# facebookresearch/DetectAndTrack

Hardware: AMD Instinct MI355X
Metric: clips/sec (8-frame 800px) (higher is better)
Workload: dtype bf16; 1 GPU; 3D R-18 FPN3D keypoint R-CNN inference, 4 clip(s) of 1x3x8x768x1344 per step (= per forward) per GPU (kT=3 body+FPN, slice-center 2D heads, per clip: 1000 proposals, 100 detections -> kps_score -> decoded keypoints); mode=infer, weights=random-init (synthetic_params, seed 3), images_per_forward=4, forwards_in_flight=3, clips_in_flight=12, keyframe_dce=False, hip_graph=True, resident_input=True, parallelism=clip-sharded x1 (no data-path collective)

## Files before the change

### detectandtrack_amd/csrc/c_api.hip

```cpp
#include <stdlib.h>

#include "dat_common.h"

int dat_ensure_ws(dat_ctx* ctx, size_t bytes) {
    if (ctx->ws_bytes >= bytes) return DAT_OK;
    const size_t want = bytes + (bytes >> 2);
    void* grown = nullptr;
    if (hipMalloc(&grown, want) != hipSuccess) {
        (void)hipGetLastError();
        DAT_FAIL(ctx, DAT_ERR_ALLOC, "workspace hipMalloc(%zu) failed", want);
    }
    if (ctx->dbg_ws_poison && (hipMemset(grown, 0xFF, want) != hipSuccess || hipDeviceSynchronize() != hipSuccess)) {
        (void)hipGetLastError();
        hipFree(grown);
        DAT_FAIL(ctx, DAT_ERR_ALLOC, "workspace poison fill failed");
    }
    if (ctx->ws) ctx->ws_retired.push_back(ctx->ws);
    ctx->ws = grown;
    ctx->ws_bytes = want;
    ctx->ws_generation++;
    return DAT_OK;
}

extern "C" {

int dat_version(void) { return 1; }
int dat_h16_format(void) { return DAT_H16_FORMAT; }

int dat_ctx_create(dat_ctx** out, int device) {
    if (!out) return DAT_ERR_ARG;
    int ndev = 0;
    if (hipGetDeviceCount(&ndev) != hipSuccess || device < 0 || device >= ndev) return DAT_ERR_ARG;
    if (hipSetDevice(device) != hipSuccess) return DAT_ERR_ARG;
    dat_ctx* c = new dat_ctx();
    c->device = device;
    c->prof_enabled = 0;
    c->prof_ev = nullptr;
    c->prof_cap = c->prof_n = 0;
    c->prof_flops = nullptr;
    c->prof_tag = nullptr;
    c->ws = nullptr;
    c->ws_bytes = 0;
    c->ws_generation = 0;
    c->zeros = nullptr;
    {
        auto env_int = [](const char* name, int dflt) { const char* e = getenv(name); return e ? atoi(e) : dflt; };
        c->force_bp = env_int("DAT_CONV_BP", 0);
        c->force_ks = env_int("DAT_CONV_KSPLIT", 0);
        c->dbg_ablate = env_int("DAT_CONV_ABLATE", 0);
        c->dbg_ntap = env_int("DAT_CONV_NTAP", 1);
        c->dbg_ws64 = env_int("DAT_CONV_WS64", 1);
        c->dbg_pwlw = env_int("DAT_CONV_PWLW", 1);
        c->dbg_pwks = env_int("DAT_CONV_PWKS", 8);
        c->dbg_temporal = env_int("DAT_CONV_TEMPORAL", 1);
        c->dbg_wgrad_direct = env_int("DAT_WGRAD_DIRECT", 1);
        c->dbg_wgrad_ks = env_int("DAT_WGRAD_KS", 0);
        c->dbg_ablate_wgrad = env_int("DAT_WGRAD_ABLATE", 0);
        c->dbg_wgrad_sub = env_int("DAT_WGRAD_SUB", 2);
        c->dbg_pw_xcd = env_int("DAT_CONV_PW_XCD", 1);
        c->dbg_wgrad_pw = env_int("DAT_WGRAD_PW", 1);
        c->dbg_kps_sep = env_int("DAT_KPS_DECODE_SEP", 1);
        c->dbg_linear = env_int("DAT_CONV_LINEAR", 1);
        c->dbg_order = env_int("DAT_CONV_ORDER", 0);
        c->dbg_persist_pct = env_int("DAT_PERSIST_PCT", 100);
        c->dbg_bt_min = env_int("DAT_CONV_BT_MIN", 390);
        c->dbg_bt = env_int("DAT_CONV_BT", 1);
        c->dbg_roi_fold = env_int("DAT_ROI_BWD_FOLD", 1);
        c->dbg_ws_poison = env_int("DAT_WS_POISON", 0);
        c->num_cu = 0;
    }
    c->util_stream = nullptr;
    c->pinned = nullptr;
    if (hipStreamCreateWithFlags((hipStream_t*)&c->util_stream, hipStreamNonBlocking) != hipSuccess ||
        hipHostMalloc(&c->pinned, 256, hipHostMallocDefault) != hipSuccess) {
        if (c->util_stream) hipStreamDestroy((hipStream_t)c->util_stream);
        delete c;
        return DAT_ERR_ALLOC;
    }
    if (hipMalloc(&c->zeros, 512) != hipSuccess || hipMemsetAsync(c->zeros, 0, 512, (hipStream_t)c->util_stream) != hipSuccess ||
        hipStreamSynchronize((hipStream_t)c->util_stream) != hipSuccess) {
        if (c->zeros) hipFree(c->zeros);
        hipHostFree(c->pinned);
        hipStreamDestroy((hipStream_t)c->util_stream);
        delete c;
        return DAT_ERR_ALLOC;
    }
    *out = c;
    return DAT_OK;
}

void dat_ctx_destroy(dat_ctx* ctx) {
    if (!ctx) return;
    if (ctx->prof_ev) {
        for (int i = 0; i < 2 * ctx->prof_cap; ++i) hipEventDestroy(ctx->prof_ev[i]);
        delete[] ctx->prof_ev;
        delete[] ctx->prof_flops;
        delete[] ctx->prof_tag;
    }
    if (ctx->ws) hipFree(ctx->ws);
    for (void* p : ctx->ws_retired) hipFree(p);
    if (ctx->zeros) hipFree(ctx->zeros);
    if (ctx->pinned) hipHostFree(ctx->pinned);
    if (ctx->util_stream) hipStreamDestroy((hipStream_t)ctx->util_stream);
    delete ctx;
}

const char* dat_last_error(dat_ctx* ctx) { return ctx ? ctx->last_error.c_str() : "null dat_ctx"; }

int dat_ws_info(dat_ctx* ctx, void** ptr, size_t* bytes, int* generation) {
    if (!ctx) return DAT_ERR_ARG;
    if (ptr) *ptr = ctx->ws;
    if (bytes) *bytes = ctx->ws_bytes;
    if (generation) *generation = ctx->ws_generation;
    return DAT_OK;
}

int dat_ws_reserve(dat_ctx* ctx, size_t bytes) {
    if (!ctx) return DAT_ERR_ARG;
    return dat_ensure_ws(ctx, bytes);
}

int dat_prof_enable(dat_ctx* ctx, int capacity) {
    if (!ctx) return DAT_ERR_ARG;
    if (capacity <= 0) {
        ctx->prof_enabled = 0;
        return DAT_OK;
    }
    if (capacity > ctx->prof_cap) {
        if (ctx->prof_ev) {
            for (int i = 0; i < 2 * ctx->prof_cap; ++i) hipEventDestroy(ctx->prof_ev[i]);
            delete[] ctx->prof_ev;
            delete[] ctx->prof_flops;
            delete[] ctx->prof_tag;
        }
        ctx->prof_ev = new hipEvent_t[2 * capacity];
        for (int i = 0; i < 2 * capacity; ++i) hipEventCreate(&ctx->prof_ev[i]);
        ctx->prof_flops = new double[capacity];
        ctx->prof_tag = new int[capacity];
        ctx->prof_cap = capacity;
    }
    ctx->prof_n = 0;
    ctx->prof_enabled = 1;
    if (hipDeviceSynchronize() != hipSuccess ||
        hipMemsetAsync((char*)ctx->zeros + 256, 0, 16, (hipStream_t)ctx->util_stream) != hipSuccess ||
        hipStreamSynchronize((hipStream_t)ctx->util_stream) != hipSuccess) return DAT_ERR_LAUNCH;
    return DAT_OK;
}

int dat_prof_clock(dat_ctx* ctx, double* shader_mhz) {
    if (!ctx || !shader_mhz) return DAT_ERR_ARG;
    unsigned long long* h = (unsigned long long*)ctx->pinned;
    if (hipDeviceSynchronize() != hipSuccess ||
        hipMemcpyAsync(h, (char*)ctx->zeros + 256, 16, hipMemcpyDeviceToHost, (hipStream_t)ctx->util_stream) != hipSuccess ||
        hipStreamSynchronize((hipStream_t)ctx->util_stream) != hipSuccess) return DAT_ERR_LAUNCH;
    *shader_mhz = h[1] ? 100.0 * (double)h[0] / (double)h[1] : 0.0;
    return DAT_OK;
}

int dat_prof_read(dat_ctx* ctx, int max_records, int* tags, double* flops, float* ms) {
    if (!ctx) return DAT_ERR_ARG;
    const int n = ctx->prof_n < max_records ? ctx->prof_n : max_records;
    for (int i = 0; i < n; ++i) {
        float t = 0.f;
        if (hipEventSynchronize(ctx->prof_ev[2 * i + 1]) != hipSuccess ||
            hipEventElapsedTime(&t, ctx->prof_ev[2 * i], ctx->prof_ev[2 * i + 1]) != hipSuccess) {
            (void)hipGetLastError();
            t = 0.f;
        }
        if (tags) tags[i] = ctx->prof_tag[i];
        if (flops) flops[i] = ctx->prof_flops[i];
        if (ms) ms[i] = t;
    }
    ctx->prof_n = 0;
    return n;
}

int dat_fill_zero(dat_ctx* ctx, dat_stream s, void* ptr, size_t bytes) {
    DAT_ENFORCE(ctx, ptr || bytes == 0, "fill_zero: null pointer");
    if (bytes == 0) return DAT_OK;
    if (hipMemsetAsync(ptr, 0, bytes, (hipStream_t)s) != hipSuccess) DAT_FAIL(ctx, DAT_ERR_LAUNCH, "fill_zero: hipMemsetAsync failed");
    return DAT_OK;
}

}
```

### detectandtrack_amd/csrc/conv3d_igemm.hip

```cpp
#include "conv_internal.h"

using namespace dat_conv;

namespace {

template <int BP, int NTAP> struct MinWaves { static constexpr int value = (NTAP > 0 && NTAP != 10 && BP == 128) ? 3 : 2; };
template <int DT, int BN, int BP, int WAVES_N, int ONE, int NTAP, int ODT>
__global__ __launch_bounds__(NTHREADS, (MinWaves<BP, NTAP>::value)) void conv3d_igemm_kernel(const ConvParams p) {
    static_assert(ONE == 1, "see the comment above");
    constexpr int ES = ElemOf<DT>::size;
    constexpr int OES = ElemOf<ODT>::size;
    constexpr int CK = Mma<DT>::CK;
    constexpr int WAVES_P = 4 / WAVES_N;
    constexpr int WN = BN / WAVES_N;
    constexpr int WP = BP / WAVES_P;
    constexpr int MT = WN / 32;
    constexpr int PT = WP / 32;
    static_assert(MT >= 1 && PT >= 1, "tile too small");

#ifdef DAT_CONV_TRACE
    const unsigned long long tr_k0 = __builtin_amdgcn_s_memtime();
    unsigned long long tr_k1 = tr_k0;
#endif
    unsigned long long clk_c0 = 0, clk_r0 = 0;
    if (p.clk) { clk_c0 = __builtin_amdgcn_s_memtime(); clk_r0 = __builtin_amdgcn_s_memrealtime(); }
    extern __shared__ __attribute__((aligned(16))) char smem[];
    char* patch = smem;

    const int tid = threadIdx.x;
    const int lane = tid & 63;
    const int wave = __builtin_amdgcn_readfirstlane(tid >> 6);
    const int wave_n = wave % WAVES_N;
    const int wave_p = wave / WAVES_N;

    unsigned bid = blockIdx.x;
    if (!(p.ablate & 16)) bid = xcd_block_map(bid, p.nblocks);
    int split, nb;
    unsigned tile;
    if (p.order) {
        tile = bid % p.ntiles;
        bid /= p.ntiles;
        split = bid % p.ksplit;
        nb = bid / p.ksplit;
    } else {
        split = bid % p.ksplit;
        bid /= p.ksplit;
        nb = bid % p.nblk_n;
        tile = bid / p.nblk_n;
    }
    const int fc = tile % p.otn;
    tile /= p.otn;
    const int tw_i = tile % p.tiles_w;
    tile /= p.tiles_w;
    const int th_i = tile % p.tiles_h;
    const int clip = tile / p.tiles_h;
    const int f = clip * p.otn + fc;
    const int t = p.ot0 + fc;
    const int f_in = clip * p.T + t;
    const int n0 = nb * BN;
    const int TW = 1 << p.tw_log2;
    const int oh0 = th_i << p.th_log2;
    const int ow0 = tw_i * p.tile_w;
    const int ih0 = oh0 * p.sh - p.ph;
    const int iw0 = ow0 * p.sw - p.pw;

    int rowbase[PT];
#pragma unroll
    for (int j = 0; j < PT; ++j) {
        const int pos = wave_p * WP + j * 32 + (lane & 31);
        const int ohl = pos >> p.tw_log2, owl = pos & (TW - 1);
        rowbase[j] = ohl * p.rsh * p.PW + owl * p.rsw;
    }
    const int khalf = lane >> 5;

    f32x16_t acc[MT][PT];
#pragma unroll
    for (int i = 0; i < MT; ++i)
#pragma unroll
        for (int j = 0; j < PT; ++j)
#pragma unroll
            for (int r = 0; r < 16; ++r) acc[i][j][r] = 0.f;

    int kt_lo = 0, kt_hi = p.KT - 1;
    while (kt_lo < p.KT && (t + kt_lo - p.pt) < p.in_lo) ++kt_lo;
    while (kt_hi >= 0 && (t + kt_hi - p.pt) >= p.in_hi) --kt_hi;
    const int n_kt = kt_hi - kt_lo + 1;
    const int ntap = p.KH * p.KW;
    const int ntab = p.tab_n;
    const int npatch = n_kt * p.n_cchunks;
    const int pi_lo = (npatch * split) / p.ksplit, pi_hi = (npatch * (split + 1)) / p.ksplit;
    const int total = (pi_hi - pi_lo) * ntab;

    const int npatch_items = p.PH * p.PW * 8;

    typedef const __attribute__((address_space(1))) void* gptr_t;
    typedef __attribute__((address_space(3))) void* lptr_t;
#ifndef DAT_PATCH_AUX
#define DAT_PATCH_AUX 0
#endif
#define P_DMA(SRC_, DST_) __builtin_amdgcn_global_load_lds((gptr_t)(SRC_), (lptr_t)(DST_), 16, 0, DAT_PATCH_AUX)
#define P_COMMIT() asm volatile("s_waitcnt vmcnt(0)" ::: "memory")

    const size_t wd_cc_stride = (size_t)(p.Cout_pad >> 5) * 4096;
    const char* const wd_lane = p.w + (size_t)((n0 + wave_n * WN) >> 5) * 4096 + lane * 16;
#define WD_PTR(KT_, CC_, TI_) (wd_lane + ((size_t)((KT_) * ntap + p.tab_tap[(TI_)]) * p.n_cchunks + (CC_)) * wd_cc_stride)
    if constexpr (NTAP > 0) {
      constexpr int NT = NTAP == 10 ? 9 : NTAP;
      if (total > 0) {
        constexpr int MAXCH = patch_pieces_per_wave(NTAP, BP);
        const int kt_hi_x = kt_lo + n_kt;
        int kshift = 0;
        if (n_kt == p.KT && (DAT_KT_ROTATE)) kshift = (p.KT - (t + kt_lo - p.pt) % p.KT) % p.KT;
        int kt = kt_lo + pi_lo / p.n_cchunks + kshift, cc = pi_lo % p.n_cchunks;
        if (kt >= kt_hi_x) kt -= n_kt;
        constexpr bool PACK16 = NTAP != 10;
        constexpr int NQ = PACK16 ? (PT + 1) / 2 : PT;
        unsigned qp[NT][NQ];
#pragma unroll
        for (int tp = 0; tp < NT; ++tp)
#pragma unroll
            for (int j = 0; j < PT; ++j) {
                int row = rowbase[j] + p.tab_rowoff[tp];
                if (p.lin_w > 0) {
                    const int gpos = ow0 + wave_p * WP + j * 32 + (lane & 31);
                    const int rem = gpos % (p.lin_h * p.lin_w);
                    const int y = rem / p.lin_w, x = rem - y * p.lin_w;
                    const int yy = y + tp / p.KW - p.KH / 2, xx = x + tp % p.KW - p.KW / 2;
                    if ((unsigned)yy >= (unsigned)p.lin_h || (unsigned)xx >= (unsigned)p.lin_w) row = p.lin_zero_row;
                }
                const int g = (row >> 1) & 7;
                const unsigned a16 = (unsigned)(row * PPITCH) + (unsigned)(((khalf ^ (g & 1)) << 4) | ((g >> 1) << 5));
                if (!PACK16) qp[tp][j] = a16;
                else if (j & 1) qp[tp][j >> 1] |= a16 << 16;
                else qp[tp][j >> 1] = a16;
            }
        const int nchunks = (npatch_items + 63) >> 6;
        int poff[MAXCH];
#pragma unroll
        for (int u = 0; u < MAXCH; ++u) {
            const int c = wave + 4 * u;
            const int it = c * 64 + lane;
            int off = -2;
            if (c < nchunks && it < npatch_items) {
                const int row = it >> 3;
                const int slot = (it ^ (row >> 1)) & 7;
                const int prow = p.pw_magic ? (int)__umulhi((unsigned)row, p.pw_magic) : row, pcol = row - prow * p.PW;
                const int ih = ih0 + p.tab_dy[0] + prow * p.psh, iw = iw0 + p.tab_dx[0] + pcol * p.psw;
                off = (ih >= 0 && ih < p.H && iw >= 0 && iw < p.W && row != p.lin_zero_row) ? (int)((unsigned)(ih * p.W + iw) * (unsigned)(p.Cin * ES) + (unsigned)(slot * 16)) : -1;
            }
            poff[u] = off;
        }
        const size_t tap_stride = (size_t)p.n_cchunks * wd_cc_stride;
        const char* const wd_base = p.w + (size_t)((n0 + wave_n * WN) >> 5) * 4096;
        const unsigned lane16 = (unsigned)lane * 16u;
        const char* wcur = wd_base + ((size_t)(kt * ntap) * p.n_cchunks + cc) * wd_cc_stride;
        uint4 wa[MT][4];
#pragma unroll
        for (int i = 0; i < MT; ++i)
#pragma unroll
            for (int ks = 0; ks < 4; ++ks) wa[i][ks] = *(const uint4*)(wcur + i * 4096 + ks * 1024 + lane16);
        const int npat = pi_hi - pi_lo;
        for (int pi = 0; pi < npat; ++pi) {
            if (!((p.ablate & 1) && pi > 0) && !(p.x3 && pi > 0 && cc % 3 == 1)) {
                __syncthreads();
                const int fin = f_in + kt - p.pt;
                const char* xbase = p.x + ((size_t)fin * p.H * p.W) * p.Cin * ES + (size_t)(p.x3 ? (cc / 3) * 2 + (cc % 3 == 2) : cc) * CK * ES;
#pragma unroll
                for (int u = 0; u < MAXCH; ++u) {
                    if (poff[u] != -2) {
                        const char* src = poff[u] >= 0 ? xbase + (unsigned)poff[u] : p.zeros;
                        P_DMA(src, patch + (wave + 4 * u) * 1024);
                    }
                }
                P_COMMIT();
                __syncthreads();
            }
            int ncc = cc + 1, nkt = kt;
            if (ncc == p.n_cchunks) { ncc = 0; if (++nkt == kt_hi_x) nkt = kt_lo; }
            const char* wnextpatch = (pi + 1 < npat) ? wd_base + ((size_t)(nkt * ntap) * p.n_cchunks + ncc) * wd_cc_stride : wcur;
            __builtin_amdgcn_s_setprio(1);
            uint4 b[2][PT];
            unsigned qa[PT];
#pragma unroll
            for (int jj = 0; jj < NQ; ++jj) asm volatile("" : "+v"(qp[0][jj]));
#pragma unroll
            for (int j = 0; j < PT; ++j) qa[j] = !PACK16 ? qp[0][j % NQ] : (j & 1) ? (qp[0][(j >> 1) % NQ] >> 16) : (qp[0][(j >> 1) % NQ] & 0xffffu);
#pragma unroll
            for (int j = 0; j < PT; ++j) b[0][j] = *(const uint4*)(patch + qa[j]);
#pragma unroll
            for (int tp = 0; tp < NT; ++tp) {
                const char* wnext = (tp + 1 < NT) ? wcur + (size_t)(tp + 1) * tap_stride : wnextpatch;
#pragma unroll
                for (int ks = 0; ks < 4; ++ks) {
                    const int cur = ks & 1, nxt = cur ^ 1;
                    if (ks < 3) {
#pragma unroll
                        for (int j = 0; j < PT; ++j) b[nxt][j] = *(const uint4*)(patch + (qa[j] ^ (unsigned)((ks + 1) << 5)));
                    } else if (tp + 1 < NT) {
#pragma unroll
                        for (int jj = 0; jj < NQ; ++jj) asm volatile("" : "+v"(qp[tp + 1 < NT ? tp + 1 : tp][jj]));
#pragma unroll
                        for (int j = 0; j < PT; ++j) {
                            const unsigned w2 = qp[tp + 1 < NT ? tp + 1 : tp][(PACK16 ? j >> 1 : j) % NQ];
                            qa[j] = !PACK16 ? w2 : (j & 1) ? (w2 >> 16) : (w2 & 0xffffu);
                        }
#pragma unroll
                        for (int j = 0; j < PT; ++j) b[nxt][j] = *(const uint4*)(patch + qa[j]);
                    }
#pragma unroll
                    for (int i = 0; i < MT; ++i)
#pragma unroll
                        for (int j = 0; j < PT; ++j) Mma<DT>::step(wa[i][ks], b[cur][j], acc[i][j]);
#pragma unroll
                    for (int i = 0; i < MT; ++i) wa[i][ks] = *(const uint4*)(wnext + i * 4096 + ks * 1024 + lane16);
                    __builtin_amdgcn_sched_barrier(0);
                }
            }
            __builtin_amdgcn_s_setprio(0);
            wcur = wnextpatch;
            cc = ncc; kt = nkt;
        }
      }
    } else
    if (total > 0) {
        const int kt_hi_x = kt_lo + n_kt;
        int kshift = 0;
        if (n_kt == p.KT && (DAT_KT_ROTATE)) kshift = (p.KT - (t + kt_lo - p.pt) % p.KT) % p.KT;
        int kt = kt_lo + pi_lo / p.n_cchunks + kshift, cc = pi_lo % p.n_cchunks, ti = 0;
        if (kt >= kt_hi_x) kt -= n_kt;
        uint4 wa[MT][4];
        {
            const char* w0 = WD_PTR(kt, cc, 0);
#pragma unroll
            for (int i = 0; i < MT; ++i)
#pragma unroll
                for (int ks = 0; ks < 4; ++ks) wa[i][ks] = *(const uint4*)(w0 + i * 4096 + ks * 1024);
        }
        const int nchunks = (npatch_items + 63) >> 6;
#ifdef DAT_CONV_TRACE
        unsigned long long tr_reload = 0, tr_wait = 0, tr_bar = 0, tr_issue = 0, tr_mma = 0, tr_t;
#define TR_NOW() __builtin_readcyclecounter()
#define TR_ADD(ACC_) { const unsigned long long n_ = TR_NOW(); ACC_ += n_ - tr_t; tr_t = n_; }
        tr_t = TR_NOW();
        const unsigned long long tr_c0 = __builtin_amdgcn_s_memtime(), tr_r0 = __builtin_amdgcn_s_memrealtime();
#else
#define TR_ADD(ACC_)
#endif
        for (int step = 0; step < total; ++step) {
            const bool x3_same = p.x3 && p.tab_new == 1u && step > 0 && cc % 3 == 1;
            if (((p.tab_new >> ti) & 1u) && !((p.ablate & 1) && step > 0) && !(p.ablate & 8) && !x3_same) {
                __syncthreads();
                const int fin = f_in + kt - p.pt;
                const char* xbase = p.x + ((size_t)fin * p.H * p.W) * p.Cin * ES + (size_t)(p.x3 ? (cc / 3) * 2 + (cc % 3 == 2) : cc) * CK * ES;
                const int py0 = ih0 + p.tab_dy[ti], px0 = iw0 + p.tab_dx[ti];
#pragma unroll 2
                for (int c = wave; c < nchunks; c += 4) {
                    const int it = c * 64 + lane;
                    if (it < npatch_items) {
                        const int row = it >> 3;
                        const int slot = (it ^ (row >> 1)) & 7;
                        const int prow = p.pw_magic ? (int)__umulhi((unsigned)row, p.pw_magic) : row, pcol = row - prow * p.PW;
                        const int ih = py0 + prow * p.psh, iw = px0 + pcol * p.psw;
                        const char* src = p.zeros;
                        if (ih >= 0 && ih < p.H && iw >= 0 && iw < p.W)
                            src = xbase + ((unsigned)(ih * p.W + iw) * (unsigned)(p.Cin * ES) + (unsigned)(slot * 16));
                        P_DMA(src, patch + c * 1024);
                    }
                }
            }
            TR_ADD(tr_reload);
            if ((p.tab_new >> ti) & 1u) {
                P_COMMIT();
                TR_ADD(tr_wait);
                __syncthreads();
            }
            TR_ADD(tr_bar);
            int nti = ti + 1, ncc = cc, nkt = kt;
            if (nti == ntab) {
                nti = 0;
                if (++ncc == p.n_cchunks) { ncc = 0; if (++nkt == kt_hi_x) nkt = kt_lo; }
            }
            const char* const wnext = (step + 1 < total) ? WD_PTR(nkt, ncc, nti) : WD_PTR(kt, cc, ti);

            TR_ADD(tr_issue);
            __builtin_amdgcn_s_setprio(1);
            {
                const int tapoff = p.tab_rowoff[ti];
                const char* bp[PT];
                int bx[PT];
#pragma unroll
                for (int j = 0; j < PT; ++j) {
                    const int row = rowbase[j] + tapoff;
                    const int g = (row >> 1) & 7;
                    bp[j] = patch + (row * PPITCH + ((khalf ^ (g & 1)) << 4));
                    bx[j] = g >> 1;
                }
                uint4 b[2][PT];
#pragma unroll
                for (int j = 0; j < PT; ++j) b[0][j] = *(const uint4*)(bp[j] + (bx[j] << 5));
#pragma unroll
                for (int ks = 0; ks < 4; ++ks) {
                    const int cur = ks & 1, nxt = cur ^ 1;
                    if (ks < 3) {
#pragma unroll
                        for (int j = 0; j < PT; ++j) b[nxt][j] = *(const uint4*)(bp[j] + (((ks + 1) ^ bx[j]) << 5));
                    }
#pragma unroll
                    for (int i = 0; i < MT; ++i)
#pragma unroll
                        for (int j = 0; j < PT; ++j) Mma<DT>::step(wa[i][ks], b[cur][j], acc[i][j]);
#pragma unroll
                    for (int i = 0; i < MT; ++i) wa[i][ks] = *(const uint4*)(wnext + i * 4096 + ks * 1024);
                    __builtin_amdgcn_sched_barrier(0);
                }
            }
            __builtin_amdgcn_s_setprio(0);
            ti = nti; cc = ncc; kt = nkt;
            TR_ADD(tr_mma);
        }
#ifdef DAT_CONV_TRACE
        if (tid == 0 && p.dbg) {
            atomicAdd(&p.dbg[0], tr_reload); atomicAdd(&p.dbg[1], tr_wait); atomicAdd(&p.dbg[2], tr_bar);
            atomicAdd(&p.dbg[3], tr_issue); atomicAdd(&p.dbg[4], tr_mma); atomicAdd(&p.dbg[5], (unsigned long long)total);
            atomicAdd(&p.dbg[6], __builtin_amdgcn_s_memtime() - tr_c0);
            atomicAdd(&p.dbg[7], __builtin_amdgcn_s_memrealtime() - tr_r0);
        }
        tr_k1 = __builtin_amdgcn_s_memtime();
#endif
    }
#undef WD_PTR
#undef P_COMMIT
#undef P_DMA

    static_assert(WN == 64, "epilogue staging assumes 64 channels per wave");
    constexpr int CPL = 16 / OES;
    constexpr int LPP = WN / CPL;
    constexpr int PPI = 64 / LPP;
    __syncthreads();
    char* est = smem + wave * (32 * EPI_PITCH);
    const int sl_c = (lane % LPP) * CPL;
    const int sl_p = lane / LPP;
    const int cbase = n0 + wave_n * WN;
    const int c_st = cbase + sl_c;
    const bool part_mode = p.ksplit > 1;
    float sc[CPL], bi[CPL];
#pragma unroll
    for (int e = 0; e < CPL; ++e) {
        const bool ok = (c_st + e) < p.Cout;
        sc[e] = (!part_mode && p.scale && ok) ? p.scale[c_st + e] : 1.f;
        bi[e] = (!part_mode && p.bias && ok) ? p.bias[c_st + e] : 0.f;
    }
    const size_t npos_all = (size_t)p.frames * p.Ho * p.Wo;
    const size_t tile_pos = ((size_t)f * p.Ho + oh0) * p.Wo + ow0;
    char* const ybase = p.y + tile_pos * p.out_cs * OES;
    const char* const rbase = p.res_mode == 2 ? p.res + (size_t)f * (p.Ho >> 1) * (p.Wo >> 1) * p.out_cs * OES
                                              : p.res + tile_pos * p.out_cs * OES;
    const char* const abase = p.res2 + tile_pos * p.out_cs * OES;
    float* const pbase = part_mode ? p.part + ((size_t)split * npos_all + tile_pos) * p.Cout : nullptr;
    constexpr int NQ = 32 / PPI;
    const bool m4 = p.res_mode == 4;
    const bool res_pre = p.res_mode && !m4 && !part_mode && (p.out_cs & 7) == 0 && c_st + CPL <= p.Cout;
    uint4 rq[2][NQ];
    auto res_fetch = [&](int j, uint4* dst) __attribute__((always_inline)) {
#pragma unroll
        for (int q = 0; q < NQ; ++q) {
            const int pos = wave_p * WP + j * 32 + q * PPI + sl_p;
            const int ohl = pos >> p.tw_log2, owl = pos & (TW - 1);
            const int oh = oh0 + ohl, ow = ow0 + owl;
            const bool live = oh < p.Ho && ow < p.Wo && !(p.ablate & 4);
            unsigned rpos = (unsigned)(ohl * p.Wo + owl);
            if (p.res_mode == 2) rpos = (unsigned)((oh >> 1) * (p.Wo >> 1) + (ow >> 1));
            dst[q] = *(const uint4*)(rbase + (live ? (rpos * (unsigned)p.out_cs + (unsigned)c_st) * (unsigned)OES : 0u));
        }
    };
    if (res_pre) res_fetch(0, rq[0]);
#pragma unroll
    for (int j = 0; j < PT; ++j) {
        if (res_pre && j + 1 < PT) res_fetch(j + 1, rq[(j + 1) & 1]);
#pragma unroll
        for (int i = 0; i < MT; ++i)
#pragma unroll
            for (int g = 0; g < 4; ++g)
                *(float4*)(est + (lane & 31) * EPI_PITCH + (i * 32 + g * 8 + khalf * 4) * 4) =
                    make_float4(acc[i][j][g * 4 + 0], acc[i][j][g * 4 + 1], acc[i][j][g * 4 + 2], acc[i][j][g * 4 + 3]);
        __builtin_amdgcn_wave_barrier();
#pragma unroll
        for (int q = 0; q < NQ; ++q) {
            const int pl = q * PPI + sl_p;
            float v[CPL];
#pragma unroll
            for (int e4 = 0; e4 < CPL / 4; ++e4) {
                const float4 t = *(const float4*)(est + pl * EPI_PITCH + (sl_c + e4 * 4) * 4);
                v[e4 * 4 + 0] = t.x; v[e4 * 4 + 1] = t.y; v[e4 * 4 + 2] = t.z; v[e4 * 4 + 3] = t.w;
            }
            const int pos = wave_p * WP + j * 32 + pl;
            const int ohl = pos >> p.tw_log2, owl = pos & (TW - 1);
            const int oh = oh0 + ohl, ow = ow0 + owl;
            if (oh >= p.Ho || ow >= p.Wo || c_st >= p.Cout || (p.ablate & 4)) continue;
            const unsigned lpos = (unsigned)(ohl * p.Wo + owl);
            const int nch = min(CPL, p.Cout - c_st);
            if (part_mode) {
                float* dst = pbase + (lpos * (unsigned)p.Cout + (unsigned)c_st);
#pragma unroll
                for (int e4 = 0; e4 < CPL / 4; ++e4)
                    if (e4 * 4 < nch) *(float4*)(dst + e4 * 4) = make_float4(v[e4 * 4], v[e4 * 4 + 1], v[e4 * 4 + 2], v[e4 * 4 + 3]);
                continue;
            }
#pragma unroll
            for (int e = 0; e < CPL; ++e) v[e] = v[e] * sc[e] + bi[e];
            if (res_pre) {
                const uint4 r = rq[j & 1][q];
                if (ODT == DAT_BF16) {
                    const uint32_t ru[4] = {r.x, r.y, r.z, r.w};
#pragma unroll
                    for (int e2 = 0; e2 < CPL / 2; ++e2) {
                        v[2 * e2] = res_combine(v[2 * e2], bf2f((uint16_t)(ru[e2 % 4] & 0xffff)), p.res_mode);
                        v[2 * e2 + 1] = res_combine(v[2 * e2 + 1], bf2f((uint16_t)(ru[e2 % 4] >> 16)), p.res_mode);
                    }
                } else {
                    v[0] = res_combine(v[0], __uint_as_float(r.x), p.res_mode); v[1] = res_combine(v[1], __uint_as_float(r.y), p.res_mode);
                    v[2] = res_combine(v[2], __uint_as_float(r.z), p.res_mode); v[3] = res_combine(v[3], __uint_as_float(r.w), p.res_mode);
                }
            } else if (m4) {
                const unsigned off = (lpos * (unsigned)p.out_cs + (unsigned)c_st) * (unsigned)OES;
                const char* rp = rbase + off;
                const char* ap = abase + off;
                if (ODT == DAT_BF16) {
#pragma unroll
                    for (int e4 = 0; e4 < CPL / 4; ++e4)
                        if (e4 * 4 < nch) {
                            const uint2 r = *(const uint2*)(rp + e4 * 8), o = *(const uint2*)(ap + e4 * 8);
                            v[e4 * 4 + 0] = res_combine4(v[e4 * 4 + 0], bf2f((uint16_t)(o.x & 0xffff)), bf2f((uint16_t)(r.x & 0xffff)));
                            v[e4 * 4 + 1] = res_combine4(v[e4 * 4 + 1], bf2f((uint16_t)(o.x >> 16)), bf2f((uint16_t)(r.x >> 16)));
                            v[e4 * 4 + 2] = res_combine4(v[e4 * 4 + 2], bf2f((uint16_t)(o.y & 0xffff)), bf2f((uint16_t)(r.y & 0xffff)));
                            v[e4 * 4 + 3] = res_combine4(v[e4 * 4 + 3], bf2f((uint16_t)(o.y >> 16)), bf2f((uint16_t)(r.y >> 16)));
                        }
                } else {
                    const float4 r = *(const float4*)rp, o = *(const float4*)ap;
                    v[0] = res_combine4(v[0], o.x, r.x); v[1] = res_combine4(v[1], o.y, r.y);
                    v[2] = res_combine4(v[2], o.z, r.z); v[3] = res_combine4(v[3], o.w, r.w);
                }
            } else if (p.res_mode) {
                unsigned rpos = lpos;
                if (p.res_mode == 2) rpos = (unsigned)((oh >> 1) * (p.Wo >> 1) + (ow >> 1));
                const char* rp = rbase + (rpos * (unsigned)p.out_cs + (unsigned)c_st) * (unsigned)OES;
                if (ODT == DAT_BF16) {
#pragma unroll
                    for (int e4 = 0; e4 < CPL / 4; ++e4)
                        if (e4 * 4 < nch) {
                            const uint2 r = *(const uint2*)(rp + e4 * 8);
                            v[e4 * 4 + 0] = res_combine(v[e4 * 4 + 0], bf2f((uint16_t)(r.x & 0xffff)), p.res_mode);
                            v[e4 * 4 + 1] = res_combine(v[e4 * 4 + 1], bf2f((uint16_t)(r.x >> 16)), p.res_mode);
                            v[e4 * 4 + 2] = res_combine(v[e4 * 4 + 2], bf2f((uint16_t)(r.y & 0xffff)), p.res_mode);
                            v[e4 * 4 + 3] = res_combine(v[e4 * 4 + 3], bf2f((uint16_t)(r.y >> 16)), p.res_mode);
                        }
                } else {
                    const float4 r = *(const float4*)rp;
                    v[0] = res_combine(v[0], r.x, p.res_mode); v[1] = res_combine(v[1], r.y, p.res_mode);
                    v[2] = res_combine(v[2], r.z, p.res_mode); v[3] = res_combine(v[3], r.w, p.res_mode);
                }
            }
            if (p.relu) {
#pragma unroll
                for (int e = 0; e < CPL; ++e) v[e] = fmaxf(v[e], 0.f);
            }
            char* yp = ybase + (lpos * (unsigned)p.out_cs + (unsigned)c_st) * (unsigned)OES;
            if (ODT == DAT_BF16) {
                uint32_t o[CPL / 2];
#pragma unroll
                for (int e2 = 0; e2 < CPL / 2; ++e2) o[e2] = f2bf2(v[2 * e2], v[2 * e2 + 1]);
                if (nch == CPL && (p.out_cs & 7) == 0) {
                    *(uint4*)yp = make_uint4(o[0], o[1], o[2], o[3]);
                } else {
                    *(uint2*)yp = make_uint2(o[0], o[1]);
                    if (nch > 4) *(uint2*)(yp + 8) = make_uint2(o[2], o[3]);
                }
            } else {
                *(float4*)yp = make_float4(v[0], v[1], v[2], v[3]);
                if (ODT == DAT_F32 && DT == DAT_BF16 && p.y_split)
                    split_hi_lo_store(p.y_split + ((tile_pos + lpos) * (size_t)(2 * p.out_cs) + (size_t)((c_st >> 6) * 128 + (c_st & 63))) * 2, v);
            }
        }
        __builtin_amdgcn_wave_barrier();
    }
    if (p.clk && threadIdx.x == 0) {
        atomicAdd(&p.clk[0], __builtin_amdgcn_s_memtime() - clk_c0);
        atomicAdd(&p.clk[1], __builtin_amdgcn_s_memrealtime() - clk_r0);
    }
#ifdef DAT_CONV_TRACE
    asm volatile("s_waitcnt vmcnt(0)" ::: "memory");
    if (tid == 0 && p.dbg) {
        const unsigned long long e = __builtin_amdgcn_s_memtime();
        atomicAdd(&p.dbg[8], e - tr_k0);
        atomicAdd(&p.dbg[9], e - tr_k1);
    }
#endif
}

template <int DT>
__global__ void splitk_finish_kernel(const float* __restrict__ part, int ksplit, size_t npos, int Cout, int out_cs,
                                     const float* __restrict__ scale, const float* __restrict__ bias,
                                     const char* __restrict__ res, int res_mode, int frames, int Ho, int Wo, int relu,
                                     char* y, char* __restrict__ y_split = nullptr, const char* res2 = nullptr) {
    const int c4 = Cout >> 2;
    const size_t total = npos * c4;
    for (size_t i = blockIdx.x * (size_t)blockDim.x + threadIdx.x; i < total; i += (size_t)gridDim.x * blockDim.x) {
        const int c = (int)(i % c4) * 4;
        const size_t opos = i / c4;
        float4 a = *(const float4*)(part + opos * Cout + c);
        for (int s = 1; s < ksplit; ++s) {
            const float4 b = *(const float4*)(part + ((size_t)s * npos + opos) * Cout + c);
            a.x += b.x; a.y += b.y; a.z += b.z; a.w += b.w;
        }
        float v[4] = {a.x, a.y, a.z, a.w};
        if (scale) { const float4 s4 = *(const float4*)(scale + c); v[0] *= s4.x; v[1] *= s4.y; v[2] *= s4.z; v[3] *= s4.w; }
        if (bias) { const float4 b4 = *(const float4*)(bias + c); v[0] += b4.x; v[1] += b4.y; v[2] += b4.z; v[3] += b4.w; }
        if (res_mode) {
            size_t rpos = opos;
            if (res_mode == 2) {
                const int ow = opos % Wo;
                const size_t q = opos / Wo;
                const int oh = q % Ho;
                const size_t f = q / Ho;
                rpos = (f * (Ho >> 1) + (oh >> 1)) * (Wo >> 1) + (ow >> 1);
            }
            if (res_mode == 4) {
                if (DT == DAT_BF16) {
                    const uint2 r = *(const uint2*)(res + (rpos * out_cs + c) * 2), o = *(const uint2*)(res2 + (opos * out_cs + c) * 2);
                    v[0] = res_combine4(v[0], bf2f((uint16_t)(o.x & 0xffff)), bf2f((uint16_t)(r.x & 0xffff)));
                    v[1] = res_combine4(v[1], bf2f((uint16_t)(o.x >> 16)), bf2f((uint16_t)(r.x >> 16)));
                    v[2] = res_combine4(v[2], bf2f((uint16_t)(o.y & 0xffff)), bf2f((uint16_t)(r.y & 0xffff)));
                    v[3] = res_combine4(v[3], bf2f((uint16_t)(o.y >> 16)), bf2f((uint16_t)(r.y >> 16)));
                } else {
                    const float4 r = *(const float4*)(res + (rpos * out_cs + c) * 4), o = *(const float4*)(res2 + (opos * out_cs + c) * 4);
                    v[0] = res_combine4(v[0], o.x, r.x); v[1] = res_combine4(v[1], o.y, r.y);
                    v[2] = res_combine4(v[2], o.z, r.z); v[3] = res_combine4(v[3], o.w, r.w);
                }
            } else if (DT == DAT_BF16) {
                const uint2 r = *(const uint2*)(res + (rpos * out_cs + c) * 2);
                v[0] = res_combine(v[0], bf2f((uint16_t)(r.x & 0xffff)), res_mode); v[1] = res_combine(v[1], bf2f((uint16_t)(r.x >> 16)), res_mode);
                v[2] = res_combine(v[2], bf2f((uint16_t)(r.y & 0xffff)), res_mode); v[3] = res_combine(v[3], bf2f((uint16_t)(r.y >> 16)), res_mode);
            } else {
                const float4 r = *(const float4*)(res + (rpos * out_cs + c) * 4);
                v[0] = res_combine(v[0], r.x, res_mode); v[1] = res_combine(v[1], r.y, res_mode);
                v[2] = res_combine(v[2], r.z, res_mode); v[3] = res_combine(v[3], r.w, res_mode);
            }
        }
        if (relu) { v[0] = fmaxf(v[0], 0.f); v[1] = fmaxf(v[1], 0.f); v[2] = fmaxf(v[2], 0.f); v[3] = fmaxf(v[3], 0.f); }
        if (DT == DAT_BF16) {
            uint2 o;
            o.x = f2bf2(v[0], v[1]);
            o.y = f2bf2(v[2], v[3]);
            *(uint2*)(y + (opos * out_cs + c) * 2) = o;
        } else {
            *(float4*)(y + (opos * out_cs + c) * 4) = make_float4(v[0], v[1], v[2], v[3]);
            if (y_split) split_hi_lo_store(y_split + (opos * (size_t)(2 * out_cs) + (size_t)((c >> 6) * 128 + (c & 63))) * 2, v);
        }
    }
}

static long long linear_tiles(const dat_ctx* ctx, const dat_conv_desc* d, const ConvParams& p, int bpv) {
    if (!ctx->dbg_linear || !ctx->dbg_ntap || d->KH != 3 || d->KW != 3 || d->stride_h != 1 || d->stride_w != 1 || d->res_mode == 2 ||
        p.H != p.Ho || p.W != p.Wo)
        return 0;
    if (d->KT == 1 && (d->pad_t != 0 || d->out_tn > 0)) return 0;
    const long long per = d->KT > 1 ? (long long)p.Ho * p.Wo : (long long)p.frames * p.Ho * p.Wo;
    const long long nr = bpv + 2 * (p.Wo + 1) + 1;
    if (((nr * 8 + 63) >> 6) > 4 * patch_pieces_per_wave(9, bpv) || nr * PPITCH >= 65536 ||
        per * std::max(p.Cin, std::max(p.out_cs, p.Cout)) * 4 >= (1ll << 31))
        return 0;
    return (d->KT > 1 ? (long long)p.frames : 1) * ((per + bpv - 1) / bpv);
}

}

namespace dat_conv {

TileChoice choose_tile(int Ho, int Wo, int bp_log2, int sh, int sw, int KH, int KW) {
    TileChoice best{0, bp_log2};
    double best_cost = 1e30;
    for (int a = 0; a <= bp_log2; ++a) {
        const int b = bp_log2 - a;
        const long long th = 1 << a, tw = 1 << b;
        const long long tiles = cdiv_ll(Ho, th) * cdiv_ll(Wo, tw);
        const double waste = (double)(tiles * th * tw) / ((double)Ho * Wo);
        const long long PH = th + (KH - 1) / sh;
        const long long PW = tw + (KW - 1) / sw;
        const double halo = (double)(PH * PW) / (double)(th * tw);
        const double conflict = (tw < 32 && KW > 1) ? 1.06 : 1.0;
        const double cost = waste * (1.0 + 0.15 * (halo - 1.0)) * conflict;
        if (cost < best_cost - 1e-9) {
            best_cost = cost;
            best = TileChoice{a, b};
        }
    }
    return best;
}

void conv_build_tap_table(ConvParams& p) {
    int n = 0;
    p.tab_new = 0;
    for (int py = 0; py < p.sh && py < p.KH; ++py)
        for (int px = 0; px < p.sw && px < p.KW; ++px) {
            bool first = true;
            for (int kh = py; kh < p.KH; kh += p.sh)
                for (int kw = px; kw < p.KW; kw += p.sw) {
                    p.tab_tap[n] = kh * p.KW + kw;
                    p.tab_rowoff[n] = (kh / p.sh) * p.PW + (kw / p.sw);
                    p.tab_dy[n] = (short)py;
                    p.tab_dx[n] = (short)px;
                    if (first) p.tab_new |= 1u << n;
                    first = false;
                    ++n;
                }
        }
    p.tab_n = n;
}

int conv_set_frame_window(dat_ctx* ctx, const dat_conv_desc* d, ConvParams& p, const char* who) {
    p.in_lo = d->in_tn > 0 ? d->in_t0 : 0;
    p.in_hi = d->in_tn > 0 ? d->in_t0 + d->in_tn : d->T;
    DAT_ENFORCE(ctx, p.in_lo >= 0 && p.in_hi <= d->T, "%s: non-zero input frames [%d, %d) outside T %d", who, p.in_lo, p.in_hi, d->T);
    p.ot0 = d->out_tn > 0 ? d->out_t0 : 0;
    p.otn = d->out_tn > 0 ? d->out_tn : d->T;
    DAT_ENFORCE(ctx, p.ot0 >= 0 && p.ot0 + p.otn <= d->T, "%s: output frames [%d, %d) outside T %d", who, p.ot0, p.ot0 + p.otn, d->T);
    p.frames = d->frames / d->T * p.otn;
    return DAT_OK;
}

}

namespace {

template <int DT, int BN, int BP, int WAVES_N, int NTAP, int ODT>
int launch_conv(dat_ctx* ctx, hipStream_t st, ConvParams& p, int bp_log2, int ksplit, bool linear = false) {
    TileChoice tc = choose_tile(p.Ho, p.Wo, bp_log2, p.sh, p.sw, p.KH, p.KW);
    p.lin_h = p.lin_w = 0;
    p.lin_zero_row = -1;
    if (linear) {
        const bool per_frame = p.KT > 1;
        const long long total = per_frame ? (long long)p.Ho * p.Wo : (long long)p.frames * p.Ho * p.Wo;
        DAT_ENFORCE(ctx, NTAP == 9 && (per_frame || p.pt == 0) && p.sh == 1 && p.sw == 1 && p.H == p.Ho && p.W == p.Wo && p.res_mode != 2 &&
                             total * std::max(p.Cin, std::max(p.out_cs, p.Cout)) * 4 < (1ll << 31),
                    "conv3d: linear tiling on an unsupported layer");
        p.lin_h = p.H; p.lin_w = p.W;
        const int wr = p.W, nr = BP + 2 * (wr + 1) + 1;
        tc = TileChoice{0, bp_log2};
        p.H = p.Ho = 1; p.W = p.Wo = (int)total;
        if (!per_frame) { p.frames = 1; p.T = 1; p.ot0 = 0; p.otn = 1; p.in_lo = 0; p.in_hi = 1; }
        p.ph = 0; p.pw = wr + 1;
        p.lin_zero_row = nr - 1;
        p.th_log2 = 0; p.tw_log2 = bp_log2;
        p.tile_w = BP;
        p.tiles_h = 1; p.tiles_w = (int)cdiv_ll(total, BP);
        p.psh = p.psw = 1; p.rsh = p.rsw = 1;
        p.PH = 1; p.PW = nr;
        p.tab_new = 1u; p.tab_n = 9;
        for (int i = 0; i < 9; ++i) { p.tab_tap[i] = i; p.tab_rowoff[i] = (i / 3) * wr + i % 3; p.tab_dy[i] = p.tab_dx[i] = 0; }
    }
    const int th = 1 << tc.th_log2, tw = 1 << tc.tw_log2;
    if (!linear) {
    p.th_log2 = tc.th_log2;
    p.tw_log2 = tc.tw_log2;
    p.tile_w = tw;
    p.tiles_h = (p.Ho + th - 1) / th;
    p.tiles_w = (p.Wo + tw - 1) / tw;
    p.psh = p.sh;
    p.psw = p.sw;
    p.rsh = p.rsw = 1;
    p.PH = th + (p.KH - 1) / p.sh;
    p.PW = tw + (p.KW - 1) / p.sw;
    }
    if (linear) {
    } else if (NTAP == 10) {
        p.psh = p.psw = 1;
        p.rsh = p.sh; p.rsw = p.sw;
        p.PH = (th - 1) * p.sh + p.KH;
        p.PW = (tw - 1) * p.sw + p.KW;
        p.tab_new = 1u;
        p.tab_n = p.KH * p.KW;
        for (int i = 0; i < p.tab_n; ++i) {
            p.tab_tap[i] = i;
            p.tab_rowoff[i] = (i / p.KW) * p.PW + i % p.KW;
            p.tab_dy[i] = p.tab_dx[i] = 0;
        }
    } else {
        DAT_ENFORCE(ctx, p.KH * p.KW <= 32, "conv3d: %dx%d spatial kernel exceeds the 32-entry tap table", p.KH, p.KW);
        conv_build_tap_table(p);
    }
    p.pw_magic = conv_pw_magic(p.PW);
    p.n_cchunks = p.x3 ? p.Cin / Mma<DT>::CK / 2 * 3 : p.Cin / Mma<DT>::CK;
    p.ablate = ctx->dbg_ablate;
    p.nblk_n = p.Cout_pad / BN;
    long long nblocks = (long long)p.frames * p.tiles_h * p.tiles_w * p.nblk_n;
    {
        const int npatch_min = (p.KT > 1 ? p.KT - 1 : 1) * p.n_cchunks;
        int ks = ksplit < 1 ? 1 : (ksplit > npatch_min ? npatch_min : ksplit);
        p.ksplit = ks;
        p.part = nullptr;
        if (ks > 1) {
            const size_t bytes = (size_t)ks * p.frames * p.Ho * p.Wo * p.Cout * sizeof(float);
            int rc = dat_ensure_ws(ctx, bytes);
            if (rc != DAT_OK) return rc;
            p.part = (float*)ctx->ws;
        }
        nblocks *= ks;
    }
    DAT_ENFORCE(ctx, nblocks > 0 && nblocks < (1ll << 31), "conv3d: grid of %lld blocks unsupported", nblocks);
    DAT_ENFORCE(ctx, (long long)p.Ho * p.Wo * std::max(p.out_cs, p.Cout) * 4 < (1ll << 31),
                "conv3d: one output frame of %dx%dx%d exceeds the 2-GB range of the epilogue's 32-bit offsets", p.Ho, p.Wo, p.out_cs);
    p.nblocks = (unsigned)nblocks;
    p.ntiles = (unsigned)(nblocks / ((long long)p.ksplit * p.nblk_n));
    p.order = ctx->dbg_order > 0;
    size_t lds = ((size_t)p.PH * p.PW * PPITCH + 1023) & ~(size_t)1023;
    if (lds < EPI_SLICES_BYTES) lds = EPI_SLICES_BYTES;
    DAT_ENFORCE(ctx, lds <= 160 * 1024, "conv3d: LDS patch of %zu bytes exceeds 160 KiB (tile %dx%d, stride %dx%d)", lds,
                th, tw, p.sh, p.sw);
    auto kern = conv3d_igemm_kernel<DT, BN, BP, WAVES_N, 1, NTAP, ODT>;
    if (NTAP > 0) {
        DAT_ENFORCE(ctx, p.tab_n == (NTAP == 10 ? 9 : NTAP) && p.tab_new == 1u &&
                             (((size_t)p.PH * p.PW * 8 + 63) >> 6) <= (size_t)4 * patch_pieces_per_wave(NTAP, BP) && (NTAP == 10 || (size_t)p.PH * p.PW * PPITCH < 65536),
                    "conv3d: unrolled-tap variant on an unsupported shape (%d taps, patch %dx%d)", p.tab_n, p.PH, p.PW);
        for (int i = 0; i < p.tab_n; ++i) DAT_ENFORCE(ctx, p.tab_tap[i] == i, "conv3d: unrolled-tap variant needs taps in natural order");
    }
    {
        const int rc = dat_ensure_lds(ctx, (const void*)kern, 160 * 1024);
        if (rc != DAT_OK) return rc;
    }
#ifdef DAT_CONV_TRACE
    static unsigned long long* dbg = nullptr;
    if (!dbg) hipMalloc(&dbg, 128);
    hipMemsetAsync(dbg, 0, 128, st);
    p.dbg = dbg;
#endif
    hipLaunchKernelGGL(kern, dim3(p.nblocks), dim3(NTHREADS), lds, st, p);
#ifdef DAT_CONV_TRACE
    {
        unsigned long long h[16];
        hipStreamSynchronize(st);
        hipMemcpy(h, dbg, 128, hipMemcpyDeviceToHost);
        if (h[5]) fprintf(stderr, "TRACE BN=%d BP=%d blocks=%u steps/blk=%.1f | per step: reload %.0f wait %.0f barrier %.0f issue %.0f mma %.0f | shader clock %.0f MHz | per block: total %.0f epilogue %.0f cycles\n",
                          BN, BP, p.nblocks, (double)h[5] / p.nblocks, (double)h[0] / h[5], (double)h[1] / h[5], (double)h[2] / h[5],
                          (double)h[3] / h[5], (double)h[4] / h[5], 100.0 * (double)h[6] / (double)h[7], (double)h[8] / p.nblocks, (double)h[9] / p.nblocks);
    }
#endif
    if (p.ksplit > 1) {
        const size_t npos = (size_t)p.frames * p.Ho * p.Wo;
        const size_t tot = npos * (p.Cout >> 2);
        const int blocks = (int)std::min<size_t>((tot + 255) / 256, 256 * 16);
        hipLaunchKernelGGL(splitk_finish_kernel<ODT>, dim3(blocks), dim3(256), 0, st, (const float*)p.part, p.ksplit, npos, p.Cout,
                           p.out_cs, p.scale, p.bias, p.res, p.res_mode, p.frames, p.Ho, p.Wo, p.relu, p.y, ODT == DAT_F32 && DT == DAT_BF16 ? p.y_split : nullptr, p.res2);
    }
    DAT_CHECK_LAUNCH(ctx, "conv3d_igemm");
    return DAT_OK;
}

}

extern "C" {

int dat_conv3d_out_shape(const dat_conv_desc* d, int* Ho, int* Wo) {
    if (!d || d->stride_h < 1 || d->stride_w < 1) return DAT_ERR_ARG;
    *Ho = (d->H + 2 * d->pad_h - d->KH) / d->stride_h + 1;
    *Wo = (d->W + 2 * d->pad_w - d->KW) / d->stride_w + 1;
    return DAT_OK;
}

size_t dat_conv3d_packed_weight_bytes(const dat_conv_desc* d) {
    if (d->dtype == DAT_BF16X3) return (size_t)d->KT * d->KH * d->KW * cout_pad_of(d) * d->Cin * 3 * 2;
    return (size_t)d->KT * d->KH * d->KW * cout_pad_of(d) * d->Cin * dat_esize(d->dtype);
}

double dat_conv3d_flops(const dat_conv_desc* d, int Cin_real, int Cout_real) {
    int Ho, Wo;
    dat_conv3d_out_shape(d, &Ho, &Wo);
    const double oframes = d->out_tn > 0 && d->T > 0 ? (double)(d->frames / d->T) * d->out_tn : (double)d->frames;
    return 2.0 * Cout_real * Cin_real * d->KT * d->KH * d->KW * oframes * Ho * Wo;
}

static int conv3d_fwd_impl(dat_ctx* ctx, dat_stream s, const dat_conv_desc* d, const void* x, const void* w_packed,
                           const float* scale, const float* bias, const void* residual, void* y, void* y_split, const void* addend = nullptr);

int dat_conv3d_fwd(dat_ctx* ctx, dat_stream s, const dat_conv_desc* d, const void* x, const void* w_packed,
                   const float* scale, const float* bias, const void* residual, void* y) {
    return conv3d_fwd_impl(ctx, s, d, x, w_packed, scale, bias, residual, y, nullptr);
}

int dat_conv3d_fwd_x3(dat_ctx* ctx, dat_stream s, const dat_conv_desc* d, const void* x_split, const void* w_packed,
                      const float* scale, const float* bias, const void* residual, void* y, void* y_split) {
    DAT_ENFORCE(ctx, d && d->dtype == DAT_BF16X3, "conv3d_fwd_x3: the descriptor's dtype must be DAT_BF16X3");
    DAT_ENFORCE(ctx, !y_split || (d->out_cstride % 64 == 0 && d->Cout == d->out_cstride),
                "conv3d_fwd_x3: a split output needs Cout == out_cstride, a multiple of 64 (got %d / %d)", d->Cout, d->out_cstride);
    return conv3d_fwd_impl(ctx, s, d, x_split, w_packed, scale, bias, residual, y, y_split);
}

int dat_conv3d_fwd_sum_mask(dat_ctx* ctx, dat_stream s, const dat_conv_desc* d, const void* x, const void* w_packed,
                            const float* scale, const float* bias, const void* addend, const void* mask, void* y) {
    DAT_ENFORCE(ctx, d && d->res_mode == 4, "conv3d_fwd_sum_mask: the descriptor's res_mode must be 4");
    DAT_ENFORCE(ctx, addend && mask, "conv3d_fwd_sum_mask: null addend / mask");
    return conv3d_fwd_impl(ctx, s, d, x, w_packed, scale, bias, mask, y, nullptr, addend);
}

static int conv3d_fwd_impl(dat_ctx* ctx, dat_stream s, const dat_conv_desc* d, const void* x, const void* w_packed,
                           const float* scale, const float* bias, const void* residual, void* y, void* y_split, const void* addend) {
    DAT_ENFORCE(ctx, d && x && w_packed && y, "conv3d_fwd: null argument");
    DAT_ENFORCE(ctx, d->dtype == DAT_F32 || d->dtype == DAT_BF16 || d->dtype == DAT_BF16X3, "conv3d_fwd: bad dtype %d", d->dtype);
    const bool x3 = d->dtype == DAT_BF16X3;
    DAT_ENFORCE(ctx, !x3 || DAT_H16_FORMAT == 0, "conv3d_fwd: DAT_BF16X3 needs the bf16 build of the library (this one holds IEEE half in its 16-bit tensors)");
    DAT_ENFORCE(ctx, d->Cin % 64 == 0, "conv3d_fwd: Cin (channel stride) %d must be a multiple of 64", d->Cin);
    DAT_ENFORCE(ctx, d->Cout % 4 == 0 && d->out_cstride % 4 == 0 && d->out_cstride >= d->Cout,
                "conv3d_fwd: Cout %d / out_cstride %d must be multiples of 4", d->Cout, d->out_cstride);
    DAT_ENFORCE(ctx, d->frames % d->T == 0, "conv3d_fwd: frames %d not a multiple of T %d", d->frames, d->T);
    DAT_ENFORCE(ctx, d->res_mode >= 0 && d->res_mode <= 4, "conv3d_fwd: res_mode %d", d->res_mode);
    DAT_ENFORCE(ctx, d->res_mode != 4 || (!x3 && !y_split && addend), "conv3d_fwd: res_mode 4 (sum + mask) goes through dat_conv3d_fwd_sum_mask, bf16 / fp32 only");
    DAT_ENFORCE(ctx, d->res_mode == 0 || residual, "conv3d_fwd: res_mode %d needs a residual pointer", d->res_mode);
    DAT_ENFORCE(ctx, d->pad_t * 2 + 1 == d->KT || d->out_tn > 0,
                "conv3d_fwd: temporal pad %d must be (KT-1)/2 for KT %d unless out_t0/out_tn select the output frames",
                d->pad_t, d->KT);
    ConvParams p;
    memset(&p, 0, sizeof(p));
    p.x = (const char*)x; p.w = (const char*)w_packed; p.scale = scale; p.bias = bias;
    p.res = (const char*)residual; p.res2 = (const char*)addend; p.y = (char*)y; p.y_split = (char*)y_split;
    p.zeros = (const char*)ctx->zeros;
    p.clk = ctx->prof_enabled ? (unsigned long long*)((char*)ctx->zeros + 256) : nullptr;
    {
        const int rcw = conv_set_frame_window(ctx, d, p, "conv3d_fwd");
        if (rcw != DAT_OK) return rcw;
    }
    p.T = d->T; p.H = d->H; p.W = d->W; p.Cin = x3 ? 2 * d->Cin : d->Cin;
    p.x3 = x3;
    dat_conv3d_out_shape(d, &p.Ho, &p.Wo);
    DAT_ENFORCE(ctx, p.Ho > 0 && p.Wo > 0, "conv3d_fwd: empty output %dx%d", p.Ho, p.Wo);
    DAT_ENFORCE(ctx, d->res_mode != 2 || (p.Ho % 2 == 0 && p.Wo % 2 == 0), "conv3d_fwd: res_mode 2 needs even output dims");
    p.Cout = d->Cout; p.out_cs = d->out_cstride; p.Cout_pad = cout_pad_of(d);
    p.KT = d->KT; p.KH = d->KH; p.KW = d->KW; p.sh = d->stride_h; p.sw = d->stride_w;
    p.pt = d->pad_t; p.ph = d->pad_h; p.pw = d->pad_w; p.relu = d->relu; p.res_mode = d->res_mode;
    hipStream_t st = (hipStream_t)s;

    const bool small_n = d->Cout <= 64;
    const int force_bp = ctx->force_bp, force_ks = ctx->force_ks;
    const int ck = d->dtype == DAT_F32 ? 32 : 64;
    const int ncc = x3 ? d->Cin / 64 * 3 : d->Cin / ck;
    const int npatch = d->KT * ncc, npatch_min = (d->KT > 1 ? d->KT - 1 : 1) * ncc;
    const int ntaps = d->KH * d->KW;
    const long long nbn = p.Cout_pad / (small_n ? 64 : 128);
    int bp = 128, ksplit = 1;
    {
        double best = 1e30;
        const bool deep_1x1 = (ntaps == 1 && ncc >= 16);
        for (int cand_bp = 128; cand_bp <= 256; cand_bp += 128) {
            if (cand_bp == 256 && (small_n || ntaps == 1)) continue;
            if (cand_bp == 256 && !force_bp && ctx->dbg_ntap && !(ctx->dbg_ntap & 4) && d->KH == 3 && d->KW == 3 && d->stride_h == 2 && d->stride_w == 2) continue;
            if (force_bp && cand_bp != force_bp && !(force_bp == 256 && (small_n || ntaps == 1))) continue;
            const int lg = cand_bp == 256 ? 8 : 7;
            const TileChoice tc = choose_tile(p.Ho, p.Wo, lg, p.sh, p.sw, p.KH, p.KW);
            long long tiles = cdiv_ll(p.Ho, 1ll << tc.th_log2) * cdiv_ll(p.Wo, 1ll << tc.tw_log2) * p.frames;
            {
                const long long tl = linear_tiles(ctx, d, p, cand_bp);
                if (tl > 0 && tl * 10 <= tiles * 9) tiles = tl;
            }
            const int ks_max = (ntaps > 1 || deep_1x1) ? (deep_1x1 ? 8 : 4) : 1;
            for (int ks = 1; ks <= ks_max && ks <= npatch_min; ++ks) {
                if (force_ks && ks != std::min(force_ks, npatch_min)) continue;
                const double nblk = (double)tiles * nbn * ks;
                const double slots = 512.0;
                double rounds = nblk / slots;
                if (rounds <= 3.0) rounds = ceil(rounds); else rounds += 0.5;
                const double steps = ceil((double)npatch / ks) * ntaps;
                const bool strided_taps = ntaps > 1 && (d->stride_h > 1 || d->stride_w > 1);
                const double step_us = cand_bp == 256 ? (strided_taps ? 2.8 : 2.15) : 1.35;
                const double fixed_us = 2.0 + 0.6 * ceil((double)npatch / ks);
                double t = rounds * (steps * step_us + fixed_us);
                if (ks > 1) t += 4.0 + 2.0 * ks * (double)p.frames * p.Ho * p.Wo * d->Cout * 4.0 / 3.0e6;
                if (t < best) { best = t; bp = cand_bp; ksplit = ks; }
            }
        }
    }
    const bool big = bp == 256;
    int tag = (small_n ? 64 : 128) * 10000 + bp * 10 + d->dtype;
    ProfBracket prof(ctx, st);
    int rc;
    long long bt_blocks = 0;
    if (bt_eligible(ctx, d)) bt_tile_twl(p, &bt_blocks);
    const long long ncu = ctx_num_cu(ctx), bt_rounds = cdiv_ll(bt_blocks, ncu);
    const bool bt_fits = ctx->dbg_bt >= 2 ? bt_blocks * 2 >= 3 * ncu : (bt_blocks * 100 >= (long long)ctx->dbg_bt_min * ncu && bt_blocks * 100 >= bt_rounds * ncu * 95);
    const bool mask_mode = d->res_mode >= 3;
    if (bt_fits && ksplit == 1 && !force_bp && !force_ks && !mask_mode) {
        tag = 256 * 10000 + 2560 + d->dtype;
        rc = launch_bt(ctx, st, p);
    } else if (pw256_eligible(ctx, d) && !force_bp && !force_ks && !mask_mode) {
        tag = 256 * 10000 + 320 + d->dtype;
        rc = launch_pw256(ctx, st, p);
    } else if (pwks_eligible(ctx, d) && !force_bp && !force_ks) {
        tag = 256 * 10000 + 340 + d->dtype;
        rc = launch_pwks(ctx, st, p);
    } else if (tks_eligible(ctx, d) && !force_bp && !force_ks) {
        tag = 256 * 10000 + 350 + d->dtype;
        rc = launch_tks(ctx, st, p);
    } else if (pwlw_eligible(ctx, d) && !force_bp && !force_ks && d->res_mode != 3) {
        tag = 256 * 10000 + 330 + d->dtype;
        rc = launch_pwlw(ctx, st, p, d);
    } else if (ws64_eligible(ctx, d) && !force_bp && !force_ks && !mask_mode) {
        tag = 64 * 10000 + 9990 + d->dtype;
        rc = launch_ws64(ctx, st, p);
    } else {
        const TileChoice tc = choose_tile(p.Ho, p.Wo, big ? 8 : 7, p.sh, p.sw, p.KH, p.KW);
        const long long prow = ((1ll << tc.th_log2) + (p.KH - 1) / p.sh) * ((1ll << tc.tw_log2) + (p.KW - 1) / p.sw);
        const bool fits = ((prow * 8 + 63) >> 6) <= 4 * patch_pieces_per_wave(9, big ? 256 : 128);
        const bool pw_small = (long long)p.frames * p.Ho * p.Wo <= 65536;
        const long long drow = (((1ll << tc.th_log2) - 1) * p.sh + p.KH) * (((1ll << tc.tw_log2) - 1) * p.sw + p.KW);
        const bool dense2 = ctx->dbg_ntap && !big && d->KH == 3 && d->KW == 3 && d->stride_h == 2 && d->stride_w == 2 && !(ctx->dbg_ntap & 4) &&
                            ((drow * 8 + 63) >> 6) <= 4 * 19;
        const int ntapv = dense2 ? 10 : !ctx->dbg_ntap || !fits ? 0 : (d->KH == 3 && d->KW == 3 && d->stride_h == 1 && d->stride_w == 1) ? 9 :
                          (d->KH == 1 && d->KW == 1 && (pw_small || (ctx->dbg_ntap & 2))) ? 1 : 0;
        bool lin = false;
        const long long tlin = ntapv == 9 ? linear_tiles(ctx, d, p, big ? 256 : 128) : 0;
        if (tlin > 0) {
            const long long t2d = (long long)p.frames * cdiv_ll(p.Ho, 1ll << tc.th_log2) * cdiv_ll(p.Wo, 1ll << tc.tw_log2);
            lin = tlin * 10 <= t2d * 9;
        }
#define DAT_CONV_LAUNCH(DT_, BN_, WN_, ODT_) (ntapv == 10 ? launch_conv<DT_, BN_, 128, WN_, 10, ODT_>(ctx, st, p, 7, ksplit) : ntapv == 9 ? (big ? launch_conv<DT_, BN_, 256, WN_, 9, ODT_>(ctx, st, p, 8, ksplit, lin) : launch_conv<DT_, BN_, 128, WN_, 9, ODT_>(ctx, st, p, 7, ksplit, lin)) \
                            : ntapv == 1 ? (big ? launch_conv<DT_, BN_, 256, WN_, 1, ODT_>(ctx, st, p, 8, ksplit) : launch_conv<DT_, BN_, 128, WN_, 1, ODT_>(ctx, st, p, 7, ksplit)) \
                            : (big ? launch_conv<DT_, BN_, 256, WN_, 0, ODT_>(ctx, st, p, 8, ksplit) : launch_conv<DT_, BN_, 128, WN_, 0, ODT_>(ctx, st, p, 7, ksplit)))
        if (x3) rc = small_n ? DAT_CONV_LAUNCH(DAT_BF16, 64, 1, DAT_F32) : DAT_CONV_LAUNCH(DAT_BF16, 128, 2, DAT_F32);
        else if (small_n) rc = d->dtype == DAT_BF16 ? DAT_CONV_LAUNCH(DAT_BF16, 64, 1, DAT_BF16) : DAT_CONV_LAUNCH(DAT_F32, 64, 1, DAT_F32);
        else rc = d->dtype == DAT_BF16 ? DAT_CONV_LAUNCH(DAT_BF16, 128, 2, DAT_BF16) : DAT_CONV_LAUNCH(DAT_F32, 128, 2, DAT_F32);
#undef DAT_CONV_LAUNCH
    }
    prof.end(2.0 * d->Cout * d->Cin * d->KT * d->KH * d->KW * (double)p.frames * p.Ho * p.Wo, tag);
    return rc;
}

int dat_conv3d_persistent_share(dat_ctx* ctx, int percent) {
    if (!ctx) return DAT_ERR_ARG;
    DAT_ENFORCE(ctx, percent >= 1 && percent <= 100, "conv3d_persistent_share: %d percent out of range", percent);
    ctx->dbg_persist_pct = percent;
    return DAT_OK;
}

int dat_conv3d_tune_plan(dat_ctx* ctx, int positions_per_block, int ksplit) {
    if (!ctx) return DAT_ERR_ARG;
    DAT_ENFORCE(ctx, (positions_per_block == 0 || positions_per_block == 128 || positions_per_block == 256) && ksplit >= 0 && ksplit <= 8,
                "conv3d_tune_plan: positions per block %d / split-K %d out of range", positions_per_block, ksplit);
    ctx->force_bp = positions_per_block;
    ctx->force_ks = ksplit;
    return DAT_OK;
}

}
```

### detectandtrack_amd/csrc/conv_epilogue.h

```cpp
#ifndef DAT_CONV_EPILOGUE_H
#define DAT_CONV_EPILOGUE_H

namespace dat_conv __attribute__((visibility("hidden"))) {

constexpr int EPI_PITCH = 64 * 4 + 16;
constexpr int EPI_SLICES_BYTES = 4 * 32 * EPI_PITCH;

__device__ __forceinline__ unsigned xcd_block_map(unsigned bid, unsigned nblocks) {
    const unsigned nx = 8, q = nblocks / nx, r = nblocks % nx;
    const unsigned xcd = bid % nx, k = bid / nx;
    return (xcd < r ? xcd * (q + 1) : r * (q + 1) + (xcd - r) * q) + k;
}

template <int PITCH = EPI_PITCH>
__device__ __forceinline__ void epi_stage(char* est, int row, int khalf, int i, const f32x16_t& acc) {
#pragma unroll
    for (int g = 0; g < 4; ++g)
        *(float4*)(est + row * PITCH + (i * 32 + g * 8 + khalf * 4) * 4) = make_float4(acc[g * 4 + 0], acc[g * 4 + 1], acc[g * 4 + 2], acc[g * 4 + 3]);
}

template <int CPL, int PITCH = EPI_PITCH>
__device__ __forceinline__ void epi_load(const char* est, int pl, int sl_c, float (&v)[CPL]) {
#pragma unroll
    for (int e4 = 0; e4 < CPL / 4; ++e4) {
        const float4 t = *(const float4*)(est + pl * PITCH + sl_c * 4 + e4 * 16);
        v[e4 * 4 + 0] = t.x; v[e4 * 4 + 1] = t.y; v[e4 * 4 + 2] = t.z; v[e4 * 4 + 3] = t.w;
    }
}

template <int CPL>
__device__ __forceinline__ void epi_affine(float (&v)[CPL], const float (&sc)[CPL], const float (&bi)[CPL]) {
#pragma unroll
    for (int e = 0; e < CPL; ++e) v[e] = v[e] * sc[e] + bi[e];
}

template <int ODT, int CPL>
__device__ __forceinline__ void epi_residual(float (&v)[CPL], const uint4& r, int mode) {
    if (ODT == DAT_BF16) {
        const uint32_t ru[4] = {r.x, r.y, r.z, r.w};
#pragma unroll
        for (int e2 = 0; e2 < CPL / 2; ++e2) {
            v[2 * e2] = res_combine(v[2 * e2], bf2f((uint16_t)(ru[e2 % 4] & 0xffff)), mode);
            v[2 * e2 + 1] = res_combine(v[2 * e2 + 1], bf2f((uint16_t)(ru[e2 % 4] >> 16)), mode);
        }
    } else {
        v[0] = res_combine(v[0], __uint_as_float(r.x), mode); v[1] = res_combine(v[1], __uint_as_float(r.y), mode);
        v[2] = res_combine(v[2], __uint_as_float(r.z), mode); v[3] = res_combine(v[3], __uint_as_float(r.w), mode);
    }
}

template <int ODT, int CPL>
__device__ __forceinline__ void epi_residual4(float (&v)[CPL], const uint4& addend, const uint4& mask) {
    static_assert(ODT == DAT_BF16, "the kernels that prefetch both rows of mode 4 are 16-bit ones");
    const uint32_t au[4] = {addend.x, addend.y, addend.z, addend.w}, mu[4] = {mask.x, mask.y, mask.z, mask.w};
#pragma unroll
    for (int e2 = 0; e2 < CPL / 2; ++e2) {
        v[2 * e2] = res_combine4(v[2 * e2], bf2f((uint16_t)(au[e2 % 4] & 0xffff)), bf2f((uint16_t)(mu[e2 % 4] & 0xffff)));
        v[2 * e2 + 1] = res_combine4(v[2 * e2 + 1], bf2f((uint16_t)(au[e2 % 4] >> 16)), bf2f((uint16_t)(mu[e2 % 4] >> 16)));
    }
}

template <int CPL>
__device__ __forceinline__ void epi_relu(float (&v)[CPL], int relu) {
    if (relu) {
#pragma unroll
        for (int e = 0; e < CPL; ++e) v[e] = fmaxf(v[e], 0.f);
    }
}

template <int ODT, int CPL>
__device__ __forceinline__ void epi_store(char* yp, const float (&v)[CPL]) {
    static_assert(CPL == (ODT == DAT_BF16 ? 8 : 4), "a lane stores 16 bytes");
    if (ODT == DAT_BF16) *(uint4*)yp = make_uint4(f2bf2(v[0], v[1]), f2bf2(v[2], v[3]), f2bf2(v[4 % CPL], v[5 % CPL]), f2bf2(v[6 % CPL], v[7 % CPL]));
    else *(float4*)yp = make_float4(v[0], v[1], v[2], v[3]);
}

__device__ __forceinline__ void split_hi_lo_store(char* sp, const float* v) {
    const uint32_t h0 = f2bf2(v[0], v[1]), h1 = f2bf2(v[2], v[3]);
    const uint32_t l0 = f2bf2(v[0] - __uint_as_float(h0 << 16), v[1] - __uint_as_float(h0 & 0xffff0000u));
    const uint32_t l1 = f2bf2(v[2] - __uint_as_float(h1 << 16), v[3] - __uint_as_float(h1 & 0xffff0000u));
    *(uint2*)sp = make_uint2(h0, h1);
    *(uint2*)(sp + 128) = make_uint2(l0, l1);
}

}

#endif
```

### detectandtrack_amd/csrc/conv_internal.h

```cpp
#ifndef DAT_CONV_INTERNAL_H
#define DAT_CONV_INTERNAL_H

#include <math.h>
#include <stdlib.h>

#include <type_traits>
#include <utility>

#include "dat_common.h"

namespace dat_conv __attribute__((visibility("hidden"))) {

constexpr int PPITCH = 128;
constexpr int NTHREADS = 256;
#ifndef DAT_KT_ROTATE
#define DAT_KT_ROTATE 1
#endif

constexpr int patch_pieces_per_wave(int ntap, int bp) { return ntap == 10 ? 19 : bp >= 256 ? 14 : 10; }

struct ConvParams {
    const char* x;
    const char* w;
    const float* scale;
    const float* bias;
    const char* res;
    const char* res2;
    char* y;
    char* y_split;
    unsigned long long* dbg;
    unsigned long long* clk;
    const char* zeros;
    int frames, T, H, W, Cin;
    int ot0, otn;
    int in_lo, in_hi;
    int Ho, Wo, Cout, out_cs, Cout_pad;
    int KT, KH, KW, sh, sw, pt, ph, pw;
    int relu, res_mode;
    int th_log2, tw_log2;
    int tiles_h, tiles_w;
    int PH, PW;
    int psh, psw;
    int rsh, rsw;
    int lin_h, lin_w;
    int tile_w;
    int lin_zero_row;
    int tab_n;
    int tab_tap[32];
    int tab_rowoff[32];
    short tab_dy[32], tab_dx[32];
    unsigned tab_new;
    unsigned pw_magic;
    int n_cchunks;
    int ksplit;
    float* part;
    int ablate;
    int nblk_n;
    unsigned nblocks;
    unsigned ntiles;
    int x3;
    int order;
};

template <int DT> struct Mma;
template <> struct Mma<DAT_BF16> {
    static constexpr int CK = 64;
    __device__ static __forceinline__ void step(const uint4& a, const uint4& b, f32x16_t& c) {
        c = DAT_MFMA16(a, b, c);
    }
};
template <> struct Mma<DAT_F32> {
    static constexpr int CK = 32;
    __device__ static __forceinline__ void step(const uint4& a, const uint4& b, f32x16_t& c) {
        c = __builtin_amdgcn_mfma_f32_32x32x2f32(__uint_as_float(a.x), __uint_as_float(b.x), c, 0, 0, 0);
        c = __builtin_amdgcn_mfma_f32_32x32x2f32(__uint_as_float(a.y), __uint_as_float(b.y), c, 0, 0, 0);
        c = __builtin_amdgcn_mfma_f32_32x32x2f32(__uint_as_float(a.z), __uint_as_float(b.z), c, 0, 0, 0);
        c = __builtin_amdgcn_mfma_f32_32x32x2f32(__uint_as_float(a.w), __uint_as_float(b.w), c, 0, 0, 0);
    }
};

__device__ __forceinline__ float res_combine(float v, float r, int mode) { return mode == 3 ? (r > 0.f ? v : 0.f) : v + r; }
__device__ __forceinline__ float res_combine4(float v, float old, float m) { return m > 0.f ? v + old : 0.f; }

}

#include "conv_epilogue.h"

namespace dat_conv __attribute__((visibility("hidden"))) {

template <int... I, class F>
__device__ __forceinline__ void static_for(std::integer_sequence<int, I...>, F&& f) {
    (f(std::integral_constant<int, I>{}), ...);
}


inline int cout_pad_of(const dat_conv_desc* d) {
    const int bn = d->Cout <= 64 ? 64 : 128;
    return (d->Cout + bn - 1) / bn * bn;
}

struct TileChoice {
    int th_log2, tw_log2;
};
TileChoice choose_tile(int Ho, int Wo, int bp_log2, int sh, int sw, int KH, int KW);
void conv_build_tap_table(ConvParams& p);
inline unsigned conv_pw_magic(int PW) { return PW == 1 ? 0u : (unsigned)((0x100000000ull + (unsigned)PW - 1) / (unsigned)PW); }
int conv_set_frame_window(dat_ctx* ctx, const dat_conv_desc* d, ConvParams& p, const char* who);

struct ProfBracket {
    dat_ctx* ctx;
    hipStream_t st;
    hipEvent_t e1 = nullptr;
    ProfBracket(dat_ctx* ctx_, hipStream_t st_) : ctx(ctx_), st(st_) {
        hipStreamCaptureStatus cap_st = hipStreamCaptureStatusNone;
        if (ctx->prof_enabled && ctx->prof_n < ctx->prof_cap && hipStreamIsCapturing(st, &cap_st) == hipSuccess &&
            cap_st == hipStreamCaptureStatusNone) {
            e1 = ctx->prof_ev[2 * ctx->prof_n + 1];
            hipEventRecord(ctx->prof_ev[2 * ctx->prof_n], st);
        }
    }
    void end(double flops, int tag) {
        if (!e1) return;
        hipEventRecord(e1, st);
        ctx->prof_flops[ctx->prof_n] = flops;
        ctx->prof_tag[ctx->prof_n] = tag;
        ctx->prof_n++;
    }
};

int ctx_num_cu(dat_ctx* ctx);
bool ws64_eligible(const dat_ctx* ctx, const dat_conv_desc* d);
int launch_ws64(dat_ctx* ctx, hipStream_t st, const ConvParams& cp);
bool pw256_eligible(const dat_ctx* ctx, const dat_conv_desc* d);
int launch_pw256(dat_ctx* ctx, hipStream_t st, const ConvParams& cp);
bool pwlw_eligible(dat_ctx* ctx, const dat_conv_desc* d);
int launch_pwlw(dat_ctx* ctx, hipStream_t st, const ConvParams& cp, const dat_conv_desc* d);
bool pwks_eligible(dat_ctx* ctx, const dat_conv_desc* d);
int launch_pwks(dat_ctx* ctx, hipStream_t st, const ConvParams& cp);
bool tks_eligible(dat_ctx* ctx, const dat_conv_desc* d);
int launch_tks(dat_ctx* ctx, hipStream_t st, const ConvParams& cp);
bool bt_eligible(const dat_ctx* ctx, const dat_conv_desc* d);
int bt_tile_twl(const ConvParams& p, long long* nblocks);
int launch_bt(dat_ctx* ctx, hipStream_t st, ConvParams& p);

int launch_wgrad_finish(dat_ctx* ctx, hipStream_t st, const float* Gt, const float* scale, float* dW, int Cout, int Cin, int ntaps);

}

#endif
```

### detectandtrack_amd/csrc/conv_special.hip

```cpp
#include "conv_internal.h"

using namespace dat_conv;

namespace {

struct Ws64Params {
    const char* x;
    const char* w;
    const float* scale;
    const float* bias;
    const char* res;
    char* y;
    const char* zeros;
    int frames, H, W, out_cs, relu, res_mode;
    int tiles_h, tiles_w, ntiles;
    int ablate;
};

template <int TWL>
__global__ __launch_bounds__(NTHREADS) __attribute__((amdgpu_waves_per_eu(1, 1))) void conv3x3_c64_ws_kernel(const Ws64Params p) {
    constexpr int TW = 1 << TWL, TH = 256 >> TWL, PW = TW + 2, PH = TH + 2;
    constexpr int NPIX = PH * PW, NPIECE = (NPIX * 8 + 63) / 64, PBYTES = NPIECE * 1024, UMAX = (NPIECE + 3) / 4;
    extern __shared__ __attribute__((aligned(16))) char smem[];
    const int tid = threadIdx.x, lane = tid & 63;
    const int wave = __builtin_amdgcn_readfirstlane(tid >> 6);
    const int khalf = lane >> 5, n = lane & 31;
    char* const est = smem + 2 * PBYTES + wave * (32 * EPI_PITCH);
    typedef const __attribute__((address_space(1))) void* gptr_t;
    typedef __attribute__((address_space(3))) void* lptr_t;

    typedef unsigned u32x4_t __attribute__((ext_vector_type(4)));
    constexpr int VT = 3;
    u32x4_t wv[VT][2][4], wg[9 - VT][2][4];
    {
        const char* wl = p.w + lane * 16;
#pragma unroll
        for (int tp = 0; tp < 9; ++tp)
#pragma unroll
            for (int mb = 0; mb < 2; ++mb)
#pragma unroll
                for (int ks = 0; ks < 4; ++ks) {
                    const u32x4_t v = *(const u32x4_t*)(wl + ((tp * 2 + mb) * 4 + ks) * 1024);
                    if (tp < VT) wv[tp][mb][ks] = v; else wg[tp - VT][mb][ks] = v;
                }
    }
#define WS_MFMA0_V(ACC_, A_, B_) asm volatile(DAT_MFMA16_OP " %0, %1, %2, 0" : "=&a"(ACC_) : "v"(A_), "v"(B_) : "memory")
#define WS_MFMA_V(ACC_, A_, B_) asm volatile(DAT_MFMA16_OP " %0, %1, %2, %0" : "+a"(ACC_) : "v"(A_), "v"(B_) : "memory")
#define WS_MFMA_A(ACC_, A_, B_) asm volatile(DAT_MFMA16_OP " %0, %1, %2, %0" : "+a"(ACC_) : "a"(A_), "v"(B_) : "memory")
    unsigned qp[9];
#pragma unroll
    for (int tp = 0; tp < 9; ++tp) {
        unsigned q = 0;
#pragma unroll
        for (int j = 0; j < 2; ++j) {
            const int r = TWL == 5 ? 2 * wave + j : 4 * wave + 2 * j + (n >> 4), c = TWL == 5 ? n : (n & 15);
            const int row = (r + tp / 3) * PW + c + tp % 3;
            const int g = (row >> 1) & 7;
            const unsigned a16 = (unsigned)(row * PPITCH) + (unsigned)(((khalf ^ (g & 1)) << 4) | ((g >> 1) << 5));
            q |= a16 << (16 * j);
        }
        qp[tp] = q;
    }
    static_assert(PBYTES < 65536, "two 16-bit patch addresses per register");
    const int sl_c = (lane & 7) * 8, sl_p = lane >> 3;
    float sc[8], bi[8];
#pragma unroll
    for (int e = 0; e < 8; ++e) {
        sc[e] = p.scale ? p.scale[sl_c + e] : 1.f;
        bi[e] = p.bias ? p.bias[sl_c + e] : 0.f;
    }
    const int tiles_per_frame = p.tiles_h * p.tiles_w;

#define WS_DMA(TL_, B_)                                                                                                   \
    {                                                                                                                     \
        const int f_ = (TL_) / tiles_per_frame, r_ = (TL_) - f_ * tiles_per_frame;                                        \
        const int th_ = r_ / p.tiles_w, tw_ = r_ - th_ * p.tiles_w;                                                       \
        const int ih0_ = th_ * TH - 1, iw0_ = tw_ * TW - 1;                                                               \
        const char* xf_ = p.x + (size_t)f_ * p.H * p.W * 128;                                                             \
        _Pragma("unroll") for (int u_ = 0; u_ < UMAX; ++u_) {                                                             \
            const int piece_ = wave + 4 * u_;                                                                             \
            if (piece_ < NPIECE) {                                                                                        \
                const int it_ = piece_ * 64 + lane, row_ = it_ >> 3;                                                      \
                const int slot_ = (it_ ^ (row_ >> 1)) & 7;                                                                \
                const int prow_ = row_ / PW, pcol_ = row_ - prow_ * PW;                                                   \
                const int ih_ = ih0_ + prow_, iw_ = iw0_ + pcol_;                                                         \
                const bool ok_ = row_ < NPIX && (unsigned)ih_ < (unsigned)p.H && (unsigned)iw_ < (unsigned)p.W;           \
                const char* src_ = ok_ ? xf_ + ((unsigned)(ih_ * p.W + iw_) * 128u + (unsigned)(slot_ * 16)) : p.zeros;   \
                __builtin_amdgcn_global_load_lds((gptr_t)src_, (lptr_t)(smem + (B_) * PBYTES + piece_ * 1024), 16, 0, 0); \
            }                                                                                                             \
        }                                                                                                                 \
    }

    int tile = blockIdx.x;
    if (tile < p.ntiles) WS_DMA(tile, 0);
    asm volatile("s_waitcnt vmcnt(0)" ::: "memory");
    int buf = 0;
    for (; tile < p.ntiles; tile += gridDim.x, buf ^= 1) {
        __syncthreads();
        const int next = tile + gridDim.x;
        if (next < p.ntiles && !(p.ablate & 1)) WS_DMA(next, buf ^ 1);
        f32x16_t acc[2][2];
        const unsigned boff = (unsigned)buf * PBYTES;
        __builtin_amdgcn_s_setprio(1);
        u32x4_t bq[3][2];
        unsigned a0 = 0, a1 = 0;
#define WS_READ(S_)                                                                                  \
        {                                                                                            \
            if ((S_) % 4 == 0) {                                                                     \
                unsigned q_ = qp[(S_) / 4];                                                          \
                asm volatile("" : "+v"(q_));    \
                a0 = (q_ & 0xffffu) + boff; a1 = (q_ >> 16) + boff;                                  \
            }                                                                                        \
            asm volatile("ds_read_b128 %0, %1" : "=v"(bq[(S_) % 3][0]) : "v"(a0 ^ (unsigned)(((S_) % 4) << 5)) : "memory"); \
            asm volatile("ds_read_b128 %0, %1" : "=v"(bq[(S_) % 3][1]) : "v"(a1 ^ (unsigned)(((S_) % 4) << 5)) : "memory"); \
        }
        WS_READ(0);
        WS_READ(1);
#pragma unroll
        for (int st = 0; st < 36; ++st) {
            if (st + 2 < 36) WS_READ(st + 2);
            if (st + 2 < 36) asm volatile("s_waitcnt lgkmcnt(4)" ::: "memory");
            else if (st + 1 < 36) asm volatile("s_waitcnt lgkmcnt(2)" ::: "memory");
            else asm volatile("s_waitcnt lgkmcnt(0)" ::: "memory");
            const int tp = st / 4, ks = st % 4;
            const u32x4_t b0 = bq[st % 3][0], b1 = bq[st % 3][1];
            if (st == 0) {
                WS_MFMA0_V(acc[0][0], wv[0][0][0], b0); WS_MFMA0_V(acc[1][0], wv[0][1][0], b0);
                WS_MFMA0_V(acc[0][1], wv[0][0][0], b1); WS_MFMA0_V(acc[1][1], wv[0][1][0], b1);
            } else if (tp < VT) {
                WS_MFMA_V(acc[0][0], wv[tp < VT ? tp : 0][0][ks], b0); WS_MFMA_V(acc[1][0], wv[tp < VT ? tp : 0][1][ks], b0);
                WS_MFMA_V(acc[0][1], wv[tp < VT ? tp : 0][0][ks], b1); WS_MFMA_V(acc[1][1], wv[tp < VT ? tp : 0][1][ks], b1);
            } else {
                WS_MFMA_A(acc[0][0], wg[tp >= VT ? tp - VT : 0][0][ks], b0); WS_MFMA_A(acc[1][0], wg[tp >= VT ? tp - VT : 0][1][ks], b0);
                WS_MFMA_A(acc[0][1], wg[tp >= VT ? tp - VT : 0][0][ks], b1); WS_MFMA_A(acc[1][1], wg[tp >= VT ? tp - VT : 0][1][ks], b1);
            }
        }
#undef WS_READ
        asm volatile("s_nop 15\n\ts_nop 15" ::: "memory");
        __builtin_amdgcn_s_setprio(0);
        asm volatile("s_waitcnt vmcnt(0)" ::: "memory");

        const int f = tile / tiles_per_frame, rr = tile - f * tiles_per_frame;
        const int th_i = rr / p.tiles_w, tw_i = rr - th_i * p.tiles_w;
        const int oh0 = th_i * TH, ow0 = tw_i * TW;
        const size_t tile_pos = ((size_t)f * p.H + oh0) * p.W + ow0;
        char* const ybase = p.y + tile_pos * p.out_cs * 2;
        const char* const rbase = p.res + tile_pos * p.out_cs * 2;
        uint4 rq[2][4];
        auto res_fetch = [&](int j, uint4* dst) __attribute__((always_inline)) {
#pragma unroll
            for (int q = 0; q < 4; ++q) {
                const int pl = q * 8 + sl_p;
                const int ohl = TWL == 5 ? 2 * wave + j : 4 * wave + 2 * j + (pl >> 4), owl = TWL == 5 ? pl : (pl & 15);
                const bool live = oh0 + ohl < p.H && ow0 + owl < p.W && !(p.ablate & 4);
                dst[q] = *(const uint4*)(rbase + (live ? ((unsigned)(ohl * p.W + owl) * (unsigned)p.out_cs + (unsigned)sl_c) * 2u : 0u));
            }
        };
        if (p.res_mode) res_fetch(0, rq[0]);
#pragma unroll
        for (int j = 0; j < 2; ++j) {
            if (p.res_mode && j == 0) res_fetch(1, rq[1]);
#pragma unroll
            for (int i = 0; i < 2; ++i) epi_stage(est, n, khalf, i, acc[i][j]);
            __builtin_amdgcn_wave_barrier();
#pragma unroll
            for (int q = 0; q < 4; ++q) {
                const int pl = q * 8 + sl_p;
                float v[8];
                epi_load(est, pl, sl_c, v);
                const int ohl = TWL == 5 ? 2 * wave + j : 4 * wave + 2 * j + (pl >> 4), owl = TWL == 5 ? pl : (pl & 15);
                if (oh0 + ohl >= p.H || ow0 + owl >= p.W || (p.ablate & 4)) continue;
                const unsigned lpos = (unsigned)(ohl * p.W + owl);
                epi_affine(v, sc, bi);
                if (p.res_mode) epi_residual<DAT_BF16>(v, rq[j][q], 1);
                epi_relu(v, p.relu);
                epi_store<DAT_BF16>(ybase + (lpos * (unsigned)p.out_cs + (unsigned)sl_c) * 2u, v);
            }
            __builtin_amdgcn_wave_barrier();
        }
    }
#undef WS_DMA
#undef WS_MFMA0_V
#undef WS_MFMA_V
#undef WS_MFMA_A
}

struct Pw256Params {
    const char* x;
    const char* w;
    const float* scale;
    const float* bias;
    const char* res;
    char* y;
    long long npos;
    int H, W, out_cs, relu, res_mode;
    int ntiles;
    unsigned hw, w_magic;
};

__global__ __launch_bounds__(NTHREADS) __attribute__((amdgpu_waves_per_eu(1, 1))) void conv1x1_k64_c256_ws_kernel(const Pw256Params p) {
    constexpr int EPITCH = 256 * 4 + 16;
    extern __shared__ __attribute__((aligned(16))) char smem[];
    const int tid = threadIdx.x, lane = tid & 63;
    const int wave = __builtin_amdgcn_readfirstlane(tid >> 6);
    const int khalf = lane >> 5, n = lane & 31;
    char* const est = smem + wave * (32 * EPITCH);
    uint4 wa[8][4];
#pragma unroll
    for (int mb = 0; mb < 8; ++mb)
#pragma unroll
        for (int ks = 0; ks < 4; ++ks) wa[mb][ks] = *(const uint4*)(p.w + (mb * 4 + ks) * 1024 + lane * 16);
    const int sl_c = (lane & 31) * 8, sl_p = lane >> 5;
    float sc[8], bi[8];
#pragma unroll
    for (int e = 0; e < 8; ++e) {
        sc[e] = p.scale ? p.scale[sl_c + e] : 1.f;
        bi[e] = p.bias ? p.bias[sl_c + e] : 0.f;
    }
    const int nwaves = gridDim.x * 4;
    int tile = blockIdx.x * 4 + wave;
    uint4 bcur[4], bnext[4];
#define PW_LOAD(DST_, TILE_)                                                                                   \
    {                                                                                                          \
        const unsigned pos_ = min((unsigned)(TILE_) * 32u + (unsigned)n, (unsigned)p.npos - 1u);               \
        const char* src_ = p.x + (size_t)(pos_ * 128u + (unsigned)khalf * 16u);                                                   \
        _Pragma("unroll") for (int ks_ = 0; ks_ < 4; ++ks_) DST_[ks_] = *(const uint4*)(src_ + ks_ * 32);      \
    }
    if (tile < p.ntiles) PW_LOAD(bcur, tile);
    for (; tile < p.ntiles; tile += nwaves) {
        const int next = tile + nwaves;
        if (next < p.ntiles) PW_LOAD(bnext, next);
        const unsigned pos0 = (unsigned)tile * 32u;
        const unsigned f0 = pos0 / p.hw;
        uint4 rr[16];
        if (p.res_mode) {
#pragma unroll
            for (int q = 0; q < 16; ++q) {
                const unsigned pl = (unsigned)(q * 2 + sl_p);
                const unsigned pos = min(pos0 + pl, (unsigned)p.npos - 1u);
                unsigned rpos = pos;
                if (p.res_mode == 2) {
                    unsigned fr = f0, rem = pos - f0 * p.hw;
                    if (rem >= p.hw) { rem -= p.hw; ++fr; }
                    const unsigned oh = __umulhi(rem, p.w_magic), ow = rem - oh * (unsigned)p.W;
                    rpos = (fr * (unsigned)(p.H >> 1) + (oh >> 1)) * (unsigned)(p.W >> 1) + (ow >> 1);
                }
                rr[q] = *(const uint4*)(p.res + (size_t)((rpos * (unsigned)p.out_cs + (unsigned)sl_c) * 2u));
            }
        }
        f32x16_t acc[8];
#pragma unroll
        for (int mb = 0; mb < 8; ++mb)
#pragma unroll
            for (int r = 0; r < 16; ++r) acc[mb][r] = 0.f;
#pragma unroll
        for (int ks = 0; ks < 4; ++ks)
#pragma unroll
            for (int mb = 0; mb < 8; ++mb) Mma<DAT_BF16>::step(wa[mb][ks], bcur[ks], acc[mb]);
#pragma unroll
        for (int mb = 0; mb < 8; ++mb) epi_stage<EPITCH>(est, n, khalf, mb, acc[mb]);
        __builtin_amdgcn_wave_barrier();
#pragma unroll
        for (int q = 0; q < 16; ++q) {
            const int pl = q * 2 + sl_p;
            float v[8];
            epi_load<8, EPITCH>(est, pl, sl_c, v);
            const unsigned pos = pos0 + (unsigned)pl;
            epi_affine(v, sc, bi);
            if (p.res_mode) epi_residual<DAT_BF16>(v, rr[q], 1);
            epi_relu(v, p.relu);
            if (pos < (unsigned)p.npos)
                epi_store<DAT_BF16>(p.y + (size_t)((pos * (unsigned)p.out_cs + (unsigned)sl_c) * 2u), v);
        }
        __builtin_amdgcn_wave_barrier();
#pragma unroll
        for (int ks = 0; ks < 4; ++ks) bcur[ks] = bnext[ks];
    }
#undef PW_LOAD
}

struct PwLwParams {
    const char* x;
    const char* w;
    const float* scale;
    const float* bias;
    const char* res;
    const char* res2;
    char* y;
    unsigned npos;
    int Ho, Wo, H, W, stride;
    int in_cs, out_cs, cout;
    int relu, res_mode;
    int ntiles;
    unsigned how, wo_magic;
    int nsplit, mb_total;
    int xcd;
};

template <int KC, int MBW, int NPASS, int M4 = 0>
__global__ __launch_bounds__(NTHREADS) __attribute__((amdgpu_waves_per_eu(1, 1))) void conv1x1_lw_kernel(const PwLwParams p) {
    constexpr int EPITCH = 32 * 4 + 16;
    constexpr int MBP = MBW * NPASS;
    constexpr int WBYTES = KC * MBP * 4096;
    extern __shared__ __attribute__((aligned(16))) char smem[];
    const int tid = threadIdx.x, lane = tid & 63;
    const int wave = __builtin_amdgcn_readfirstlane(tid >> 6);
    const int khalf = lane >> 5, n = lane & 31;
    int part = blockIdx.x % p.nsplit, stream = blockIdx.x / p.nsplit;
    if (p.xcd) {
        const int xcd = blockIdx.x & 7, k = blockIdx.x >> 3;
        part = k % p.nsplit;
        stream = (k / p.nsplit) * 8 + xcd;
    }
    char* const wl = smem;
    float* const sbl = (float*)(smem + WBYTES);
    char* const est = smem + WBYTES + MBP * 32 * 8 + wave * (32 * EPITCH);
    const int c_part0 = part * MBP * 32;
    for (int i = tid; i < WBYTES / 16; i += NTHREADS) {
        const int frag = i >> 6, l16 = i & 63;
        const int ks = frag & 3, mbl = (frag >> 2) % MBP, kc = (frag >> 2) / MBP;
        const size_t src = ((((size_t)kc * p.mb_total + (size_t)part * MBP + mbl) * 4 + ks) * 64 + l16) * 16;
        *(uint4*)(wl + (size_t)i * 16) = *(const uint4*)(p.w + src);
    }
    for (int i = tid; i < MBP * 32; i += NTHREADS) {
        const int c = c_part0 + i;
        const bool ok = c < p.cout;
        sbl[i] = ok ? (p.scale ? p.scale[c] : 1.f) : 0.f;
        sbl[MBP * 32 + i] = (ok && p.bias) ? p.bias[c] : 0.f;
    }
    __syncthreads();
    const int sq = lane & 3, spl = lane >> 2;
    const int nwaves = (gridDim.x / p.nsplit) * 4;
    int tile = stream * 4 + wave;
    uint4 bcur[KC * 4], bnext[KC * 4];
#define LW_LOAD(DST_, TILE_)                                                                                          \
    {                                                                                                                 \
        const unsigned pos_ = min((unsigned)(TILE_) * 32u + (unsigned)n, p.npos - 1u);                                \
        unsigned ip_ = pos_;                                                                                          \
        if (p.stride == 2) {                                                                                          \
            const unsigned f_ = pos_ / p.how, rem_ = pos_ - f_ * p.how;                                               \
            const unsigned oh_ = __umulhi(rem_, p.wo_magic), ow_ = rem_ - oh_ * (unsigned)p.Wo;                       \
            ip_ = (f_ * (unsigned)p.H + 2u * oh_) * (unsigned)p.W + 2u * ow_;                                         \
        }                                                                                                             \
        const char* src_ = p.x + ((size_t)ip_ * (unsigned)p.in_cs + (unsigned)khalf * 8u) * 2u;                       \
        _Pragma("unroll") for (int i_ = 0; i_ < KC * 4; ++i_) DST_[i_] = *(const uint4*)(src_ + (i_ >> 2) * 128 + (i_ & 3) * 32); \
    }
    if (tile < p.ntiles) LW_LOAD(bcur, tile);
    for (; tile < p.ntiles; tile += nwaves) {
        const int next = tile + nwaves;
        if (next < p.ntiles) LW_LOAD(bnext, next);
        const unsigned pos0 = (unsigned)tile * 32u;
        bool live[2];
        uint4 rr[NPASS][MBW][2];
        uint4 rm[NPASS == 1 ? MBW : 1][2];
        constexpr bool m4 = M4 != 0;
        const char* rb[2];
        const char* ab[2];
#pragma unroll
        for (int r = 0; r < 2; ++r) {
            const unsigned pos = pos0 + (unsigned)(r * 16 + spl);
            live[r] = pos < p.npos;
            if (m4) {
                const unsigned pc = min(pos, p.npos - 1u);
                rb[r] = p.res + ((size_t)pc * (unsigned)p.out_cs) * 2u;
                ab[r] = p.res2 + ((size_t)pc * (unsigned)p.out_cs) * 2u;
            } else if (p.res_mode) {
                const unsigned pc = min(pos, p.npos - 1u);
                unsigned rpos = pc;
                if (p.res_mode == 2) {
                    const unsigned fr = pc / p.how, rem = pc - fr * p.how;
                    const unsigned oh = __umulhi(rem, p.wo_magic), ow = rem - oh * (unsigned)p.Wo;
                    rpos = (fr * (unsigned)(p.Ho >> 1) + (oh >> 1)) * (unsigned)(p.Wo >> 1) + (ow >> 1);
                }
                const char* rbl = p.res + ((size_t)rpos * (unsigned)p.out_cs) * 2u;
#pragma unroll
                for (int pass = 0; pass < NPASS; ++pass)
#pragma unroll
                    for (int mb = 0; mb < MBW; ++mb) {
                        const unsigned c = (unsigned)min(c_part0 + (pass * MBW + mb) * 32 + sq * 8, p.out_cs - 8);
                        rr[pass][mb][r] = *(const uint4*)(rbl + c * 2u);
                    }
            }
        }
#pragma unroll
        for (int pass = 0; pass < NPASS; ++pass) {
            if (m4) {
#pragma unroll
                for (int r = 0; r < 2; ++r)
#pragma unroll
                    for (int mb = 0; mb < MBW; ++mb) {
                        const unsigned c = (unsigned)min(c_part0 + (pass * MBW + mb) * 32 + sq * 8, p.out_cs - 8);
                        rr[0][mb][r] = *(const uint4*)(ab[r] + c * 2u);
                        if (NPASS == 1) rm[NPASS == 1 ? mb : 0][r] = *(const uint4*)(rb[r] + c * 2u);
                        else rr[NPASS - 1][mb][r] = *(const uint4*)(rb[r] + c * 2u);
                    }
            }
            f32x16_t acc[MBW];
#pragma unroll
            for (int mb = 0; mb < MBW; ++mb)
#pragma unroll
                for (int r = 0; r < 16; ++r) acc[mb][r] = 0.f;
            const char* wp = wl + (size_t)(pass * MBW) * 4096 + lane * 16;
#pragma unroll
            for (int kc = 0; kc < KC; ++kc)
#pragma unroll
                for (int ks = 0; ks < 4; ++ks)
#pragma unroll
                    for (int mb = 0; mb < MBW; ++mb) {
                        const uint4 a = *(const uint4*)(wp + ((size_t)(kc * MBP + mb) * 4 + ks) * 1024);
                        Mma<DAT_BF16>::step(a, bcur[kc * 4 + ks], acc[mb]);
                    }
#pragma unroll
            for (int mb = 0; mb < MBW; ++mb) {
                const int cl = (pass * MBW + mb) * 32 + sq * 8;
                const int c0 = c_part0 + cl;
                epi_stage<EPITCH>(est, n, khalf, 0, acc[mb]);
                __builtin_amdgcn_wave_barrier();
                const float4 s0 = *(const float4*)(sbl + cl), s1 = *(const float4*)(sbl + cl + 4);
                const float4 b0 = *(const float4*)(sbl + MBP * 32 + cl), b1 = *(const float4*)(sbl + MBP * 32 + cl + 4);
                const float sc[8] = {s0.x, s0.y, s0.z, s0.w, s1.x, s1.y, s1.z, s1.w};
                const float bi[8] = {b0.x, b0.y, b0.z, b0.w, b1.x, b1.y, b1.z, b1.w};
#pragma unroll
                for (int r = 0; r < 2; ++r) {
                    const int pl = r * 16 + spl;
                    float v[8];
                    epi_load<8, EPITCH>(est, pl, sq * 8, v);
                    epi_affine(v, sc, bi);
                    if (m4) epi_residual4<DAT_BF16>(v, rr[0][mb][r], NPASS == 1 ? rm[NPASS == 1 ? mb : 0][r] : rr[NPASS - 1][mb][r]);
                    else if (p.res_mode) epi_residual<DAT_BF16>(v, rr[pass][mb][r], 1);
                    epi_relu(v, p.relu);
                    if (live[r] && c0 < p.cout) {
                        const unsigned pos = pos0 + (unsigned)pl;
                        epi_store<DAT_BF16>(p.y + ((size_t)pos * (unsigned)p.out_cs + (unsigned)c0) * 2u, v);
                    }
                }
                __builtin_amdgcn_wave_barrier();
            }
        }
#pragma unroll
        for (int i = 0; i < KC * 4; ++i) bcur[i] = bnext[i];
    }
#undef LW_LOAD
}

struct PwKsParams {
    const char* x;
    const char* w;
    const float* scale;
    const float* bias;
    const char* res;
    const char* res2;
    char* y;
    unsigned npos;
    int Ho, Wo, H, W, stride;
    int in_cs, out_cs, cout;
    int relu, res_mode;
    int ncb;
    int kchunks, mb_total;
    unsigned how, wo_magic;
    int ablate;
    int xcd;
};

constexpr int KS_THREADS = 512;
constexpr int KS_XBYTES = 256 * 128, KS_WBYTES = 8 * 4 * 1024;

__global__ __launch_bounds__(KS_THREADS) void conv1x1_ks_kernel(const PwKsParams p) {
    extern __shared__ __attribute__((aligned(16))) char smem[];
    char* const xb = smem;
    char* const wb = smem + 3 * KS_XBYTES;
    const int tid = threadIdx.x, lane = tid & 63;
    const int wave = __builtin_amdgcn_readfirstlane(tid >> 6);
    const int khalf = lane >> 5, n = lane & 31;
    unsigned bid = blockIdx.x;
    if (p.xcd) bid = xcd_block_map(bid, gridDim.x);
    const int cb = bid % p.ncb;
    const unsigned pos0 = (bid / p.ncb) * 256u;
    const int wq = wave & 3, ph = wave >> 2;
    typedef const __attribute__((address_space(1))) void* gptr_t;
    typedef __attribute__((address_space(3))) void* lptr_t;
    const char* xsrc[4];
#pragma unroll
    for (int u = 0; u < 4; ++u) {
        const int row = wave * 32 + u * 8 + (lane >> 3);
        const int slot = (lane & 7) ^ ((row >> 1) & 7);
        const unsigned pos = min(pos0 + (unsigned)row, p.npos - 1u);
        unsigned ip = pos;
        if (p.stride == 2) {
            const unsigned f = pos / p.how, rem = pos - f * p.how;
            const unsigned oh = __umulhi(rem, p.wo_magic), ow = rem - oh * (unsigned)p.Wo;
            ip = (f * (unsigned)p.H + 2u * oh) * (unsigned)p.W + 2u * ow;
        }
        xsrc[u] = p.x + (size_t)ip * (unsigned)p.in_cs * 2u + slot * 16;
    }
    const char* wsrc = p.w + (size_t)cb * 8 * 4096 + (size_t)(wave * 4) * 1024 + lane * 16;
    const size_t wstep = (size_t)p.mb_total * 4096;
    char* const xdma = xb + wave * (32 * 128);
    char* const wdma = wb + wave * 4096;
#define KS_DMA_X(KC_, BUF_)                                                                                  \
    {                                                                                                        \
        const size_t ko_ = (size_t)min((KC_), p.kchunks - 1) * 128;       \
        _Pragma("unroll") for (int u_ = 0; u_ < 4; ++u_)                                                     \
            __builtin_amdgcn_global_load_lds((gptr_t)(xsrc[u_] + ko_), (lptr_t)(xdma + (BUF_) * KS_XBYTES + u_ * 1024), 16, 0, 0); \
    }
#define KS_DMA_W(KC_, BUF_)                                                                                  \
    {                                                                                                        \
        const char* ws_ = wsrc + (size_t)min((KC_), p.kchunks - 1) * wstep;                                  \
        _Pragma("unroll") for (int u_ = 0; u_ < 4; ++u_)                                                     \
            __builtin_amdgcn_global_load_lds((gptr_t)(ws_ + u_ * 1024), (lptr_t)(wdma + (BUF_) * KS_WBYTES + u_ * 1024), 16, 0, 0); \
    }
#define KS_COMPUTE(XBUF_, WBUF_)                                                                             \
    {                                                                                                        \
        const char* xc_ = xb + (XBUF_) * KS_XBYTES + b_base;                                                 \
        const char* wc_ = wb + (WBUF_) * KS_WBYTES + a_off;                                                  \
        _Pragma("unroll") for (int ks_ = 0; ks_ < 4; ++ks_) {                                                \
            uint4 a_[2], b_[4];                                                                              \
            _Pragma("unroll") for (int i_ = 0; i_ < 2; ++i_) a_[i_] = *(const uint4*)(wc_ + (i_ * 4 + ks_) * 1024); \
            _Pragma("unroll") for (int j_ = 0; j_ < 4; ++j_) b_[j_] = *(const uint4*)(xc_ + j_ * 4096 + b_slot[ks_]); \
            _Pragma("unroll") for (int i_ = 0; i_ < 2; ++i_)                                                 \
                _Pragma("unroll") for (int j_ = 0; j_ < 4; ++j_) Mma<DAT_BF16>::step(a_[i_], b_[j_], acc[i_][j_]); \
        }                                                                                                    \
    }
    KS_DMA_W(0, 0);
    KS_DMA_X(0, 0);
    KS_DMA_X(1, 1);
    f32x16_t acc[2][4];
#pragma unroll
    for (int i = 0; i < 2; ++i)
#pragma unroll
        for (int j = 0; j < 4; ++j)
#pragma unroll
            for (int r = 0; r < 16; ++r) acc[i][j][r] = 0.f;
    const int a_off = (2 * wq) * 4096 + lane * 16;
    const int b_base = (ph * 128 + n) * 128;
    int b_slot[4];
#pragma unroll
    for (int ks = 0; ks < 4; ++ks) b_slot[ks] = (((ks * 2 + khalf) ^ (n >> 1)) & 7) << 4;
    asm volatile("s_waitcnt vmcnt(4)" ::: "memory");
    __syncthreads();
    int xi = 0;
    for (int kc = 0; kc < p.kchunks; ++kc) {
        const int x2 = xi >= 1 ? xi - 1 : 2;
        if (!(p.ablate & 2)) KS_DMA_W(kc + 1, (kc + 1) & 1);
        if (!(p.ablate & 1)) KS_DMA_X(kc + 2, x2);
        if (!(p.ablate & 4)) KS_COMPUTE(xi, kc & 1);
        asm volatile("s_waitcnt vmcnt(4)" ::: "memory");
        __syncthreads();
        xi = xi == 2 ? 0 : xi + 1;
    }
    asm volatile("s_waitcnt vmcnt(0)" ::: "memory");
    __syncthreads();
#undef KS_DMA_X
#undef KS_DMA_W
#undef KS_COMPUTE
    char* const est = smem + wave * (32 * EPI_PITCH);
    const int sq = lane & 7, spl = lane >> 3;
    const int c0 = cb * 256 + wq * 64 + sq * 8;
    float sc[8], bi[8];
#pragma unroll
    for (int e = 0; e < 8; ++e) {
        const bool ok = c0 + e < p.cout;
        const int c = ok ? c0 + e : 0;
        sc[e] = ok ? (p.scale ? p.scale[c] : 1.f) : 0.f;
        bi[e] = (ok && p.bias) ? p.bias[c] : 0.f;
    }
    const unsigned cres = (unsigned)min(c0, p.out_cs - 8);
#pragma unroll
    for (int j = 0; j < 4; ++j) {
        const unsigned tile0 = pos0 + (unsigned)(ph * 128 + j * 32);
        uint4 rr[4], ra[4];
        if (p.res_mode) {
#pragma unroll
            for (int r = 0; r < 4; ++r) {
                const unsigned pc = min(tile0 + (unsigned)(r * 8 + spl), p.npos - 1u);
                unsigned rpos = pc;
                if (p.res_mode == 2) {
                    const unsigned fr = pc / p.how, rem = pc - fr * p.how;
                    const unsigned oh = __umulhi(rem, p.wo_magic), ow = rem - oh * (unsigned)p.Wo;
                    rpos = (fr * (unsigned)(p.Ho >> 1) + (oh >> 1)) * (unsigned)(p.Wo >> 1) + (ow >> 1);
                }
                rr[r] = *(const uint4*)(p.res + ((size_t)rpos * (unsigned)p.out_cs + cres) * 2u);
                if (p.res_mode == 4) ra[r] = *(const uint4*)(p.res2 + ((size_t)pc * (unsigned)p.out_cs + cres) * 2u);
            }
        }
#pragma unroll
        for (int i = 0; i < 2; ++i) epi_stage(est, n, khalf, i, acc[i][j]);
        __builtin_amdgcn_wave_barrier();
#pragma unroll
        for (int r = 0; r < 4; ++r) {
            const int pl = r * 8 + spl;
            float v[8];
            epi_load(est, pl, sq * 8, v);
            epi_affine(v, sc, bi);
            if (p.res_mode == 4) epi_residual4<DAT_BF16>(v, ra[r], rr[r]);
            else if (p.res_mode) epi_residual<DAT_BF16>(v, rr[r], p.res_mode);
            epi_relu(v, p.relu);
            const unsigned pos = tile0 + (unsigned)pl;
            if (pos < p.npos && c0 < p.cout)
                epi_store<DAT_BF16>(p.y + ((size_t)pos * (unsigned)p.out_cs + (unsigned)c0) * 2u, v);
        }
        __builtin_amdgcn_wave_barrier();
    }
}

struct TkParams {
    const char* x;
    const char* w;
    const float* scale;
    const float* bias;
    const char* res;
    const char* zeros;
    char* y;
    unsigned npos;
    unsigned how;
    int T, pt, kt_n;
    int in_cs, out_cs, cout;
    int relu, res_mode;
    int ncb;
    int ncc, kchunks, mb_total;
    int xcd;
};

__global__ __launch_bounds__(KS_THREADS) void conv_kt1x1_ks_kernel(const TkParams p) {
    constexpr int CB = 256;
    constexpr int NWQ = CB / 64;
    constexpr int NJ = NWQ;
    constexpr int WBYTES = CB / 32 * 4 * 1024;
    constexpr int WPIECES = CB / 64;
    extern __shared__ __attribute__((aligned(16))) char smem[];
    char* const xb = smem;
    char* const wb = smem + 3 * KS_XBYTES;
    const int tid = threadIdx.x, lane = tid & 63;
    const int wave = __builtin_amdgcn_readfirstlane(tid >> 6);
    const int khalf = lane >> 5, n = lane & 31;
    unsigned bid = blockIdx.x;
    if (p.xcd) bid = xcd_block_map(bid, gridDim.x);
    const int cb = bid % p.ncb;
    const unsigned pos0 = (bid / p.ncb) * 256u;
    const int wq = wave % NWQ, ph = wave / NWQ;
    typedef const __attribute__((address_space(1))) void* gptr_t;
    typedef __attribute__((address_space(3))) void* lptr_t;
    const char* xsrc[4];
    int tq[4];
#pragma unroll
    for (int u = 0; u < 4; ++u) {
        const int row = wave * 32 + u * 8 + (lane >> 3);
        const int slot = (lane & 7) ^ ((row >> 1) & 7);
        const unsigned pos = min(pos0 + (unsigned)row, p.npos - 1u);
        const unsigned f = pos / p.how;
        tq[u] = (int)(f % (unsigned)p.T);
        xsrc[u] = p.x + (size_t)pos * (unsigned)p.in_cs * 2u + slot * 16;
    }
    const char* wsrc = p.w + (size_t)cb * (CB / 32) * 4096 + (size_t)(wave * WPIECES) * 1024 + lane * 16;
    const size_t wstep = (size_t)p.mb_total * 4096;
    const ptrdiff_t fstep = (ptrdiff_t)p.how * p.in_cs * 2;
    char* const xdma = xb + wave * (32 * 128);
    char* const wdma = wb + wave * (WPIECES * 1024);
    int rq_t = 0, rq_c = 0;
#define TK_DMA_X(BUF_)                                                                                       \
    {                                                                                                        \
        const int kt_ = min(rq_t, p.kt_n - 1), cc_ = rq_t < p.kt_n ? rq_c : p.ncc - 1;                       \
        const int dt_ = kt_ - p.pt;                                                                          \
        const ptrdiff_t off_ = (ptrdiff_t)dt_ * fstep + cc_ * 128;                                           \
        _Pragma("unroll") for (int u_ = 0; u_ < 4; ++u_) {                                                   \
            const bool in_ = (unsigned)(tq[u_] + dt_) < (unsigned)p.T;                                       \
            const char* s_ = in_ ? xsrc[u_] + off_ : p.zeros;                                     \
            __builtin_amdgcn_global_load_lds((gptr_t)s_, (lptr_t)(xdma + (BUF_) * KS_XBYTES + u_ * 1024), 16, 0, 0); \
        }                                                                                                    \
        if (++rq_c == p.ncc) { rq_c = 0; ++rq_t; }                                                           \
    }
#define TK_DMA_W(KC_, BUF_)                                                                                  \
    {                                                                                                        \
        const char* ws_ = wsrc + (size_t)min((KC_), p.kchunks - 1) * wstep;                                  \
        _Pragma("unroll") for (int u_ = 0; u_ < WPIECES; ++u_)                                               \
            __builtin_amdgcn_global_load_lds((gptr_t)(ws_ + u_ * 1024), (lptr_t)(wdma + (BUF_) * WBYTES + u_ * 1024), 16, 0, 0); \
    }
#define TK_COMPUTE(XBUF_, WBUF_)                                                                             \
    {                                                                                                        \
        const char* xc_ = xb + (XBUF_) * KS_XBYTES + b_base;                                                 \
        const char* wc_ = wb + (WBUF_) * WBYTES + a_off;                                                     \
        _Pragma("unroll") for (int ks_ = 0; ks_ < 4; ++ks_) {                                                \
            uint4 a_[2], b_[NJ];                                                                             \
            _Pragma("unroll") for (int i_ = 0; i_ < 2; ++i_) a_[i_] = *(const uint4*)(wc_ + (i_ * 4 + ks_) * 1024); \
            _Pragma("unroll") for (int j_ = 0; j_ < NJ; ++j_) b_[j_] = *(const uint4*)(xc_ + j_ * 4096 + b_slot[ks_]); \
            _Pragma("unroll") for (int i_ = 0; i_ < 2; ++i_)                                                 \
                _Pragma("unroll") for (int j_ = 0; j_ < NJ; ++j_) Mma<DAT_BF16>::step(a_[i_], b_[j_], acc[i_][j_]); \
        }                                                                                                    \
    }
    TK_DMA_W(0, 0);
    TK_DMA_X(0);
    TK_DMA_X(1);
    f32x16_t acc[2][NJ];
#pragma unroll
    for (int i = 0; i < 2; ++i)
#pragma unroll
        for (int j = 0; j < NJ; ++j)
#pragma unroll
            for (int r = 0; r < 16; ++r) acc[i][j][r] = 0.f;
    const int a_off = (2 * wq) * 4096 + lane * 16;
    const int b_base = (ph * (32 * NJ) + n) * 128;
    int b_slot[4];
#pragma unroll
    for (int ks = 0; ks < 4; ++ks) b_slot[ks] = (((ks * 2 + khalf) ^ (n >> 1)) & 7) << 4;
    asm volatile("s_waitcnt vmcnt(4)" ::: "memory");
    __syncthreads();
    int xi = 0;
    for (int kc = 0; kc < p.kchunks; ++kc) {
        const int x2 = xi >= 1 ? xi - 1 : 2;
        TK_DMA_W(kc + 1, (kc + 1) & 1);
        TK_DMA_X(x2);
        TK_COMPUTE(xi, kc & 1);
        asm volatile("s_waitcnt vmcnt(4)" ::: "memory");
        __syncthreads();
        xi = xi == 2 ? 0 : xi + 1;
    }
    asm volatile("s_waitcnt vmcnt(0)" ::: "memory");
    __syncthreads();
#undef TK_DMA_X
#undef TK_DMA_W
#undef TK_COMPUTE
    char* const est = smem + wave * (32 * EPI_PITCH);
    const int sq = lane & 7, spl = lane >> 3;
    const int c0 = cb * CB + wq * 64 + sq * 8;
    float sc[8], bi[8];
#pragma unroll
    for (int e = 0; e < 8; ++e) {
        const bool ok = c0 + e < p.cout;
        const int c = ok ? c0 + e : 0;
        sc[e] = ok ? (p.scale ? p.scale[c] : 1.f) : 0.f;
        bi[e] = (ok && p.bias) ? p.bias[c] : 0.f;
    }
    const unsigned cres = (unsigned)min(c0, p.out_cs - 8);
#pragma unroll
    for (int j = 0; j < NJ; ++j) {
        const unsigned tile0 = pos0 + (unsigned)(ph * (32 * NJ) + j * 32);
        uint4 rr[4];
        if (p.res_mode) {
#pragma unroll
            for (int r = 0; r < 4; ++r) {
                const unsigned pc = min(tile0 + (unsigned)(r * 8 + spl), p.npos - 1u);
                rr[r] = *(const uint4*)(p.res + ((size_t)pc * (unsigned)p.out_cs + cres) * 2u);
            }
        }
#pragma unroll
        for (int i = 0; i < 2; ++i) epi_stage(est, n, khalf, i, acc[i][j]);
        __builtin_amdgcn_wave_barrier();
#pragma unroll
        for (int r = 0; r < 4; ++r) {
            const int pl = r * 8 + spl;
            float v[8];
            epi_load(est, pl, sq * 8, v);
            epi_affine(v, sc, bi);
            if (p.res_mode) epi_residual<DAT_BF16>(v, rr[r], 1);
            epi_relu(v, p.relu);
            const unsigned pos = tile0 + (unsigned)pl;
            if (pos < p.npos && c0 < p.cout)
                epi_store<DAT_BF16>(p.y + ((size_t)pos * (unsigned)p.out_cs + (unsigned)c0) * 2u, v);
        }
        __builtin_amdgcn_wave_barrier();
    }
}

template <int TWL, int R>
__global__ __launch_bounds__(NTHREADS) __attribute__((amdgpu_waves_per_eu(1, 1))) void conv3x3_bt_kernel(const ConvParams p) {
    constexpr int TW = 1 << TWL, TH = 256 >> TWL, PW = TW + 2, PH = TH + 2;
    constexpr int NPIX = PH * PW, NPIECE = (NPIX * 8 + 63) / 64, PBYTES = NPIECE * 1024, UMAX = (NPIECE + 3) / 4;
    static_assert(36 % R == 0 && PBYTES < 65536, "ring slots are static per unrolled step; 16-bit patch addresses");
    typedef unsigned u32x4_t __attribute__((ext_vector_type(4)));
    typedef const __attribute__((address_space(1))) void* gptr_t;
    typedef __attribute__((address_space(3))) void* lptr_t;
    extern __shared__ __attribute__((aligned(16))) char smem[];
    unsigned long long clk_c0 = 0, clk_r0 = 0;
    if (p.clk) { clk_c0 = __builtin_amdgcn_s_memtime(); clk_r0 = __builtin_amdgcn_s_memrealtime(); }
    const int tid = threadIdx.x, lane = tid & 63;
    const int wave = __builtin_amdgcn_readfirstlane(tid >> 6);
    const int wave_n = wave & 1, wave_p = wave >> 1;
    const int khalf = lane >> 5, n = lane & 31;

    const unsigned bid = xcd_block_map(blockIdx.x, p.nblocks);
    const int nb = bid % p.nblk_n;
    unsigned tile = bid / p.nblk_n;
    const int fc = tile % p.otn; tile /= p.otn;
    const int tw_i = tile % p.tiles_w; tile /= p.tiles_w;
    const int th_i = tile % p.tiles_h;
    const int clip = tile / p.tiles_h;
    const int f = clip * p.otn + fc;
    const int t = p.ot0 + fc;
    const int f_in = clip * p.T + t;
    const int oh0 = th_i * TH, ow0 = tw_i * TW;

    int kt_lo = 0, kt_hi = p.KT - 1;
    while (kt_lo < p.KT && (t + kt_lo - p.pt) < p.in_lo) ++kt_lo;
    while (kt_hi >= 0 && (t + kt_hi - p.pt) >= p.in_hi) --kt_hi;
    const int n_kt = kt_hi - kt_lo + 1;
    const int npat = n_kt * p.n_cchunks;
    const int kt_hi_x = kt_lo + n_kt;
    int kshift = 0;
    if (n_kt == p.KT && (DAT_KT_ROTATE)) kshift = (p.KT - (t + kt_lo - p.pt) % p.KT) % p.KT;
    int kt = kt_lo + kshift, cc = 0;
    if (kt >= kt_hi_x) kt -= n_kt;

    unsigned qp[9][2];
#pragma unroll
    for (int tp = 0; tp < 9; ++tp)
#pragma unroll
        for (int j = 0; j < 4; ++j) {
            const int r = TWL == 5 ? 4 * wave_p + j : 8 * wave_p + 2 * j + (n >> 4), c = TWL == 5 ? n : (n & 15);
            const int row = (r + tp / 3) * PW + c + tp % 3;
            const int g = (row >> 1) & 7;
            const unsigned a16 = (unsigned)(row * PPITCH) + (unsigned)(((khalf ^ (g & 1)) << 4) | ((g >> 1) << 5));
            if (j & 1) qp[tp][j >> 1] |= a16 << 16; else qp[tp][j >> 1] = a16;
        }
    const size_t wd_cc_stride = (size_t)(p.Cout_pad >> 5) * 4096;
    const size_t tap_stride = (size_t)p.n_cchunks * wd_cc_stride;
    const char* const wd_base = p.w + (size_t)(nb * 8 + wave_n * 4) * 4096;
    unsigned aoff[4];
#pragma unroll
    for (int i = 0; i < 4; ++i) aoff[i] = (unsigned)lane * 16u + (unsigned)i * 4096u;

#define BT_DMA(KT_, CC_, B_)                                                                                              \
    {                                                                                                                     \
        const int fin_ = f_in + (KT_) - p.pt;                                                                             \
        const char* xf_ = p.x + ((size_t)fin_ * p.H * p.W) * p.Cin * 2 + (size_t)(CC_) * 128;                             \
        _Pragma("unroll") for (int u_ = 0; u_ < UMAX; ++u_) {                                                             \
            const int piece_ = min(wave + 4 * u_, NPIECE - 1);                                                            \
            const int it_ = piece_ * 64 + lane, row_ = it_ >> 3;                                                          \
            const int slot_ = (it_ ^ (row_ >> 1)) & 7;                                                                    \
            const int prow_ = row_ / PW, pcol_ = row_ - prow_ * PW;                                                       \
            const int ih_ = oh0 - 1 + prow_, iw_ = ow0 - 1 + pcol_;                                                       \
            const bool ok_ = row_ < NPIX && (unsigned)ih_ < (unsigned)p.H && (unsigned)iw_ < (unsigned)p.W;               \
            const char* src_ = ok_ ? xf_ + ((size_t)(unsigned)(ih_ * p.W + iw_) * (unsigned)(p.Cin * 2) + (unsigned)(slot_ * 16)) : p.zeros; \
            __builtin_amdgcn_global_load_lds((gptr_t)src_, (lptr_t)(smem + (B_) * PBYTES + piece_ * 1024), 16, 0, 0);     \
        }                                                                                                                 \
    }
#define BT_WPATCH(KT_, CC_) (wd_base + ((size_t)((KT_) * 9) * p.n_cchunks + (CC_)) * wd_cc_stride)
#define BT_ALOAD(WP_, S_, SLOT_)                                                                                          \
    {                                                                                                                     \
        const char* wt_ = (WP_) + (size_t)((S_) / 4) * tap_stride;                                                        \
        _Pragma("unroll") for (int i_ = 0; i_ < 4; ++i_)                                                                  \
            asm volatile("global_load_dwordx4 %0, %1, %2 offset:%3" : "=v"(aq[SLOT_][i_]) : "v"(aoff[i_]), "s"(wt_), "n"(((S_) % 4) * 1024) : "memory"); \
    }
#define BT_BREAD(S_, BOFF_)                                                                                               \
    {                                                                                                                     \
        if ((S_) % 4 == 0) {                                                                                              \
            unsigned q0_ = qp[(S_) / 4][0], q1_ = qp[(S_) / 4][1];                                                        \
            asm volatile("" : "+v"(q0_), "+v"(q1_));    \
            ba[0] = (q0_ & 0xffffu) + (BOFF_); ba[1] = (q0_ >> 16) + (BOFF_);                                             \
            ba[2] = (q1_ & 0xffffu) + (BOFF_); ba[3] = (q1_ >> 16) + (BOFF_);                                             \
        }                                                                                                                 \
        _Pragma("unroll") for (int j_ = 0; j_ < 4; ++j_)                                                                  \
            asm volatile("ds_read_b128 %0, %1" : "=v"(bq[(S_) % 2][j_]) : "v"(ba[j_] ^ (unsigned)(((S_) % 4) << 5)) : "memory"); \
    }
#define BT_MFMA(ACC_, A_, B_) asm volatile(DAT_MFMA16_OP " %0, %1, %2, %0" : "+a"(ACC_) : "v"(A_), "v"(B_) : "memory")

    f32x16_t acc[4][4];
#pragma unroll
    for (int i = 0; i < 4; ++i)
#pragma unroll
        for (int j = 0; j < 4; ++j)
#pragma unroll
            for (int r = 0; r < 16; ++r) acc[i][j][r] = 0.f;
    u32x4_t aq[R][4], bq[2][4];
    unsigned ba[4] = {0, 0, 0, 0};

    if (npat > 0) {
        BT_DMA(kt, cc, 0);
        const char* wcur = BT_WPATCH(kt, cc);
        static_for(std::make_integer_sequence<int, R>{}, [&](auto ic_) __attribute__((always_inline)) {
            constexpr int s0 = decltype(ic_)::value;
            (void)&aq; (void)&aoff;
            BT_ALOAD(wcur, s0, s0);
        });
        asm volatile("s_waitcnt vmcnt(%0)" :: "n"(4 * R) : "memory");
        __syncthreads();
        int buf = 0;
        for (int pi = 0; pi < npat; ++pi, buf ^= 1) {
            int ncc = cc + 1, nkt = kt;
            if (ncc == p.n_cchunks) { ncc = 0; if (++nkt == kt_hi_x) nkt = kt_lo; }
            const bool has_next = pi + 1 < npat;
            if (has_next) BT_DMA(nkt, ncc, buf ^ 1);
            const char* wnxt = has_next ? BT_WPATCH(nkt, ncc) : wcur;
            const unsigned boff = (unsigned)buf * PBYTES;
            __builtin_amdgcn_s_setprio(1);
            BT_BREAD(0, boff);
            static_for(std::make_integer_sequence<int, 36>{}, [&](auto ic_) __attribute__((always_inline)) {
                constexpr int st = decltype(ic_)::value;
                (void)&aq; (void)&aoff; (void)&bq; (void)&ba; (void)&acc; (void)&qp;
                if (st + 1 < 36) BT_BREAD(st + 1, boff);
                if (st + 1 < 36) asm volatile("s_waitcnt lgkmcnt(4)" ::: "memory"); else asm volatile("s_waitcnt lgkmcnt(0)" ::: "memory");
                if constexpr (st < R) {
                    if (has_next) asm volatile("s_waitcnt vmcnt(%0)" :: "n"(4 * (R - 1) + UMAX) : "memory");
                    else asm volatile("s_waitcnt vmcnt(%0)" :: "n"(4 * (R - 1)) : "memory");
                } else {
                    asm volatile("s_waitcnt vmcnt(%0)" :: "n"(4 * (R - 1)) : "memory");
                }
#pragma unroll
                for (int i = 0; i < 4; ++i)
#pragma unroll
                    for (int j = 0; j < 4; ++j) BT_MFMA(acc[i][j], aq[st % R][i], bq[st % 2][j]);
                if constexpr (st + R < 36) { BT_ALOAD(wcur, st + R, st % R); } else { BT_ALOAD(wnxt, st + R - 36, st % R); }
            });
            __builtin_amdgcn_s_setprio(0);
            __syncthreads();
            kt = nkt; cc = ncc; wcur = wnxt;
        }
    }
    asm volatile("s_waitcnt vmcnt(0) lgkmcnt(0)\n\ts_nop 15\n\ts_nop 15" ::: "memory");
#undef BT_MFMA
#undef BT_BREAD
#undef BT_ALOAD
#undef BT_WPATCH
#undef BT_DMA

    constexpr int EPITCH = EPI_PITCH;
    char* const est = smem + wave * (32 * EPITCH);
    const int sl_c = (lane & 7) * 8, sl_p = lane >> 3;
    const size_t tile_pos = ((size_t)f * p.Ho + oh0) * p.Wo + ow0;
    char* const ybase = p.y + tile_pos * p.out_cs * 2;
    const char* const rbase = p.res_mode == 2 ? p.res + (size_t)f * (p.Ho >> 1) * (p.Wo >> 1) * p.out_cs * 2 : p.res + tile_pos * p.out_cs * 2;
#pragma unroll
    for (int h = 0; h < 2; ++h) {
        const int c_st = nb * 256 + wave_n * 128 + h * 64 + sl_c;
        float sc[8], bi[8];
#pragma unroll
        for (int e = 0; e < 8; ++e) {
            const bool ok = (c_st + e) < p.Cout;
            sc[e] = (p.scale && ok) ? p.scale[c_st + e] : 1.f;
            bi[e] = (p.bias && ok) ? p.bias[c_st + e] : 0.f;
        }
        uint4 rq[2][4];
        const bool res_on = p.res_mode && c_st < p.Cout;
        auto res_fetch = [&](int j, uint4* dst) __attribute__((always_inline)) {
#pragma unroll
            for (int q = 0; q < 4; ++q) {
                const int pl = q * 8 + sl_p;
                const int ohl = TWL == 5 ? 4 * wave_p + j : 8 * wave_p + 2 * j + (pl >> 4), owl = TWL == 5 ? pl : (pl & 15);
                const int oh = oh0 + ohl, ow = ow0 + owl;
                const bool live = oh < p.Ho && ow < p.Wo && !(p.ablate & 4);
                unsigned rpos = (unsigned)(ohl * p.Wo + owl);
                if (p.res_mode == 2) rpos = (unsigned)((oh >> 1) * (p.Wo >> 1) + (ow >> 1));
                dst[q] = *(const uint4*)(rbase + (live ? (rpos * (unsigned)p.out_cs + (unsigned)c_st) * 2u : 0u));
            }
        };
        if (res_on) res_fetch(0, rq[0]);
#pragma unroll
        for (int j = 0; j < 4; ++j) {
            if (res_on && j + 1 < 4) res_fetch(j + 1, rq[(j + 1) & 1]);
#pragma unroll
            for (int i = 0; i < 2; ++i)
#pragma unroll
                for (int g = 0; g < 4; ++g)
                    *(float4*)(est + n * EPITCH + (i * 32 + g * 8 + khalf * 4) * 4) =
                        make_float4(acc[2 * h + i][j][g * 4 + 0], acc[2 * h + i][j][g * 4 + 1], acc[2 * h + i][j][g * 4 + 2], acc[2 * h + i][j][g * 4 + 3]);
            __builtin_amdgcn_wave_barrier();
#pragma unroll
            for (int q = 0; q < 4; ++q) {
                const int pl = q * 8 + sl_p;
                const float4 t0 = *(const float4*)(est + pl * EPITCH + sl_c * 4);
                const float4 t1 = *(const float4*)(est + pl * EPITCH + sl_c * 4 + 16);
                float v[8] = {t0.x, t0.y, t0.z, t0.w, t1.x, t1.y, t1.z, t1.w};
                const int ohl = TWL == 5 ? 4 * wave_p + j : 8 * wave_p + 2 * j + (pl >> 4), owl = TWL == 5 ? pl : (pl & 15);
                const int oh = oh0 + ohl, ow = ow0 + owl;
                if (oh >= p.Ho || ow >= p.Wo || c_st >= p.Cout || (p.ablate & 4)) continue;
                const unsigned lpos = (unsigned)(ohl * p.Wo + owl);
#pragma unroll
                for (int e = 0; e < 8; ++e) v[e] = v[e] * sc[e] + bi[e];
                if (p.res_mode) {
                    const uint4 r = rq[j & 1][q];
                    const uint32_t ru[4] = {r.x, r.y, r.z, r.w};
#pragma unroll
                    for (int e2 = 0; e2 < 4; ++e2) {
                        v[2 * e2] += bf2f((uint16_t)(ru[e2] & 0xffff));
                        v[2 * e2 + 1] += bf2f((uint16_t)(ru[e2] >> 16));
                    }
                }
                if (p.relu) {
#pragma unroll
                    for (int e = 0; e < 8; ++e) v[e] = fmaxf(v[e], 0.f);
                }
                *(uint4*)(ybase + (lpos * (unsigned)p.out_cs + (unsigned)c_st) * 2u) =
                    make_uint4(f2bf2(v[0], v[1]), f2bf2(v[2], v[3]), f2bf2(v[4], v[5]), f2bf2(v[6], v[7]));
            }
            __builtin_amdgcn_wave_barrier();
        }
    }
    if (p.clk && threadIdx.x == 0) {
        atomicAdd(&p.clk[0], __builtin_amdgcn_s_memtime() - clk_c0);
        atomicAdd(&p.clk[1], __builtin_amdgcn_s_memrealtime() - clk_r0);
    }
}

}

namespace dat_conv {

bool ws64_eligible(const dat_ctx* ctx, const dat_conv_desc* d) {
    return ctx->dbg_ws64 && d->dtype == DAT_BF16 && d->Cin == 64 && d->Cout == 64 && d->KT == 1 && d->KH == 3 && d->KW == 3 &&
           d->stride_h == 1 && d->stride_w == 1 && d->pad_h == 1 && d->pad_w == 1 && d->pad_t == 0 && d->res_mode != 2 &&
           d->out_tn <= 0 && d->out_cstride % 8 == 0;
}

int ctx_num_cu(dat_ctx* ctx);
static long long persist_cus(dat_ctx* ctx, int mult) {
    long long n = ctx_num_cu(ctx);
    if (ctx->dbg_persist_pct > 0 && ctx->dbg_persist_pct < 100) n = std::max<long long>(mult, n * ctx->dbg_persist_pct / 100 / mult * mult);
    return n;
}

int ctx_num_cu(dat_ctx* ctx) {
    if (ctx->num_cu == 0) {
        int dev = 0, n = 0;
        if (hipGetDevice(&dev) != hipSuccess || hipDeviceGetAttribute(&n, hipDeviceAttributeMultiprocessorCount, dev) != hipSuccess) n = 0;
        ctx->num_cu = n > 0 ? n : 256;
    }
    return ctx->num_cu;
}

bool bt_eligible(const dat_ctx* ctx, const dat_conv_desc* d) {
    return ctx->dbg_bt && d->dtype == DAT_BF16 && d->Cin % 64 == 0 && cout_pad_of(d) % 256 == 0 && d->Cout % 8 == 0 && d->KH == 3 && d->KW == 3 &&
           d->stride_h == 1 && d->stride_w == 1 && d->pad_h == 1 && d->pad_w == 1 && d->out_cstride % 8 == 0;
}

int bt_tile_twl(const ConvParams& p, long long* nblocks) {
    int best = 4;
    long long best_tiles = -1;
    for (int twl = 4; twl <= 5; ++twl) {
        const long long tiles = cdiv_ll(p.Ho, 256 >> twl) * cdiv_ll(p.Wo, 1 << twl);
        if (best_tiles < 0 || tiles < best_tiles) { best_tiles = tiles; best = twl; }
    }
    *nblocks = best_tiles * p.frames * (p.Cout_pad / 256);
    return best;
}

int launch_bt(dat_ctx* ctx, hipStream_t st, ConvParams& p) {
    long long nblocks = 0;
    const int twl = bt_tile_twl(p, &nblocks);
    const int tw = 1 << twl, th = 256 >> twl;
    p.th_log2 = 8 - twl; p.tw_log2 = twl; p.tile_w = tw;
    p.tiles_h = (int)cdiv_ll(p.Ho, th); p.tiles_w = (int)cdiv_ll(p.Wo, tw);
    p.n_cchunks = p.Cin / 64;
    p.nblk_n = p.Cout_pad / 256;
    p.ksplit = 1; p.part = nullptr;
    p.ablate = ctx->dbg_ablate;
    DAT_ENFORCE(ctx, nblocks > 0 && nblocks < (1ll << 31), "conv3d: grid of %lld blocks unsupported", nblocks);
    DAT_ENFORCE(ctx, (long long)p.Ho * p.Wo * std::max(p.out_cs, p.Cout) * 4 < (1ll << 31) && (long long)p.H * p.W * p.Cin * 2 < (1ll << 32),
                "conv3d: one frame of %dx%d exceeds the 32-bit offsets of the big-tile kernel", p.H, p.W);
    p.nblocks = (unsigned)nblocks;
    const int npiece = ((th + 2) * (tw + 2) * 8 + 63) / 64;
    const size_t lds = (size_t)2 * npiece * 1024;
#define BT_LAUNCH(TWL_, R_)                                                                                            \
    {                                                                                                                  \
        if (dat_ensure_lds(ctx, (const void*)conv3x3_bt_kernel<TWL_, R_>, 160 * 1024) != DAT_OK) return DAT_ERR_LAUNCH; \
        hipLaunchKernelGGL((conv3x3_bt_kernel<TWL_, R_>), dim3(p.nblocks), dim3(NTHREADS), lds, st, p);                \
    }
    if (twl == 5) BT_LAUNCH(5, 6) else BT_LAUNCH(4, 6)
#undef BT_LAUNCH
    DAT_CHECK_LAUNCH(ctx, "conv3x3_bt");
    return DAT_OK;
}

bool pw256_eligible(const dat_ctx* ctx, const dat_conv_desc* d) {
    return ctx->dbg_ws64 && d->dtype == DAT_BF16 && d->Cin == 64 && d->Cout == 256 && d->KT == 1 && d->KH == 1 && d->KW == 1 &&
           d->stride_h == 1 && d->stride_w == 1 && d->pad_h == 0 && d->pad_w == 0 && d->pad_t == 0 && d->out_tn <= 0 &&
           d->out_cstride % 8 == 0 &&
           (long long)d->H * d->W >= 32 && (long long)d->H * d->W * d->W < (1ll << 32) &&
           (long long)d->frames * d->H * d->W * std::max(d->out_cstride, 64) * 2 < (1ll << 32);
}

int launch_pw256(dat_ctx* ctx, hipStream_t st, const ConvParams& cp) {
    Pw256Params p;
    p.x = cp.x; p.w = cp.w; p.scale = cp.scale; p.bias = cp.bias; p.res = cp.res; p.y = cp.y;
    p.npos = (long long)cp.frames * cp.H * cp.W;
    p.H = cp.H; p.W = cp.W; p.out_cs = cp.out_cs; p.relu = cp.relu; p.res_mode = cp.res_mode;
    const long long ntiles = cdiv_ll(p.npos, 32);
    DAT_ENFORCE(ctx, ntiles > 0 && ntiles < (1ll << 31), "conv3d: %lld wave tiles unsupported", ntiles);
    p.ntiles = (int)ntiles;
    p.hw = (unsigned)(cp.H * cp.W);
    p.w_magic = cp.W == 1 ? 0u : (unsigned)((0x100000000ull + (unsigned)cp.W - 1) / (unsigned)cp.W);
    const unsigned grid = (unsigned)std::min<long long>(cdiv_ll(ntiles, 4), persist_cus(ctx, 8));
    const size_t lds = (size_t)4 * 32 * (256 * 4 + 16);
    if (dat_ensure_lds(ctx, (const void*)conv1x1_k64_c256_ws_kernel, 160 * 1024) != DAT_OK) return DAT_ERR_LAUNCH;
    hipLaunchKernelGGL(conv1x1_k64_c256_ws_kernel, dim3(grid), dim3(NTHREADS), lds, st, p);
    DAT_CHECK_LAUNCH(ctx, "conv1x1_k64_c256_ws");
    return DAT_OK;
}

static int lw_nsplit(const dat_conv_desc* d) {
    const long long wbytes = (long long)d->Cin * cout_pad_of(d) * 2;
    int ns = 1;
    while (wbytes / ns > 128 * 1024) ns *= 2;
    return ns;
}

bool pwlw_eligible(dat_ctx* ctx, const dat_conv_desc* d) {
    if (!(ctx->dbg_pwlw && d->dtype == DAT_BF16 && d->KT == 1 && d->KH == 1 && d->KW == 1 && d->pad_h == 0 && d->pad_w == 0 && d->pad_t == 0 &&
          d->out_tn <= 0 && d->stride_h == d->stride_w && (d->stride_h == 1 || d->stride_h == 2)))
        return false;
    const int kc = d->Cin / 64;
    if (d->Cin % 64 || !(kc == 1 || kc == 2 || kc == 4 || kc == 8)) return false;
    const int ns = lw_nsplit(d), mbt = cout_pad_of(d) / 32;
    if (ns > 4 || mbt % ns) return false;
    const int mbp = mbt / ns;
    if (!(mbp == 2 || mbp == 4 || mbp == 8 || mbp == 16) || (kc == 8 && mbp > 4)) return false;
    if ((long long)kc * mbp * 4096 + mbp * 256 + 4 * 32 * 144 > 160 * 1024) return false;
    if (d->out_cstride % 8 || d->out_cstride < d->Cout) return false;
    int Ho, Wo;
    dat_conv3d_out_shape(d, &Ho, &Wo);
    const long long npos = (long long)d->frames * Ho * Wo;
    if ((long long)Ho * Wo < 32 || (long long)Ho * Wo * Wo >= (1ll << 32)) return false;
    if (npos >= (1ll << 31) || (long long)d->frames * d->H * d->W >= (1ll << 31)) return false;
    return npos / 32 >= 2ll * 4 * ctx_num_cu(ctx) / ns;
}

template <int KC, int MBW, int NPASS>
static int launch_pwlw_t(dat_ctx* ctx, hipStream_t st, const PwLwParams& p, unsigned grid, size_t lds) {
    if (p.res_mode == 4) {
        if (dat_ensure_lds(ctx, (const void*)conv1x1_lw_kernel<KC, MBW, NPASS, 1>, 160 * 1024) != DAT_OK) return DAT_ERR_LAUNCH;
        hipLaunchKernelGGL((conv1x1_lw_kernel<KC, MBW, NPASS, 1>), dim3(grid), dim3(NTHREADS), lds, st, p);
        return DAT_OK;
    }
    if (dat_ensure_lds(ctx, (const void*)conv1x1_lw_kernel<KC, MBW, NPASS>, 160 * 1024) != DAT_OK) return DAT_ERR_LAUNCH;
    hipLaunchKernelGGL((conv1x1_lw_kernel<KC, MBW, NPASS>), dim3(grid), dim3(NTHREADS), lds, st, p);
    return DAT_OK;
}

int launch_pwlw(dat_ctx* ctx, hipStream_t st, const ConvParams& cp, const dat_conv_desc* d) {
    PwLwParams p;
    p.x = cp.x; p.w = cp.w; p.scale = cp.scale; p.bias = cp.bias; p.res = cp.res; p.y = cp.y; p.res2 = cp.res2;
    p.npos = (unsigned)((long long)cp.frames * cp.Ho * cp.Wo);
    p.Ho = cp.Ho; p.Wo = cp.Wo; p.H = cp.H; p.W = cp.W; p.stride = cp.sh;
    p.in_cs = cp.Cin; p.out_cs = cp.out_cs; p.cout = cp.Cout; p.relu = cp.relu; p.res_mode = cp.res_mode;
    p.ntiles = (int)cdiv_ll(p.npos, 32);
    p.how = (unsigned)(cp.Ho * cp.Wo);
    p.wo_magic = cp.Wo == 1 ? 0u : (unsigned)((0x100000000ull + (unsigned)cp.Wo - 1) / (unsigned)cp.Wo);
    p.nsplit = lw_nsplit(d); p.mb_total = cp.Cout_pad / 32;
    const int kc = cp.Cin / 64, mbp = p.mb_total / p.nsplit;
    const int mbw = kc <= 4 ? std::min(mbp, 8) : std::min(mbp, 4), npass = mbp / mbw;
    const long long per_part = std::min<long long>(cdiv_ll(p.ntiles, 4), persist_cus(ctx, 8 * p.nsplit) / p.nsplit);
    const unsigned grid = (unsigned)(per_part * p.nsplit);
    p.xcd = ctx->dbg_pw_xcd && p.nsplit > 1 && grid % (8u * (unsigned)p.nsplit) == 0;
    const size_t lds = (size_t)kc * mbp * 4096 + (size_t)mbp * 32 * 8 + 4 * 32 * (32 * 4 + 16);
    DAT_ENFORCE(ctx, lds <= 160 * 1024, "conv1x1_lw: %zu bytes of LDS", lds);
    int rc = DAT_ERR_UNSUPPORTED;
#define LW_CASE(KC_, MBW_, NP_) if (kc == KC_ && mbw == MBW_ && npass == NP_) rc = launch_pwlw_t<KC_, MBW_, NP_>(ctx, st, p, grid, lds);
    LW_CASE(1, 2, 1) LW_CASE(1, 4, 1) LW_CASE(1, 8, 1) LW_CASE(1, 8, 2)
    LW_CASE(2, 2, 1) LW_CASE(2, 4, 1) LW_CASE(2, 8, 1) LW_CASE(2, 8, 2)
    LW_CASE(4, 2, 1) LW_CASE(4, 4, 1) LW_CASE(4, 8, 1)
    LW_CASE(8, 2, 1) LW_CASE(8, 4, 1)
#undef LW_CASE
    if (rc != DAT_OK) DAT_FAIL(ctx, rc, "conv1x1_lw: no instantiation for K chunks %d x %d row blocks x %d passes", kc, mbw, npass);
    DAT_CHECK_LAUNCH(ctx, "conv1x1_lw");
    return DAT_OK;
}

bool pwks_eligible(dat_ctx* ctx, const dat_conv_desc* d) {
    if (!(ctx->dbg_pwks > 0 && d->dtype == DAT_BF16 && d->KT == 1 && d->KH == 1 && d->KW == 1 && d->pad_h == 0 && d->pad_w == 0 && d->pad_t == 0 &&
          d->out_tn <= 0 && d->stride_h == d->stride_w && (d->stride_h == 1 || d->stride_h == 2)))
        return false;
    if (d->Cin % 64 || d->Cin / 64 < ctx->dbg_pwks || cout_pad_of(d) % 256) return false;
    if (d->out_cstride % 8 || d->out_cstride < d->Cout || d->out_cstride < 8) return false;
    int Ho, Wo;
    dat_conv3d_out_shape(d, &Ho, &Wo);
    const long long npos = (long long)d->frames * Ho * Wo;
    if ((long long)Ho * Wo < 1 || (long long)Ho * Wo * Wo >= (1ll << 32)) return false;
    if (npos >= (1ll << 31) || (long long)d->frames * d->H * d->W >= (1ll << 31)) return false;
    const long long blocks = cdiv_ll(npos, 256) * (cout_pad_of(d) / 256);
    return npos >= 256 && blocks * 4 >= 3ll * ctx_num_cu(ctx);
}

int launch_pwks(dat_ctx* ctx, hipStream_t st, const ConvParams& cp) {
    PwKsParams p;
    p.x = cp.x; p.w = cp.w; p.scale = cp.scale; p.bias = cp.bias; p.res = cp.res; p.y = cp.y; p.res2 = cp.res2;
    p.npos = (unsigned)((long long)cp.frames * cp.Ho * cp.Wo);
    p.Ho = cp.Ho; p.Wo = cp.Wo; p.H = cp.H; p.W = cp.W; p.stride = cp.sh;
    p.in_cs = cp.Cin; p.out_cs = cp.out_cs; p.cout = cp.Cout; p.relu = cp.relu; p.res_mode = cp.res_mode;
    p.ncb = cp.Cout_pad / 256; p.kchunks = cp.Cin / 64; p.mb_total = cp.Cout_pad / 32;
    p.how = (unsigned)(cp.Ho * cp.Wo);
    p.wo_magic = cp.Wo == 1 ? 0u : (unsigned)((0x100000000ull + (unsigned)cp.Wo - 1) / (unsigned)cp.Wo);
    p.ablate = ctx->dbg_ablate;
    p.xcd = ctx->dbg_pw_xcd && p.ncb > 1;
    const long long blocks = cdiv_ll(p.npos, 256) * p.ncb;
    DAT_ENFORCE(ctx, blocks > 0 && blocks < (1ll << 31), "conv1x1_ks: grid of %lld blocks unsupported", blocks);
    const size_t lds = (size_t)3 * KS_XBYTES + 2 * KS_WBYTES;
    if (dat_ensure_lds(ctx, (const void*)conv1x1_ks_kernel, 160 * 1024) != DAT_OK) return DAT_ERR_LAUNCH;
    hipLaunchKernelGGL(conv1x1_ks_kernel, dim3((unsigned)blocks), dim3(KS_THREADS), lds, st, p);
    DAT_CHECK_LAUNCH(ctx, "conv1x1_ks");
    return DAT_OK;
}

bool tks_eligible(dat_ctx* ctx, const dat_conv_desc* d) {
    if (!(ctx->dbg_temporal > 0 && DAT_H16_FORMAT == 0 && d->dtype == DAT_BF16 && d->KT > 1 && d->KH == 1 && d->KW == 1 && d->pad_h == 0 &&
          d->pad_w == 0 && d->pad_t * 2 + 1 == d->KT && d->out_tn <= 0 && d->in_tn <= 0 && d->stride_h == 1 && d->stride_w == 1 &&
          (d->res_mode == 0 || d->res_mode == 1)))
        return false;
    if (d->Cin % 64 || cout_pad_of(d) % 256) return false;
    if (d->out_cstride % 8 || d->out_cstride < d->Cout || d->out_cstride < 8) return false;
    const long long how = (long long)d->H * d->W, npos = (long long)d->frames * how;
    if (how < 1 || npos >= (1ll << 31) || npos * d->Cin >= (1ll << 40)) return false;
    const long long blocks = cdiv_ll(npos, 256) * (cout_pad_of(d) / 256);
    return npos >= 256 && (ctx->dbg_temporal >= 2 || blocks * 4 >= 3ll * ctx_num_cu(ctx));
}

int launch_tks(dat_ctx* ctx, hipStream_t st, const ConvParams& cp) {
    TkParams p;
    p.x = cp.x; p.w = cp.w; p.scale = cp.scale; p.bias = cp.bias; p.res = cp.res; p.zeros = cp.zeros; p.y = cp.y;
    p.npos = (unsigned)((long long)cp.frames * cp.Ho * cp.Wo);
    p.how = (unsigned)(cp.Ho * cp.Wo);
    p.T = cp.T; p.pt = cp.pt; p.kt_n = cp.KT;
    p.in_cs = cp.Cin; p.out_cs = cp.out_cs; p.cout = cp.Cout; p.relu = cp.relu; p.res_mode = cp.res_mode;
    p.ncb = cp.Cout_pad / 256; p.ncc = cp.Cin / 64; p.kchunks = cp.KT * p.ncc; p.mb_total = cp.Cout_pad / 32;
    p.xcd = ctx->dbg_pw_xcd && p.ncb > 1;
    const long long blocks = cdiv_ll(p.npos, 256) * p.ncb;
    DAT_ENFORCE(ctx, blocks > 0 && blocks < (1ll << 31), "conv_kt1x1_ks: grid of %lld blocks unsupported", blocks);
    DAT_ENFORCE(ctx, cp.Ho == cp.H && cp.Wo == cp.W && cp.res_mode <= 1 && cp.Cout_pad % 256 == 0 && cp.zeros,
                "conv_kt1x1_ks: unsupported call");
    const size_t lds = (size_t)3 * KS_XBYTES + 2 * KS_WBYTES;
    if (dat_ensure_lds(ctx, (const void*)conv_kt1x1_ks_kernel, 160 * 1024) != DAT_OK) return DAT_ERR_LAUNCH;
    hipLaunchKernelGGL(conv_kt1x1_ks_kernel, dim3((unsigned)blocks), dim3(KS_THREADS), lds, st, p);
    DAT_CHECK_LAUNCH(ctx, "conv_kt1x1_ks");
    return DAT_OK;
}

int launch_ws64(dat_ctx* ctx, hipStream_t st, const ConvParams& cp) {
    Ws64Params p;
    p.x = cp.x; p.w = cp.w; p.scale = cp.scale; p.bias = cp.bias; p.res = cp.res; p.y = cp.y; p.zeros = cp.zeros;
    p.frames = cp.frames; p.H = cp.H; p.W = cp.W; p.out_cs = cp.out_cs; p.relu = cp.relu; p.res_mode = cp.res_mode;
    p.ablate = ctx->dbg_ablate;
    DAT_ENFORCE(ctx, (long long)p.H * p.W * std::max(p.out_cs, 64) * 2 < (1ll << 31), "conv3d: frame of %dx%d exceeds 32-bit offsets", p.H, p.W);
    int best_twl = 4;
    long long best_rounds = -1, best_tiles = 0;
    for (int twl = 4; twl <= 5; ++twl) {
        if ((ctx->dbg_ws64 == 2 && twl != 5) || (ctx->dbg_ws64 == 3 && twl != 4)) continue;
        const int tw = 1 << twl, th = 256 >> twl;
        const long long tiles = (long long)p.frames * cdiv_ll(p.H, th) * cdiv_ll(p.W, tw);
        const long long rounds = cdiv_ll(tiles, ctx_num_cu(ctx));
        if (best_rounds < 0 || rounds < best_rounds) { best_rounds = rounds; best_twl = twl; best_tiles = tiles; }
    }
    const int tw = 1 << best_twl, th = 256 >> best_twl;
    p.tiles_h = (int)cdiv_ll(p.H, th); p.tiles_w = (int)cdiv_ll(p.W, tw);
    DAT_ENFORCE(ctx, best_tiles > 0 && best_tiles < (1ll << 31), "conv3d: %lld tiles unsupported", best_tiles);
    p.ntiles = (int)best_tiles;
    const int npiece = ((th + 2) * (tw + 2) * 8 + 63) / 64;
    const size_t lds = (size_t)2 * npiece * 1024 + EPI_SLICES_BYTES;
    const unsigned grid = (unsigned)std::min<long long>(best_tiles, persist_cus(ctx, 8));
    if (best_twl == 5) {
        if (dat_ensure_lds(ctx, (const void*)conv3x3_c64_ws_kernel<5>, 160 * 1024) != DAT_OK) return DAT_ERR_LAUNCH;
        hipLaunchKernelGGL(conv3x3_c64_ws_kernel<5>, dim3(grid), dim3(NTHREADS), lds, st, p);
    } else {
        if (dat_ensure_lds(ctx, (const void*)conv3x3_c64_ws_kernel<4>, 160 * 1024) != DAT_OK) return DAT_ERR_LAUNCH;
        hipLaunchKernelGGL(conv3x3_c64_ws_kernel<4>, dim3(grid), dim3(NTHREADS), lds, st, p);
    }
    DAT_CHECK_LAUNCH(ctx, "conv3x3_c64_ws");
    return DAT_OK;
}

}
```

### detectandtrack_amd/csrc/dat_common.h

```cpp
#pragma once
#include <hip/hip_runtime.h>
#include <stdint.h>
#include <stdio.h>
#include <string.h>

#include <string>
#include <unordered_set>
#include <vector>

#include "../../include/dat_hip.h"

struct dat_ctx {
    int device;
    std::string last_error;
    int prof_enabled;
    hipEvent_t* prof_ev;
    int prof_cap, prof_n;
    double* prof_flops;
    int* prof_tag;
    void* ws;
    size_t ws_bytes;
    std::vector<void*> ws_retired;
    int ws_generation;
    void* zeros;
    void* util_stream;
    void* pinned;
    int force_bp, force_ks;
    int dbg_ablate;
    int dbg_linear;
    int dbg_order;
    int dbg_persist_pct;
    int dbg_bt_min;
    int dbg_bt;
    int dbg_ws64;
    int dbg_pwks;
    int dbg_pwlw;
    int dbg_wgrad_direct;
    int dbg_ablate_wgrad;
    int dbg_wgrad_sub;
    int dbg_pw_xcd;
    int dbg_wgrad_ks;
    int dbg_wgrad_pw;
    int dbg_kps_sep;
    int dbg_ws_poison;
    int dbg_roi_fold;
    int num_cu;
    int dbg_ntap;
    int dbg_temporal;
    std::unordered_set<const void*> lds_attr_done;
};

static inline int dat_ensure_lds(dat_ctx* ctx, const void* kern, int bytes) {
    if (ctx->lds_attr_done.count(kern)) return DAT_OK;
    if (hipFuncSetAttribute(kern, hipFuncAttributeMaxDynamicSharedMemorySize, bytes) != hipSuccess) {
        (void)hipGetLastError();
        ctx->last_error = "hipFuncSetAttribute(MaxDynamicSharedMemorySize) failed";
        return DAT_ERR_LAUNCH;
    }
    ctx->lds_attr_done.insert(kern);
    return DAT_OK;
}

#define DAT_FAIL(ctx, code, ...)                                  \
    do {                                                          \
        char _b[512];                                             \
        snprintf(_b, sizeof(_b), __VA_ARGS__);                    \
        if (ctx) (ctx)->last_error = _b;                          \
        return (code);                                            \
    } while (0)

#define DAT_CHECK_LAUNCH(ctx, what)                                                         \
    do {                                                                                    \
        hipError_t _e = hipGetLastError();                                                  \
        if (_e != hipSuccess) DAT_FAIL(ctx, DAT_ERR_LAUNCH, "%s: %s", what, hipGetErrorString(_e)); \
    } while (0)

#define DAT_ENFORCE(ctx, cond, ...)                               \
    do {                                                          \
        if (!(cond)) DAT_FAIL(ctx, DAT_ERR_ARG, __VA_ARGS__);     \
    } while (0)

typedef __attribute__((ext_vector_type(8))) __bf16 bf16x8_t;
typedef __attribute__((ext_vector_type(16))) float f32x16_t;
typedef __attribute__((ext_vector_type(4))) float f32x4_t;

#ifdef DAT_H16_IS_FP16
typedef __attribute__((ext_vector_type(8))) _Float16 h16x8_t;
typedef _Float16 dat_h16x2_t __attribute__((ext_vector_type(2)));
typedef float dat_f32x2_t __attribute__((ext_vector_type(2)));
__device__ __forceinline__ uint16_t f2bf(float f) { return __builtin_bit_cast(uint16_t, (_Float16)f); }
__device__ __forceinline__ uint32_t f2bf2(float lo, float hi) {
    const dat_f32x2_t v = {lo, hi};
    return __builtin_bit_cast(uint32_t, __builtin_convertvector(v, dat_h16x2_t));
}
__device__ __forceinline__ float bf2f(uint16_t h) { return (float)__builtin_bit_cast(_Float16, h); }
#define DAT_MFMA16(A_, B_, C_) __builtin_amdgcn_mfma_f32_32x32x16_f16(__builtin_bit_cast(h16x8_t, A_), __builtin_bit_cast(h16x8_t, B_), C_, 0, 0, 0)
#define DAT_MFMA16_OP "v_mfma_f32_32x32x16_f16"
#define DAT_H16_FORMAT 1
#else
typedef __bf16 dat_bf16x2_t __attribute__((ext_vector_type(2)));
typedef float dat_f32x2_t __attribute__((ext_vector_type(2)));
__device__ __forceinline__ uint16_t f2bf(float f) { return __builtin_bit_cast(uint16_t, (__bf16)f); }
__device__ __forceinline__ uint32_t f2bf2(float lo, float hi) {
    const dat_f32x2_t v = {lo, hi};
    return __builtin_bit_cast(uint32_t, __builtin_convertvector(v, dat_bf16x2_t));
}
__device__ __forceinline__ float bf2f(uint16_t h) { return __uint_as_float(((uint32_t)h) << 16); }
#define DAT_MFMA16(A_, B_, C_) __builtin_amdgcn_mfma_f32_32x32x16_bf16(__builtin_bit_cast(bf16x8_t, A_), __builtin_bit_cast(bf16x8_t, B_), C_, 0, 0, 0)
#define DAT_MFMA16_OP "v_mfma_f32_32x32x16_bf16"
#define DAT_H16_FORMAT 0
#endif

template <int DT> struct ElemOf;
template <> struct ElemOf<DAT_F32> {
    typedef float type;
    static constexpr int size = 4;
    __device__ static __forceinline__ float ld(const void* p, size_t i) { return ((const float*)p)[i]; }
    __device__ static __forceinline__ void st(void* p, size_t i, float v) { ((float*)p)[i] = v; }
};
template <> struct ElemOf<DAT_BF16> {
    typedef uint16_t type;
    static constexpr int size = 2;
    __device__ static __forceinline__ float ld(const void* p, size_t i) { return bf2f(((const uint16_t*)p)[i]); }
    __device__ static __forceinline__ void st(void* p, size_t i, float v) { ((uint16_t*)p)[i] = f2bf(v); }
};

template <typename T, int N>
__device__ __forceinline__ T dat_pick(const T (&a)[N], int i) {
    T r = a[0];
#pragma unroll
    for (int k = 1; k < N; ++k)
        if (i == k) r = a[k];
    return r;
}

int dat_ensure_ws(dat_ctx* ctx, size_t bytes);

static inline int dat_esize(int dtype) { return dtype == DAT_BF16 ? 2 : 4; }
static inline long long cdiv_ll(long long a, long long b) { return (a + b - 1) / b; }
```

Before: 248.8 clips/s.

## Use 16x16x32 MFMA tiles for bf16 dense 3x3 conv kernels

Adds an MF template variant of the implicit-GEMM and bt 3x3 conv kernels that issues v_mfma_f32_16x16x32 instead of 32x32x16. To match the new fragment shape it changes the LDS patch swizzle, the weight fragment offsets, the accumulator types and the epilogue staging. The variant is on by default through DAT_CONV_MFMA and applies to bf16 128-channel dense 3x3 convs. The bt kernel's weight ring depth drops from 6 to 3. The aim is better MFMA issue efficiency and register pressure, at the cost of twice as many MFMA instructions and different LDS access patterns.

```diff
diff --git a/detectandtrack_amd/csrc/c_api.hip b/detectandtrack_amd/csrc/c_api.hip
--- a/detectandtrack_amd/csrc/c_api.hip
+++ b/detectandtrack_amd/csrc/c_api.hip
@@ -65,6 +65,7 @@
         c->dbg_persist_pct = env_int("DAT_PERSIST_PCT", 100);
         c->dbg_bt_min = env_int("DAT_CONV_BT_MIN", 390);
         c->dbg_bt = env_int("DAT_CONV_BT", 1);
+        c->dbg_mfma = env_int("DAT_CONV_MFMA", 1) == 1;
         c->dbg_roi_fold = env_int("DAT_ROI_BWD_FOLD", 1);
         c->dbg_ws_poison = env_int("DAT_WS_POISON", 0);
         c->num_cu = 0;
diff --git a/detectandtrack_amd/csrc/conv3d_igemm.hip b/detectandtrack_amd/csrc/conv3d_igemm.hip
--- a/detectandtrack_amd/csrc/conv3d_igemm.hip
+++ b/detectandtrack_amd/csrc/conv3d_igemm.hip
@@ -5,9 +5,10 @@
 namespace {
 
 template <int BP, int NTAP> struct MinWaves { static constexpr int value = (NTAP > 0 && NTAP != 10 && BP == 128) ? 3 : 2; };
-template <int DT, int BN, int BP, int WAVES_N, int ONE, int NTAP, int ODT>
+template <int DT, int BN, int BP, int WAVES_N, int ONE, int NTAP, int ODT, int MF = 0>
 __global__ __launch_bounds__(NTHREADS, (MinWaves<BP, NTAP>::value)) void conv3d_igemm_kernel(const ConvParams p) {
     static_assert(ONE == 1, "see the comment above");
+    static_assert(!MF || (DT == DAT_BF16 && ODT == DAT_BF16 && BN == 128 && NTAP == 9), "the 16x16x32 shape exists for the bf16 128-channel dense 3x3 variants");
     constexpr int ES = ElemOf<DT>::size;
     constexpr int OES = ElemOf<ODT>::size;
     constexpr int CK = Mma<DT>::CK;
@@ -17,6 +18,8 @@
     constexpr int MT = WN / 32;
     constexpr int PT = WP / 32;
     static_assert(MT >= 1 && PT >= 1, "tile too small");
+    constexpr int MTX = MF ? 2 * MT : MT, PTX = MF ? 2 * PT : PT;
+    typedef std::conditional_t<MF != 0, f32x4_t, f32x16_t> acc_t;
 
 #ifdef DAT_CONV_TRACE
     const unsigned long long tr_k0 = __builtin_amdgcn_s_memtime();
@@ -64,22 +67,22 @@
     const int ih0 = oh0 * p.sh - p.ph;
     const int iw0 = ow0 * p.sw - p.pw;
 
-    int rowbase[PT];
-#pragma unroll
-    for (int j = 0; j < PT; ++j) {
-        const int pos = wave_p * WP + j * 32 + (lane & 31);
+    int rowbase[PTX];
+#pragma unroll
+    for (int j = 0; j < PTX; ++j) {
+        const int pos = wave_p * WP + (MF ? j * 16 + (lane & 15) : j * 32 + (lane & 31));
         const int ohl = pos >> p.tw_log2, owl = pos & (TW - 1);
         rowbase[j] = ohl * p.rsh * p.PW + owl * p.rsw;
     }
     const int khalf = lane >> 5;
 
-    f32x16_t acc[MT][PT];
-#pragma unroll
-    for (int i = 0; i < MT; ++i)
-#pragma unroll
-        for (int j = 0; j < PT; ++j)
-#pragma unroll
-            for (int r = 0; r < 16; ++r) acc[i][j][r] = 0.f;
+    acc_t acc[MTX][PTX];
+#pragma unroll
+    for (int i = 0; i < MTX; ++i)
+#pragma unroll
+        for (int j = 0; j < PTX; ++j)
+#pragma unroll
+            for (int r = 0; r < (MF ? 4 : 16); ++r) acc[i][j][r] = 0.f;
 
     int kt_lo = 0, kt_hi = p.KT - 1;
     while (kt_lo < p.KT && (t + kt_lo - p.pt) < p.in_lo) ++kt_lo;
@@ -114,22 +117,21 @@
         int kt = kt_lo + pi_lo / p.n_cchunks + kshift, cc = pi_lo % p.n_cchunks;
         if (kt >= kt_hi_x) kt -= n_kt;
         constexpr bool PACK16 = NTAP != 10;
-        constexpr int NQ = PACK16 ? (PT + 1) / 2 : PT;
+        constexpr int NQ = PACK16 ? (PTX + 1) / 2 : PTX;
         unsigned qp[NT][NQ];
 #pragma unroll
         for (int tp = 0; tp < NT; ++tp)
 #pragma unroll
-            for (int j = 0; j < PT; ++j) {
+            for (int j = 0; j < PTX; ++j) {
                 int row = rowbase[j] + p.tab_rowoff[tp];
                 if (p.lin_w > 0) {
-                    const int gpos = ow0 + wave_p * WP + j * 32 + (lane & 31);
+                    const int gpos = ow0 + wave_p * WP + (MF ? j * 16 + (lane & 15) : j * 32 + (lane & 31));
                     const int rem = gpos % (p.lin_h * p.lin_w);
                     const int y = rem / p.lin_w, x = rem - y * p.lin_w;
                     const int yy = y + tp / p.KW - p.KH / 2, xx = x + tp % p.KW - p.KW / 2;
                     if ((unsigned)yy >= (unsigned)p.lin_h || (unsigned)xx >= (unsigned)p.lin_w) row = p.lin_zero_row;
                 }
-                const int g = (row >> 1) & 7;
-                const unsigned a16 = (unsigned)(row * PPITCH) + (unsigned)(((khalf ^ (g & 1)) << 4) | ((g >> 1) << 5));
+                const unsigned a16 = patch_frag_addr<MF>(row, MF ? lane >> 4 : khalf);
                 if (!PACK16) qp[tp][j] = a16;
                 else if (j & 1) qp[tp][j >> 1] |= a16 << 16;
                 else qp[tp][j >> 1] = a16;
@@ -143,7 +145,7 @@
             int off = -2;
             if (c < nchunks && it < npatch_items) {
                 const int row = it >> 3;
-                const int slot = (it ^ (row >> 1)) & 7;
+                const int slot = patch_src_slot<MF>(it);
                 const int prow = p.pw_magic ? (int)__umulhi((unsigned)row, p.pw_magic) : row, pcol = row - prow * p.PW;
                 const int ih = ih0 + p.tab_dy[0] + prow * p.psh, iw = iw0 + p.tab_dx[0] + pcol * p.psw;
                 off = (ih >= 0 && ih < p.H && iw >= 0 && iw < p.W && row != p.lin_zero_row) ? (int)((unsigned)(ih * p.W + iw) * (unsigned)(p.Cin * ES) + (unsigned)(slot * 16)) : -1;
@@ -152,13 +154,15 @@
         }
         const size_t tap_stride = (size_t)p.n_cchunks * wd_cc_stride;
         const char* const wd_base = p.w + (size_t)((n0 + wave_n * WN) >> 5) * 4096;
-        const unsigned lane16 = (unsigned)lane * 16u;
+        constexpr int NKS = MF ? 2 : 4;
+        const unsigned lane16 = MF ? 16u * (((unsigned)lane & 15u) + 32u * (((unsigned)lane >> 4) & 1u)) + ((unsigned)lane >> 5) * 1024u : (unsigned)lane * 16u;
+#define W_OFF(I_, KS_) (MF ? ((I_) & 1) * 256 + ((I_) >> 1) * 4096 + (KS_) * 2048 : (I_) * 4096 + (KS_) * 1024)
         const char* wcur = wd_base + ((size_t)(kt * ntap) * p.n_cchunks + cc) * wd_cc_stride;
-        uint4 wa[MT][4];
-#pragma unroll
-        for (int i = 0; i < MT; ++i)
-#pragma unroll
-            for (int ks = 0; ks < 4; ++ks) wa[i][ks] = *(const uint4*)(wcur + i * 4096 + ks * 1024 + lane16);
+        uint4 wa[MTX][NKS];
+#pragma unroll
+        for (int i = 0; i < MTX; ++i)
+#pragma unroll
+            for (int ks = 0; ks < NKS; ++ks) wa[i][ks] = *(const uint4*)(wcur + W_OFF(i, ks) + lane16);
         const int npat = pi_hi - pi_lo;
         for (int pi = 0; pi < npat; ++pi) {
             if (!((p.ablate & 1) && pi > 0) && !(p.x3 && pi > 0 && cc % 3 == 1)) {
@@ -167,8 +171,10 @@
                 const char* xbase = p.x + ((size_t)fin * p.H * p.W) * p.Cin * ES + (size_t)(p.x3 ? (cc / 3) * 2 + (cc % 3 == 2) : cc) * CK * ES;
 #pragma unroll
                 for (int u = 0; u < MAXCH; ++u) {
-                    if (poff[u] != -2) {
-                        const char* src = poff[u] >= 0 ? xbase + (unsigned)poff[u] : p.zeros;
+                    int po = poff[u];
+                    if constexpr (MF != 0) asm volatile("" : "+v"(po));
+                    if (po != -2) {
+                        const char* src = po >= 0 ? xbase + (unsigned)po : p.zeros;
                         P_DMA(src, patch + (wave + 4 * u) * 1024);
                     }
                 }
@@ -179,43 +185,56 @@
             if (ncc == p.n_cchunks) { ncc = 0; if (++nkt == kt_hi_x) nkt = kt_lo; }
             const char* wnextpatch = (pi + 1 < npat) ? wd_base + ((size_t)(nkt * ntap) * p.n_cchunks + ncc) * wd_cc_stride : wcur;
             __builtin_amdgcn_s_setprio(1);
-            uint4 b[2][PT];
-            unsigned qa[PT];
+            constexpr int BF = MF ? (PT >= 4 ? 2 : PT) : PT;
+            constexpr int UPS = PTX / BF, NU = NKS * UPS;
+            uint4 b[2][BF];
+            unsigned qa[MF ? 1 : PT];
+#define Q_ADDR(TP_, J_) (!PACK16 ? qp[TP_][(J_) % NQ] : ((J_) & 1) ? (qp[TP_][((J_) >> 1) % NQ] >> 16) : (qp[TP_][((J_) >> 1) % NQ] & 0xffffu))
 #pragma unroll
             for (int jj = 0; jj < NQ; ++jj) asm volatile("" : "+v"(qp[0][jj]));
-#pragma unroll
-            for (int j = 0; j < PT; ++j) qa[j] = !PACK16 ? qp[0][j % NQ] : (j & 1) ? (qp[0][(j >> 1) % NQ] >> 16) : (qp[0][(j >> 1) % NQ] & 0xffffu);
-#pragma unroll
-            for (int j = 0; j < PT; ++j) b[0][j] = *(const uint4*)(patch + qa[j]);
+            if constexpr (!MF) {
+#pragma unroll
+                for (int j = 0; j < PT; ++j) qa[j] = Q_ADDR(0, j);
+            }
+#pragma unroll
+            for (int j = 0; j < BF; ++j) b[0][j] = *(const uint4*)(patch + (MF ? Q_ADDR(0, j) : qa[j % (MF ? 1 : PT)]));
 #pragma unroll
             for (int tp = 0; tp < NT; ++tp) {
                 const char* wnext = (tp + 1 < NT) ? wcur + (size_t)(tp + 1) * tap_stride : wnextpatch;
 #pragma unroll
-                for (int ks = 0; ks < 4; ++ks) {
-                    const int cur = ks & 1, nxt = cur ^ 1;
-                    if (ks < 3) {
-#pragma unroll
-                        for (int j = 0; j < PT; ++j) b[nxt][j] = *(const uint4*)(patch + (qa[j] ^ (unsigned)((ks + 1) << 5)));
+                for (int u = 0; u < NU; ++u) {
+                    const int cur = u & 1, nxt = cur ^ 1;
+                    const int ks = u / UPS, jb = (u % UPS) * BF;
+                    if (u + 1 < NU) {
+                        const int nks = (u + 1) / UPS, njb = ((u + 1) % UPS) * BF;
+#pragma unroll
+                        for (int j = 0; j < BF; ++j)
+                            b[nxt][j] = *(const uint4*)(patch + ((MF ? Q_ADDR(tp, njb + j) : qa[j % (MF ? 1 : PT)]) ^ (unsigned)(nks << (MF ? 6 : 5))));
                     } else if (tp + 1 < NT) {
 #pragma unroll
                         for (int jj = 0; jj < NQ; ++jj) asm volatile("" : "+v"(qp[tp + 1 < NT ? tp + 1 : tp][jj]));
-#pragma unroll
-                        for (int j = 0; j < PT; ++j) {
-                            const unsigned w2 = qp[tp + 1 < NT ? tp + 1 : tp][(PACK16 ? j >> 1 : j) % NQ];
-                            qa[j] = !PACK16 ? w2 : (j & 1) ? (w2 >> 16) : (w2 & 0xffffu);
+                        if constexpr (!MF) {
+#pragma unroll
+                            for (int j = 0; j < PT; ++j) qa[j] = Q_ADDR(tp + 1 < NT ? tp + 1 : tp, j);
                         }
 #pragma unroll
-                        for (int j = 0; j < PT; ++j) b[nxt][j] = *(const uint4*)(patch + qa[j]);
+                        for (int j = 0; j < BF; ++j) b[nxt][j] = *(const uint4*)(patch + (MF ? Q_ADDR(tp + 1 < NT ? tp + 1 : tp, j) : qa[j % (MF ? 1 : PT)]));
                     }
 #pragma unroll
-                    for (int i = 0; i < MT; ++i)
-#pragma unroll
-                        for (int j = 0; j < PT; ++j) Mma<DT>::step(wa[i][ks], b[cur][j], acc[i][j]);
-#pragma unroll
-                    for (int i = 0; i < MT; ++i) wa[i][ks] = *(const uint4*)(wnext + i * 4096 + ks * 1024 + lane16);
+                    for (int i = 0; i < MTX; ++i)
+#pragma unroll
+                        for (int j = 0; j < BF; ++j) {
+                            if constexpr (MF) acc[i][jb + j] = DAT_MFMA16K32(wa[i][ks], b[cur][j], acc[i][jb + j]);
+                            else Mma<DT>::step(wa[i][ks], b[cur][j], acc[i][j]);
+                        }
+                    if ((u + 1) % UPS == 0) {
+#pragma unroll
+                        for (int i = 0; i < MTX; ++i) wa[i][ks] = *(const uint4*)(wnext + W_OFF(i, ks) + lane16);
+                    }
                     __builtin_amdgcn_sched_barrier(0);
                 }
             }
+#undef Q_ADDR
             __builtin_amdgcn_s_setprio(0);
             wcur = wnextpatch;
             cc = ncc; kt = nkt;
@@ -223,6 +242,7 @@
       }
     } else
     if (total > 0) {
+        static_assert(!MF, "the table-driven loop runs 32x32x16 only");
         const int kt_hi_x = kt_lo + n_kt;
         int kshift = 0;
         if (n_kt == p.KT && (DAT_KT_ROTATE)) kshift = (p.KT - (t + kt_lo - p.pt) % p.KT) % p.KT;
@@ -328,6 +348,7 @@
         tr_k1 = __builtin_amdgcn_s_memtime();
 #endif
     }
+#undef W_OFF
 #undef WD_PTR
 #undef P_COMMIT
 #undef P_DMA
@@ -377,12 +398,19 @@
 #pragma unroll
     for (int j = 0; j < PT; ++j) {
         if (res_pre && j + 1 < PT) res_fetch(j + 1, rq[(j + 1) & 1]);
-#pragma unroll
-        for (int i = 0; i < MT; ++i)
-#pragma unroll
-            for (int g = 0; g < 4; ++g)
-                *(float4*)(est + (lane & 31) * EPI_PITCH + (i * 32 + g * 8 + khalf * 4) * 4) =
-                    make_float4(acc[i][j][g * 4 + 0], acc[i][j][g * 4 + 1], acc[i][j][g * 4 + 2], acc[i][j][g * 4 + 3]);
+        if constexpr (MF) {
+#pragma unroll
+            for (int i = 0; i < MTX; ++i)
+#pragma unroll
+                for (int jl = 0; jl < 2; ++jl) epi_stage16(est, lane, i, jl, acc[i][(2 * j + jl) % PTX]);
+        } else {
+#pragma unroll
+            for (int i = 0; i < MT; ++i)
+#pragma unroll
+                for (int g = 0; g < 4; ++g)
+                    *(float4*)(est + (lane & 31) * EPI_PITCH + (i * 32 + g * 8 + khalf * 4) * 4) =
+                        make_float4(acc[i][j][g * 4 + 0], acc[i][j][g * 4 + 1], acc[i][j][g * 4 + 2], acc[i][j][g * 4 + 3]);
+        }
         __builtin_amdgcn_wave_barrier();
 #pragma unroll
         for (int q = 0; q < NQ; ++q) {
@@ -632,7 +660,7 @@
 
 namespace {
 
-template <int DT, int BN, int BP, int WAVES_N, int NTAP, int ODT>
+template <int DT, int BN, int BP, int WAVES_N, int NTAP, int ODT, int MF = 0>
 int launch_conv(dat_ctx* ctx, hipStream_t st, ConvParams& p, int bp_log2, int ksplit, bool linear = false) {
     TileChoice tc = choose_tile(p.Ho, p.Wo, bp_log2, p.sh, p.sw, p.KH, p.KW);
     p.lin_h = p.lin_w = 0;
@@ -716,7 +744,7 @@
     if (lds < EPI_SLICES_BYTES) lds = EPI_SLICES_BYTES;
     DAT_ENFORCE(ctx, lds <= 160 * 1024, "conv3d: LDS patch of %zu bytes exceeds 160 KiB (tile %dx%d, stride %dx%d)", lds,
                 th, tw, p.sh, p.sw);
-    auto kern = conv3d_igemm_kernel<DT, BN, BP, WAVES_N, 1, NTAP, ODT>;
+    auto kern = conv3d_igemm_kernel<DT, BN, BP, WAVES_N, 1, NTAP, ODT, MF>;
     if (NTAP > 0) {
         DAT_ENFORCE(ctx, p.tab_n == (NTAP == 10 ? 9 : NTAP) && p.tab_new == 1u &&
                              (((size_t)p.PH * p.PW * 8 + 63) >> 6) <= (size_t)4 * patch_pieces_per_wave(NTAP, BP) && (NTAP == 10 || (size_t)p.PH * p.PW * PPITCH < 65536),
@@ -922,7 +950,9 @@
 #define DAT_CONV_LAUNCH(DT_, BN_, WN_, ODT_) (ntapv == 10 ? launch_conv<DT_, BN_, 128, WN_, 10, ODT_>(ctx, st, p, 7, ksplit) : ntapv == 9 ? (big ? launch_conv<DT_, BN_, 256, WN_, 9, ODT_>(ctx, st, p, 8, ksplit, lin) : launch_conv<DT_, BN_, 128, WN_, 9, ODT_>(ctx, st, p, 7, ksplit, lin)) \
                             : ntapv == 1 ? (big ? launch_conv<DT_, BN_, 256, WN_, 1, ODT_>(ctx, st, p, 8, ksplit) : launch_conv<DT_, BN_, 128, WN_, 1, ODT_>(ctx, st, p, 7, ksplit)) \
                             : (big ? launch_conv<DT_, BN_, 256, WN_, 0, ODT_>(ctx, st, p, 8, ksplit) : launch_conv<DT_, BN_, 128, WN_, 0, ODT_>(ctx, st, p, 7, ksplit)))
-        if (x3) rc = small_n ? DAT_CONV_LAUNCH(DAT_BF16, 64, 1, DAT_F32) : DAT_CONV_LAUNCH(DAT_BF16, 128, 2, DAT_F32);
+        if (ctx->dbg_mfma && ntapv == 9 && !x3 && !small_n && d->dtype == DAT_BF16)
+            rc = big ? launch_conv<DAT_BF16, 128, 256, 2, 9, DAT_BF16, 1>(ctx, st, p, 8, ksplit, lin) : launch_conv<DAT_BF16, 128, 128, 2, 9, DAT_BF16, 1>(ctx, st, p, 7, ksplit, lin);
+        else if (x3) rc = small_n ? DAT_CONV_LAUNCH(DAT_BF16, 64, 1, DAT_F32) : DAT_CONV_LAUNCH(DAT_BF16, 128, 2, DAT_F32);
         else if (small_n) rc = d->dtype == DAT_BF16 ? DAT_CONV_LAUNCH(DAT_BF16, 64, 1, DAT_BF16) : DAT_CONV_LAUNCH(DAT_F32, 64, 1, DAT_F32);
         else rc = d->dtype == DAT_BF16 ? DAT_CONV_LAUNCH(DAT_BF16, 128, 2, DAT_BF16) : DAT_CONV_LAUNCH(DAT_F32, 128, 2, DAT_F32);
 #undef DAT_CONV_LAUNCH
diff --git a/detectandtrack_amd/csrc/conv_epilogue.h b/detectandtrack_amd/csrc/conv_epilogue.h
--- a/detectandtrack_amd/csrc/conv_epilogue.h
+++ b/detectandtrack_amd/csrc/conv_epilogue.h
@@ -17,6 +17,11 @@
 #pragma unroll
     for (int g = 0; g < 4; ++g)
         *(float4*)(est + row * PITCH + (i * 32 + g * 8 + khalf * 4) * 4) = make_float4(acc[g * 4 + 0], acc[g * 4 + 1], acc[g * 4 + 2], acc[g * 4 + 3]);
+}
+
+template <int PITCH = EPI_PITCH>
+__device__ __forceinline__ void epi_stage16(char* est, int lane, int i16, int jl, const f32x4_t& acc) {
+    *(float4*)(est + (jl * 16 + (lane & 15)) * PITCH + (i16 * 16 + (lane >> 4) * 4) * 4) = make_float4(acc[0], acc[1], acc[2], acc[3]);
 }
 
 template <int CPL, int PITCH = EPI_PITCH>
diff --git a/detectandtrack_amd/csrc/conv_internal.h b/detectandtrack_amd/csrc/conv_internal.h
--- a/detectandtrack_amd/csrc/conv_internal.h
+++ b/detectandtrack_amd/csrc/conv_internal.h
@@ -88,6 +88,17 @@
 
 namespace dat_conv __attribute__((visibility("hidden"))) {
 
+template <int MF>
+__device__ __forceinline__ int patch_swz(int row) { return MF ? ((row >> 1) & 3) << 1 : (row >> 1) & 7; }
+template <int MF>
+__device__ __forceinline__ int patch_src_slot(int it) { const int row = it >> 3; return MF ? (it & 7) ^ patch_swz<1>(row) : (it ^ (row >> 1)) & 7; }
+template <int MF>
+__device__ __forceinline__ unsigned patch_frag_addr(int row, int kg) {
+    if (MF) return (unsigned)(row * PPITCH) + (unsigned)((kg ^ patch_swz<1>(row)) << 4);
+    const int g = (row >> 1) & 7;
+    return (unsigned)(row * PPITCH) + (unsigned)(((kg ^ (g & 1)) << 4) | ((g >> 1) << 5));
+}
+
 template <int... I, class F>
 __device__ __forceinline__ void static_for(std::integer_sequence<int, I...>, F&& f) {
     (f(std::integral_constant<int, I>{}), ...);
diff --git a/detectandtrack_amd/csrc/conv_special.hip b/detectandtrack_amd/csrc/conv_special.hip
--- a/detectandtrack_amd/csrc/conv_special.hip
+++ b/detectandtrack_amd/csrc/conv_special.hip
@@ -761,11 +761,13 @@
     }
 }
 
-template <int TWL, int R>
+template <int TWL, int R, int MF>
 __global__ __launch_bounds__(NTHREADS) __attribute__((amdgpu_waves_per_eu(1, 1))) void conv3x3_bt_kernel(const ConvParams p) {
     constexpr int TW = 1 << TWL, TH = 256 >> TWL, PW = TW + 2, PH = TH + 2;
     constexpr int NPIX = PH * PW, NPIECE = (NPIX * 8 + 63) / 64, PBYTES = NPIECE * 1024, UMAX = (NPIECE + 3) / 4;
-    static_assert(36 % R == 0 && PBYTES < 65536, "ring slots are static per unrolled step; 16-bit patch addresses");
+    constexpr int NSTEP = MF ? 18 : 36, APS = MF ? 8 : 4;
+    static_assert(NSTEP % R == 0 && PBYTES < 65536, "ring slots are static per unrolled step; 16-bit patch addresses");
+    static_assert(APS * R + UMAX < 64, "vmcnt is a 6-bit counter");
     typedef unsigned u32x4_t __attribute__((ext_vector_type(4)));
     typedef const __attribute__((address_space(1))) void* gptr_t;
     typedef __attribute__((address_space(3))) void* lptr_t;
@@ -800,23 +802,31 @@
     int kt = kt_lo + kshift, cc = 0;
     if (kt >= kt_hi_x) kt -= n_kt;
 
-    unsigned qp[9][2];
+    constexpr int NJ = MF ? 8 : 4;
+    unsigned qp[9][NJ / 2];
 #pragma unroll
     for (int tp = 0; tp < 9; ++tp)
 #pragma unroll
-        for (int j = 0; j < 4; ++j) {
-            const int r = TWL == 5 ? 4 * wave_p + j : 8 * wave_p + 2 * j + (n >> 4), c = TWL == 5 ? n : (n & 15);
+        for (int j = 0; j < NJ; ++j) {
+            const int pos = wave_p * 128 + (MF ? j * 16 + (lane & 15) : j * 32 + n);
+            const int r = pos >> TWL, c = pos & (TW - 1);
             const int row = (r + tp / 3) * PW + c + tp % 3;
-            const int g = (row >> 1) & 7;
-            const unsigned a16 = (unsigned)(row * PPITCH) + (unsigned)(((khalf ^ (g & 1)) << 4) | ((g >> 1) << 5));
+            const unsigned a16 = patch_frag_addr<MF>(row, MF ? lane >> 4 : khalf);
             if (j & 1) qp[tp][j >> 1] |= a16 << 16; else qp[tp][j >> 1] = a16;
         }
     const size_t wd_cc_stride = (size_t)(p.Cout_pad >> 5) * 4096;
     const size_t tap_stride = (size_t)p.n_cchunks * wd_cc_stride;
     const char* const wd_base = p.w + (size_t)(nb * 8 + wave_n * 4) * 4096;
-    unsigned aoff[4];
-#pragma unroll
-    for (int i = 0; i < 4; ++i) aoff[i] = (unsigned)lane * 16u + (unsigned)i * 4096u;
+    unsigned aoff[APS];
+#pragma unroll
+    for (int i = 0; i < APS; ++i) {
+        if (MF) {
+            const unsigned kg = (unsigned)lane >> 4;
+            aoff[i] = 16u * ((unsigned)((i & 1) << 4) + ((unsigned)lane & 15u) + 32u * (kg & 1u)) + (kg >> 1) * 1024u + (unsigned)(i >> 1) * 4096u;
+        } else {
+            aoff[i] = (unsigned)lane * 16u + (unsigned)i * 4096u;
+        }
+    }
 
 #define BT_DMA(KT_, CC_, B_)                                                                                              \
     {                                                                                                                     \
@@ -825,7 +835,7 @@
         _Pragma("unroll") for (int u_ = 0; u_ < UMAX; ++u_) {                                                             \
             const int piece_ = min(wave + 4 * u_, NPIECE - 1);                                                            \
             const int it_ = piece_ * 64 + lane, row_ = it_ >> 3;                                                          \
-            const int slot_ = (it_ ^ (row_ >> 1)) & 7;                                                                    \
+            const int slot_ = patch_src_slot<MF>(it_);                                                                    \
             const int prow_ = row_ / PW, pcol_ = row_ - prow_ * PW;                                                       \
             const int ih_ = oh0 - 1 + prow_, iw_ = ow0 - 1 + pcol_;                                                       \
             const bool ok_ = row_ < NPIX && (unsigned)ih_ < (unsigned)p.H && (unsigned)iw_ < (unsigned)p.W;               \
@@ -834,34 +844,46 @@
         }                                                                                                                 \
     }
 #define BT_WPATCH(KT_, CC_) (wd_base + ((size_t)((KT_) * 9) * p.n_cchunks + (CC_)) * wd_cc_stride)
+    constexpr int SPT = NSTEP / 9;
 #define BT_ALOAD(WP_, S_, SLOT_)                                                                                          \
     {                                                                                                                     \
-        const char* wt_ = (WP_) + (size_t)((S_) / 4) * tap_stride;                                                        \
-        _Pragma("unroll") for (int i_ = 0; i_ < 4; ++i_)                                                                  \
-            asm volatile("global_load_dwordx4 %0, %1, %2 offset:%3" : "=v"(aq[SLOT_][i_]) : "v"(aoff[i_]), "s"(wt_), "n"(((S_) % 4) * 1024) : "memory"); \
-    }
-#define BT_BREAD(S_, BOFF_)                                                                                               \
+        const char* wt_ = (WP_) + (size_t)((S_) / SPT) * tap_stride;                                                      \
+        _Pragma("unroll") for (int i_ = 0; i_ < APS; ++i_)                                                                \
+            asm volatile("global_load_dwordx4 %0, %1, %2 offset:%3" : "=v"(aq[SLOT_][i_]) : "v"(aoff[i_]), "s"(wt_), "n"(((S_) % SPT) * (4096 / SPT)) : "memory"); \
+    }
+#define BT_BREAD(U_, BOFF_)                                                                                               \
     {                                                                                                                     \
-        if ((S_) % 4 == 0) {                                                                                              \
-            unsigned q0_ = qp[(S_) / 4][0], q1_ = qp[(S_) / 4][1];                                                        \
+        if ((U_) % 4 == 0) {                                                                                              \
+            unsigned q0_ = qp[(U_) / 4][0], q1_ = qp[(U_) / 4][1], q2_ = qp[(U_) / 4][NJ / 2 - 2], q3_ = qp[(U_) / 4][NJ / 2 - 1]; \
             asm volatile("" : "+v"(q0_), "+v"(q1_));    \
             ba[0] = (q0_ & 0xffffu) + (BOFF_); ba[1] = (q0_ >> 16) + (BOFF_);                                             \
             ba[2] = (q1_ & 0xffffu) + (BOFF_); ba[3] = (q1_ >> 16) + (BOFF_);                                             \
+            if constexpr (MF != 0) {                                                                                      \
+                asm volatile("" : "+v"(q2_), "+v"(q3_));                                                                  \
+                ba[NJ - 4] = (q2_ & 0xffffu) + (BOFF_); ba[NJ - 3] = (q2_ >> 16) + (BOFF_);                               \
+                ba[NJ - 2] = (q3_ & 0xffffu) + (BOFF_); ba[NJ - 1] = (q3_ >> 16) + (BOFF_);                               \
+            }                                                                                                             \
         }                                                                                                                 \
         _Pragma("unroll") for (int j_ = 0; j_ < 4; ++j_)                                                                  \
-            asm volatile("ds_read_b128 %0, %1" : "=v"(bq[(S_) % 2][j_]) : "v"(ba[j_] ^ (unsigned)(((S_) % 4) << 5)) : "memory"); \
-    }
-#define BT_MFMA(ACC_, A_, B_) asm volatile(DAT_MFMA16_OP " %0, %1, %2, %0" : "+a"(ACC_) : "v"(A_), "v"(B_) : "memory")
-
-    f32x16_t acc[4][4];
-#pragma unroll
-    for (int i = 0; i < 4; ++i)
-#pragma unroll
-        for (int j = 0; j < 4; ++j)
-#pragma unroll
-            for (int r = 0; r < 16; ++r) acc[i][j][r] = 0.f;
-    u32x4_t aq[R][4], bq[2][4];
-    unsigned ba[4] = {0, 0, 0, 0};
+            asm volatile("ds_read_b128 %0, %1" : "=v"(bq[(U_) % 2][j_])                                                   \
+                         : "v"(ba[(MF ? ((U_) % 2) * 4 : 0) + j_] ^ (unsigned)(MF ? (((U_) / 2) % 2) << 6 : ((U_) % 4) << 5)) : "memory"); \
+    }
+#define BT_MFMA(ACC_, A_, B_)                                                                                             \
+    {                                                                                                                     \
+        if constexpr (MF) asm volatile(DAT_MFMA16K32_OP " %0, %1, %2, %0" : "+a"(ACC_) : "v"(A_), "v"(B_) : "memory");    \
+        else asm volatile(DAT_MFMA16_OP " %0, %1, %2, %0" : "+a"(ACC_) : "v"(A_), "v"(B_) : "memory");                    \
+    }
+
+    typedef std::conditional_t<MF != 0, f32x4_t, f32x16_t> acc_t;
+    acc_t acc[APS][NJ];
+#pragma unroll
+    for (int i = 0; i < APS; ++i)
+#pragma unroll
+        for (int j = 0; j < NJ; ++j)
+#pragma unroll
+            for (int r = 0; r < (MF ? 4 : 16); ++r) acc[i][j][r] = 0.f;
+    u32x4_t aq[R][APS], bq[2][4];
+    unsigned ba[NJ] = {};
 
     if (npat > 0) {
         BT_DMA(kt, cc, 0);
@@ -871,7 +893,7 @@
             (void)&aq; (void)&aoff;
             BT_ALOAD(wcur, s0, s0);
         });
-        asm volatile("s_waitcnt vmcnt(%0)" :: "n"(4 * R) : "memory");
+        asm volatile("s_waitcnt vmcnt(%0)" :: "n"(APS * R) : "memory");
         __syncthreads();
         int buf = 0;
         for (int pi = 0; pi < npat; ++pi, buf ^= 1) {
@@ -884,21 +906,27 @@
             __builtin_amdgcn_s_setprio(1);
             BT_BREAD(0, boff);
             static_for(std::make_integer_sequence<int, 36>{}, [&](auto ic_) __attribute__((always_inline)) {
-                constexpr int st = decltype(ic_)::value;
+                constexpr int un = decltype(ic_)::value;
+                constexpr int st = MF ? un / 2 : un, jb = MF ? (un % 2) * 4 : 0;
+                constexpr bool opens = !MF || un % 2 == 0, ends = !MF || un % 2 == 1;
                 (void)&aq; (void)&aoff; (void)&bq; (void)&ba; (void)&acc; (void)&qp;
-                if (st + 1 < 36) BT_BREAD(st + 1, boff);
-                if (st + 1 < 36) asm volatile("s_waitcnt lgkmcnt(4)" ::: "memory"); else asm volatile("s_waitcnt lgkmcnt(0)" ::: "memory");
-                if constexpr (st < R) {
-                    if (has_next) asm volatile("s_waitcnt vmcnt(%0)" :: "n"(4 * (R - 1) + UMAX) : "memory");
-                    else asm volatile("s_waitcnt vmcnt(%0)" :: "n"(4 * (R - 1)) : "memory");
-                } else {
-                    asm volatile("s_waitcnt vmcnt(%0)" :: "n"(4 * (R - 1)) : "memory");
+                if (un + 1 < 36) BT_BREAD(un + 1, boff);
+                if (un + 1 < 36) asm volatile("s_waitcnt lgkmcnt(4)" ::: "memory"); else asm volatile("s_waitcnt lgkmcnt(0)" ::: "memory");
+                if constexpr (opens) {
+                    if constexpr (st < R) {
+                        if (has_next) asm volatile("s_waitcnt vmcnt(%0)" :: "n"(APS * (R - 1) + UMAX) : "memory");
+                        else asm volatile("s_waitcnt vmcnt(%0)" :: "n"(APS * (R - 1)) : "memory");
+                    } else {
+                        asm volatile("s_waitcnt vmcnt(%0)" :: "n"(APS * (R - 1)) : "memory");
+                    }
                 }
 #pragma unroll
-                for (int i = 0; i < 4; ++i)
-#pragma unroll
-                    for (int j = 0; j < 4; ++j) BT_MFMA(acc[i][j], aq[st % R][i], bq[st % 2][j]);
-                if constexpr (st + R < 36) { BT_ALOAD(wcur, st + R, st % R); } else { BT_ALOAD(wnxt, st + R - 36, st % R); }
+                for (int i = 0; i < APS; ++i)
+#pragma unroll
+                    for (int j = 0; j < 4; ++j) BT_MFMA(acc[i][jb + j], aq[st % R][i], bq[un % 2][j]);
+                if constexpr (ends) {
+                    if constexpr (st + R < NSTEP) { BT_ALOAD(wcur, st + R, st % R); } else { BT_ALOAD(wnxt, st + R - NSTEP, st % R); }
+                }
             });
             __builtin_amdgcn_s_setprio(0);
             __syncthreads();
@@ -946,12 +974,19 @@
 #pragma unroll
         for (int j = 0; j < 4; ++j) {
             if (res_on && j + 1 < 4) res_fetch(j + 1, rq[(j + 1) & 1]);
-#pragma unroll
-            for (int i = 0; i < 2; ++i)
-#pragma unroll
-                for (int g = 0; g < 4; ++g)
-                    *(float4*)(est + n * EPITCH + (i * 32 + g * 8 + khalf * 4) * 4) =
-                        make_float4(acc[2 * h + i][j][g * 4 + 0], acc[2 * h + i][j][g * 4 + 1], acc[2 * h + i][j][g * 4 + 2], acc[2 * h + i][j][g * 4 + 3]);
+            if constexpr (MF) {
+#pragma unroll
+                for (int i = 0; i < 4; ++i)
+#pragma unroll
+                    for (int jl = 0; jl < 2; ++jl) epi_stage16(est, lane, i, jl, acc[(4 * h + i) % APS][(2 * j + jl) % NJ]);
+            } else {
+#pragma unroll
+                for (int i = 0; i < 2; ++i)
+#pragma unroll
+                    for (int g = 0; g < 4; ++g)
+                        *(float4*)(est + n * EPITCH + (i * 32 + g * 8 + khalf * 4) * 4) =
+                            make_float4(acc[2 * h + i][j][g * 4 + 0], acc[2 * h + i][j][g * 4 + 1], acc[2 * h + i][j][g * 4 + 2], acc[2 * h + i][j][g * 4 + 3]);
+            }
             __builtin_amdgcn_wave_barrier();
 #pragma unroll
             for (int q = 0; q < 4; ++q) {
@@ -1048,12 +1083,13 @@
     p.nblocks = (unsigned)nblocks;
     const int npiece = ((th + 2) * (tw + 2) * 8 + 63) / 64;
     const size_t lds = (size_t)2 * npiece * 1024;
-#define BT_LAUNCH(TWL_, R_)                                                                                            \
+#define BT_LAUNCH(TWL_, R_, MF_)                                                                                           \
     {                                                                                                                  \
-        if (dat_ensure_lds(ctx, (const void*)conv3x3_bt_kernel<TWL_, R_>, 160 * 1024) != DAT_OK) return DAT_ERR_LAUNCH; \
-        hipLaunchKernelGGL((conv3x3_bt_kernel<TWL_, R_>), dim3(p.nblocks), dim3(NTHREADS), lds, st, p);                \
-    }
-    if (twl == 5) BT_LAUNCH(5, 6) else BT_LAUNCH(4, 6)
+        if (dat_ensure_lds(ctx, (const void*)conv3x3_bt_kernel<TWL_, R_, MF_>, 160 * 1024) != DAT_OK) return DAT_ERR_LAUNCH; \
+        hipLaunchKernelGGL((conv3x3_bt_kernel<TWL_, R_, MF_>), dim3(p.nblocks), dim3(NTHREADS), lds, st, p);           \
+    }
+    if (ctx->dbg_mfma) { if (twl == 5) BT_LAUNCH(5, 3, 1) else BT_LAUNCH(4, 3, 1) }
+    else if (twl == 5) BT_LAUNCH(5, 6, 0) else BT_LAUNCH(4, 6, 0)
 #undef BT_LAUNCH
     DAT_CHECK_LAUNCH(ctx, "conv3x3_bt");
     return DAT_OK;
diff --git a/detectandtrack_amd/csrc/dat_common.h b/detectandtrack_amd/csrc/dat_common.h
--- a/detectandtrack_amd/csrc/dat_common.h
+++ b/detectandtrack_amd/csrc/dat_common.h
@@ -46,6 +46,7 @@
     int dbg_roi_fold;
     int num_cu;
     int dbg_ntap;
+    int dbg_mfma;
     int dbg_temporal;
     std::unordered_set<const void*> lds_attr_done;
 };
@@ -96,6 +97,8 @@
 __device__ __forceinline__ float bf2f(uint16_t h) { return (float)__builtin_bit_cast(_Float16, h); }
 #define DAT_MFMA16(A_, B_, C_) __builtin_amdgcn_mfma_f32_32x32x16_f16(__builtin_bit_cast(h16x8_t, A_), __builtin_bit_cast(h16x8_t, B_), C_, 0, 0, 0)
 #define DAT_MFMA16_OP "v_mfma_f32_32x32x16_f16"
+#define DAT_MFMA16K32(A_, B_, C_) __builtin_amdgcn_mfma_f32_16x16x32_f16(__builtin_bit_cast(h16x8_t, A_), __builtin_bit_cast(h16x8_t, B_), C_, 0, 0, 0)
+#define DAT_MFMA16K32_OP "v_mfma_f32_16x16x32_f16"
 #define DAT_H16_FORMAT 1
 #else
 typedef __bf16 dat_bf16x2_t __attribute__((ext_vector_type(2)));
@@ -108,6 +111,8 @@
 __device__ __forceinline__ float bf2f(uint16_t h) { return __uint_as_float(((uint32_t)h) << 16); }
 #define DAT_MFMA16(A_, B_, C_) __builtin_amdgcn_mfma_f32_32x32x16_bf16(__builtin_bit_cast(bf16x8_t, A_), __builtin_bit_cast(bf16x8_t, B_), C_, 0, 0, 0)
 #define DAT_MFMA16_OP "v_mfma_f32_32x32x16_bf16"
+#define DAT_MFMA16K32(A_, B_, C_) __builtin_amdgcn_mfma_f32_16x16x32_bf16(__builtin_bit_cast(bf16x8_t, A_), __builtin_bit_cast(bf16x8_t, B_), C_, 0, 0, 0)
+#define DAT_MFMA16K32_OP "v_mfma_f32_16x16x32_bf16"
 #define DAT_H16_FORMAT 0
 #endif
 
```

Measured after the change: 261.2 clips/s (median of 6 runs). +5.0%, better.
